# noporpoise/seq-align

Measured on AMD Instinct MI355X. Metric: dp_cell_updates_per_sec, higher is better.
Workload: dtype int32; 1 GPU; C2: 10k NW pairs, DNA 150x150, default scoring 1/-2/-4/-1 (BASELINE configs[1]); pairs_per_gpu=10000, global_pairs=10000, kernel=stream, arena_placement=spread

## Files before the change

include/seqalign_hip.h:

```cpp
#ifndef SEQALIGN_HIP_H
#define SEQALIGN_HIP_H

#include <stddef.h>
#include <stdint.h>

#include "seqalign_compat.h"

#ifdef __cplusplus
extern "C" {
#endif

enum {
  SEQALIGN_OK = 0,
  SEQALIGN_E_NO_DEVICE = 1,
  SEQALIGN_E_HIP = 2,
  SEQALIGN_E_ARG = 3,
  SEQALIGN_E_NOMEM = 4,
  SEQALIGN_E_UNKNOWN_PAIR = 5,
  SEQALIGN_E_DOMAIN = 6,
  SEQALIGN_E_TRACEBACK = 7,
  SEQALIGN_E_TOO_LARGE = 8
};

const char *seqalign_strerror(int code);
// ... 67 lines not shown
  uint32_t *cand_index;
  int32_t *cand_score;
} seqalign_sw_reduce_t;

int seqalign_sw_reduce_device(seqalign_ctx_t *ctx, const seqalign_sw_reduce_t *r,
                              void *stream);

typedef struct {
  const uint64_t *str_off;
  char *out_a, *out_b;
  uint32_t *out_head, *out_len;
  int32_t *out_score;
  uint32_t *status;
  const uint64_t *start_index;
  uint32_t *out_pos;
} seqalign_trace_t;

int seqalign_nw_traceback_device(seqalign_ctx_t *ctx,
                                 const seqalign_dev_scoring_t *scoring,
                                 const seqalign_dev_batch_t *batch,
                                 const seqalign_trace_t *trace, void *stream);
int seqalign_sw_traceback_device(seqalign_ctx_t *ctx,
                                 const seqalign_dev_scoring_t *scoring,
                                 const seqalign_dev_batch_t *batch,
                                 const seqalign_trace_t *trace, void *stream);

int seqalign_fill_batch(seqalign_ctx_t *ctx, const seqalign_batch_t *batch,
                        const scoring_t *scoring, int is_sw,
                        const uint64_t *mat_off, int32_t *match_scores,
                        int32_t *gap_a_scores, int32_t *gap_b_scores,
                        uint64_t *status);

int seqalign_nw_batch(seqalign_ctx_t *ctx, const seqalign_batch_t *batch,
                      const scoring_t *scoring, const uint64_t *str_off,
                      char *out_a, char *out_b, uint32_t *out_len,
                      int32_t *out_score);

typedef struct {
  uint64_t pair;
  int32_t score;
  uint32_t pos_a, pos_b, len_a, len_b;
  uint32_t length;
  uint64_t str_off;
} seqalign_sw_hit_t;

int seqalign_sw_batch(seqalign_ctx_t *ctx, const seqalign_batch_t *batch,
                      const scoring_t *scoring, const int32_t *min_score,
                      uint32_t max_hits, seqalign_sw_hit_t *hits,
                      uint64_t hit_cap, uint64_t *n_hits, char *out_a,
                      char *out_b, uint64_t str_cap);

typedef struct seqalign_job seqalign_job_t;
int seqalign_nw_batch_submit(seqalign_ctx_t *ctx, const seqalign_batch_t *batch, const scoring_t *scoring,
                             const uint64_t *str_off, char *out_a, char *out_b, uint32_t *out_len, int32_t *out_score,
                             seqalign_job_t **job);
int seqalign_sw_batch_submit(seqalign_ctx_t *ctx, const seqalign_batch_t *batch, const scoring_t *scoring,
                             const int32_t *min_score, uint32_t max_hits, seqalign_sw_hit_t *hits, uint64_t hit_cap,
                             uint64_t *n_hits, char *out_a, char *out_b, uint64_t str_cap, seqalign_job_t **job);
int seqalign_job_wait(seqalign_job_t *job);
int seqalign_job_done(seqalign_job_t *job);

int seqalign_fill_batch_multi(seqalign_ctx_t *const *ctxs, int n_ctx,
                              const seqalign_batch_t *batch, const scoring_t *scoring,
                              int is_sw, const uint64_t *mat_off, int32_t *match_scores,
                              int32_t *gap_a_scores, int32_t *gap_b_scores, uint64_t *status);
int seqalign_nw_batch_multi(seqalign_ctx_t *const *ctxs, int n_ctx,
                            const seqalign_batch_t *batch, const scoring_t *scoring,
                            const uint64_t *str_off, char *out_a, char *out_b,
                            uint32_t *out_len, int32_t *out_score);
int seqalign_sw_batch_multi(seqalign_ctx_t *const *ctxs, int n_ctx,
                            const seqalign_batch_t *batch, const scoring_t *scoring,
                            const int32_t *min_score, uint32_t max_hits,
                            seqalign_sw_hit_t *hits, uint64_t hit_cap, uint64_t *n_hits,
                            char *out_a, char *out_b, uint64_t str_cap);

int seqalign_arenas_alloc(seqalign_ctx_t *ctx, uint64_t bytes_each, void *arenas[3], float *quality);
int seqalign_arenas_free(seqalign_ctx_t *ctx, void *arenas[3]);

#define SEQALIGN_ARENA_MAX_TRIES 96
typedef struct {
  float quality;
  float target;
  int32_t vmm;
  uint32_t chunk_mib;
  float depth_gib;
  float scanned_gib;
  float depth_a_gib;
  uint32_t tries;
  uint32_t second_walk_from;
  float try_quality[SEQALIGN_ARENA_MAX_TRIES];
  float try_depth_gib[SEQALIGN_ARENA_MAX_TRIES];
  float kept_gib;
  float seconds;
} seqalign_arena_info_t;
int seqalign_arenas_info(seqalign_ctx_t *ctx, void *const arenas[3], seqalign_arena_info_t *info);

int seqalign_pool_trim(seqalign_ctx_t *ctx, uint64_t keep_bytes, uint64_t *held_bytes);

int seqalign_ctx_set_option(seqalign_ctx_t *ctx, const char *key, const char *value);

int seqalign_ctx_get_option(const seqalign_ctx_t *ctx, const char *key, char *value, size_t cap);

enum {
  SEQALIGN_K_FILL_WAVEFRONT = 0,
  SEQALIGN_K_FILL_ROWSCAN,
  SEQALIGN_K_FILL_STREAM,
  SEQALIGN_K_FILL_STRIPS,
  SEQALIGN_K_FILL_WGSTREAM,
  SEQALIGN_K_FILL_NW_DIRS,
  SEQALIGN_K_FILL_NW_DIRS_X2,
  SEQALIGN_K_FILL_SW_DIRS,
  SEQALIGN_K_FILL_SW_DIRS_X2,
  SEQALIGN_K_FILL_SW_BEST_X2,
  SEQALIGN_K_SW_REDUCE,
  SEQALIGN_K_SW_BOX,
  SEQALIGN_K_SWEEP_REGS,
  SEQALIGN_K_SWEEP_LDS,
  SEQALIGN_K_SWEEP_STRIPS,
  SEQALIGN_K_SWEEP_DIRS,
  SEQALIGN_K_SWEEP_DIRS_X2,
  SEQALIGN_K_WALK_LANE,
  SEQALIGN_K_WALK_WAVE,
  SEQALIGN_K_WALK_DIRS_LANE,
  SEQALIGN_K_WALK_DIRS_TILE,
  SEQALIGN_K_WALK_MOVES_LANE,
  SEQALIGN_K_WALK_MOVES_TILE,
  SEQALIGN_K_FILL_NW_DIRS_X4,
  SEQALIGN_K_FILL_SW_BEST_X4,
  SEQALIGN_K_SCORE_ROWS,
  SEQALIGN_K_SCORE_STRIPS,
  SEQALIGN_K_SCORE_CROSS,
  SEQALIGN_K_SCORE_SELECT,
  SEQALIGN_K_LONG_FORWARD,
  SEQALIGN_K_LONG_BLOCK,
  SEQALIGN_K_LONG_WALK,
  SEQALIGN_K_COUNT
};
#define SEQALIGN_K_MAX 32
#if defined(__cplusplus)
static_assert(SEQALIGN_K_COUNT <= SEQALIGN_K_MAX, "seqalign_call_info_t has SEQALIGN_K_MAX slots");
#elif defined(__STDC_VERSION__) && __STDC_VERSION__ >= 201112L
_Static_assert(SEQALIGN_K_COUNT <= SEQALIGN_K_MAX, "seqalign_call_info_t has SEQALIGN_K_MAX slots");
#endif
typedef struct {
  uint32_t launches[SEQALIGN_K_MAX];
  uint64_t items[SEQALIGN_K_MAX];
} seqalign_call_info_t;
int seqalign_ctx_last_call_info(const seqalign_ctx_t *ctx, seqalign_call_info_t *out);
const char *seqalign_kernel_kind_name(int kind);
enum {
  SEQALIGN_KX_BAND_SCORE = 0,
  SEQALIGN_KX_BAND_FILL,
  SEQALIGN_KX_BAND_WALK,
  SEQALIGN_KX_COUNT
};
#define SEQALIGN_KX_MAX 32
typedef struct {
  uint32_t launches[SEQALIGN_KX_MAX];
  uint64_t items[SEQALIGN_KX_MAX];
} seqalign_call_info_ext_t;
int seqalign_ctx_last_call_info_ext(const seqalign_ctx_t *ctx, seqalign_call_info_ext_t *out);
const char *seqalign_kernel_kind_ext_name(int kind);

size_t seqalign_cigar(const char *result_a, const char *result_b, size_t length, int extended,
                      int case_insensitive, char *out, size_t cap);

#define SEQALIGN_CIGAR_M 1
#define SEQALIGN_CIGAR_EQX 2
int seqalign_nw_batch_cigar(seqalign_ctx_t *ctx, const seqalign_batch_t *batch, const scoring_t *scoring, int format,
                            const uint64_t *cigar_off, char *cigar, uint32_t *cigar_len, int32_t *out_score);
int seqalign_sw_batch_cigar(seqalign_ctx_t *ctx, const seqalign_batch_t *batch, const scoring_t *scoring,
                            const int32_t *min_score, uint32_t max_hits, int format, seqalign_sw_hit_t *hits,
                            uint64_t hit_cap, uint64_t *n_hits, char *cigar, uint64_t cigar_cap);
int seqalign_nw_batch_cigar_submit(seqalign_ctx_t *ctx, const seqalign_batch_t *batch, const scoring_t *scoring, int format,
                                   const uint64_t *cigar_off, char *cigar, uint32_t *cigar_len, int32_t *out_score,
                                   seqalign_job_t **job);
int seqalign_nw_batch_cigar_multi(seqalign_ctx_t *const *ctxs, int n_ctx, const seqalign_batch_t *batch, const scoring_t *scoring,
                                  int format, const uint64_t *cigar_off, char *cigar, uint32_t *cigar_len, int32_t *out_score);
int seqalign_sw_batch_cigar_multi(seqalign_ctx_t *const *ctxs, int n_ctx, const seqalign_batch_t *batch, const scoring_t *scoring,
                                  const int32_t *min_score, uint32_t max_hits, int format, seqalign_sw_hit_t *hits,
                                  uint64_t hit_cap, uint64_t *n_hits, char *cigar, uint64_t cigar_cap);

int seqalign_nw_score_batch(seqalign_ctx_t *ctx, const seqalign_batch_t *batch, const scoring_t *scoring,
                            int32_t *out_score);
int seqalign_sw_score_batch(seqalign_ctx_t *ctx, const seqalign_batch_t *batch, const scoring_t *scoring,
                            int32_t *out_score, uint32_t *out_end_a, uint32_t *out_end_b);
int seqalign_nw_score_batch_multi(seqalign_ctx_t *const *ctxs, int n_ctx, const seqalign_batch_t *batch,
                                  const scoring_t *scoring, int32_t *out_score);
int seqalign_sw_score_batch_multi(seqalign_ctx_t *const *ctxs, int n_ctx, const seqalign_batch_t *batch,
                                  const scoring_t *scoring, int32_t *out_score, uint32_t *out_end_a, uint32_t *out_end_b);
int seqalign_nw_align_long(seqalign_ctx_t *ctx, const seqalign_batch_t *batch, const scoring_t *scoring,
                           const uint64_t *str_off, char *out_a, char *out_b, uint32_t *out_len, int32_t *out_score);
int seqalign_sw_align_long(seqalign_ctx_t *ctx, const seqalign_batch_t *batch, const scoring_t *scoring,
                           const int32_t *min_score, seqalign_sw_hit_t *hits, uint64_t hit_cap, uint64_t *n_hits,
                           char *out_a, char *out_b, uint64_t str_cap);
#define SEQALIGN_BAND_MAX_WIDTH 1024
int seqalign_nw_score_banded(seqalign_ctx_t *ctx, const seqalign_batch_t *batch, const scoring_t *scoring,
                             const uint32_t *band, int32_t *out_score);
int seqalign_nw_align_banded(seqalign_ctx_t *ctx, const seqalign_batch_t *batch, const scoring_t *scoring,
                             const uint32_t *band, const uint64_t *str_off, char *out_a, char *out_b, uint32_t *out_len,
                             int32_t *out_score);
int seqalign_band_score_time_ms(seqalign_ctx_t *ctx, const seqalign_batch_t *batch, const scoring_t *scoring,
                                const uint32_t *band, int repeats, float *ms_each);
typedef struct {
  uint64_t n_seqs;
  const char *arena;
  uint64_t arena_bytes;
  const uint64_t *off;
  const uint32_t *len;
} seqalign_seqset_t;
int seqalign_nw_score_cross(seqalign_ctx_t *ctx, const seqalign_seqset_t *queries, const seqalign_seqset_t *targets,
                            const scoring_t *scoring, int32_t *out_score);
int seqalign_sw_score_cross(seqalign_ctx_t *ctx, const seqalign_seqset_t *queries, const seqalign_seqset_t *targets,
                            const scoring_t *scoring, int32_t *out_score, uint32_t *out_end_a, uint32_t *out_end_b);
int seqalign_nw_score_cross_multi(seqalign_ctx_t *const *ctxs, int n_ctx, const seqalign_seqset_t *queries,
                                  const seqalign_seqset_t *targets, const scoring_t *scoring, int32_t *out_score);
int seqalign_sw_score_cross_multi(seqalign_ctx_t *const *ctxs, int n_ctx, const seqalign_seqset_t *queries,
                                  const seqalign_seqset_t *targets, const scoring_t *scoring, int32_t *out_score,
                                  uint32_t *out_end_a, uint32_t *out_end_b);
#define SEQALIGN_SEARCH_MAX_K 1024
typedef struct {
  uint32_t target;
  int32_t score;
  uint32_t end_a, end_b;
} seqalign_search_hit_t;
int seqalign_nw_score_search(seqalign_ctx_t *ctx, const seqalign_seqset_t *queries, const seqalign_seqset_t *targets,
                             const scoring_t *scoring, uint32_t k, int32_t min_score, seqalign_search_hit_t *hits,
                             uint32_t *n_hits);
int seqalign_sw_score_search(seqalign_ctx_t *ctx, const seqalign_seqset_t *queries, const seqalign_seqset_t *targets,
                             const scoring_t *scoring, uint32_t k, int32_t min_score, seqalign_search_hit_t *hits,
                             uint32_t *n_hits);
int seqalign_nw_score_search_multi(seqalign_ctx_t *const *ctxs, int n_ctx, const seqalign_seqset_t *queries,
                                   const seqalign_seqset_t *targets, const scoring_t *scoring, uint32_t k, int32_t min_score,
                                   seqalign_search_hit_t *hits, uint32_t *n_hits);
int seqalign_sw_score_search_multi(seqalign_ctx_t *const *ctxs, int n_ctx, const seqalign_seqset_t *queries,
                                   const seqalign_seqset_t *targets, const scoring_t *scoring, uint32_t k, int32_t min_score,
                                   seqalign_search_hit_t *hits, uint32_t *n_hits);
int seqalign_score_time_ms(seqalign_ctx_t *ctx, const seqalign_batch_t *batch, const scoring_t *scoring, int is_sw,
                           int repeats, float *ms_each);

int seqalign_host_legs_nw(const seqalign_batch_t *batch, const uint64_t *str_off, char *out_a, char *out_b,
                          uint32_t *out_len, int iterations, double *pack_ms, double *expand_ms);

void *seqalign_ctx_stream(seqalign_ctx_t *ctx);

int seqalign_time_fill_ms(seqalign_ctx_t *ctx,
                          const seqalign_dev_scoring_t *scoring,
                          const seqalign_dev_batch_t *batch, int kernel,
                          void *stream, int repeats, float *ms_each);

#ifdef __cplusplus
}
#endif
#endif
```

seq-align_amd/csrc/sa_batch.hip:

```cpp
#include "sa_ctx.hpp"

using namespace sa_host;



std::vector<Chunk> sa_host::plan_chunks(const seqalign_batch_t *b, size_t budget, size_t bytes_per_cell, const uint64_t *extra_bytes) {
  std::vector<Chunk> out;
  Chunk c;
  const uint64_t per_cell = std::max<size_t>(bytes_per_cell, 1);
  uint64_t used = 0;
  for (uint64_t p = 0; p < b->n_pairs; ++p) {
    const uint64_t cells = (uint64_t)(b->len_a[p] + 1ull) * (b->len_b[p] + 1ull);
    const uint64_t need = cells * per_cell + (extra_bytes ? extra_bytes[p] : 0);
    if (c.count && used + need > budget) { out.push_back(c); c = Chunk(); c.first = p; used = 0; }
    used += need;
    c.count++; c.cells += cells; c.seq_bytes += (uint64_t)b->len_a[p] + b->len_b[p];
    c.max_a = std::max(c.max_a, b->len_a[p]); c.max_b = std::max(c.max_b, b->len_b[p]);
  }
  if (c.count) out.push_back(c);
  return out;
}

int sa_host::ensure_copy_streams(seqalign_ctx *ctx, int count) {
  int least = 0, greatest = 0;
  bool have_range = false;
  for (int k = 0; k < count; ++k) {
    if (ctx->copy_streams[k]) continue;
    if (!have_range) { HIP_TRY(hipDeviceGetStreamPriorityRange(&least, &greatest)); have_range = true; }
    HIP_TRY(hipStreamCreateWithPriority(&ctx->copy_streams[k], hipStreamNonBlocking, k == 0 ? least : greatest));
  }
  return SEQALIGN_OK;
}

int sa_host::run_chunk(seqalign_ctx *ctx, const seqalign_batch_t *b, const Chunk &c,
                       const seqalign_dev_scoring *sc, seqalign_dev_batch_t *dev_out, bool *best_done,
                       const SaCandBox *cand, bool *cand_done, uint64_t uniform_stride) {
  const bool bucket = uniform_stride == kBucketShapes;
  if (bucket) uniform_stride = 0;
  const uint64_t n = c.count;
  int rc;
  StageTimer tm(ctx->opt.timing);
  const size_t desc_bytes = n * (3 * sizeof(uint64_t) + 2 * sizeof(uint32_t)) + (bucket ? 2 * n * sizeof(uint32_t) : 0);
  if ((rc = ctx->h_desc.reserve(desc_bytes))) return rc;
  if ((rc = ctx->h_arena.reserve(c.seq_bytes + 16))) return rc;
  uint64_t *h_off_a = ctx->h_desc.as<uint64_t>(), *h_off_b = h_off_a + n, *h_mat = h_off_b + n;
  uint32_t *h_len_a = reinterpret_cast<uint32_t *>(h_mat + n), *h_len_b = h_len_a + n;
  uint8_t *h_seq = ctx->h_arena.as<uint8_t>();
  uint64_t pos = 0, cell = 0;
  for (uint64_t k = 0; k < n; ++k) {
    const uint64_t p = c.first + k;
    h_off_a[k] = pos; pos += b->len_a[p];
    h_off_b[k] = pos; pos += b->len_b[p];
    h_len_a[k] = b->len_a[p]; h_len_b[k] = b->len_b[p];
    h_mat[k] = uniform_stride ? k * uniform_stride : cell;
    const uint64_t cells_k = (cand && cand->best_only && sa_dirs_blocked_shape(c.max_a)) ? sa_dirs_blocked_bytes(b->len_a[p], b->len_b[p])
                                                                                       : (uint64_t)(b->len_a[p] + 1ull) * (b->len_b[p] + 1ull);
    cell += bucket ? ((cells_k + 255u) & ~(uint64_t)255u) : cells_k;
  }
  const uint64_t mat_total = uniform_stride ? n * uniform_stride : cell;
  uint32_t *h_list = reinterpret_cast<uint32_t *>(h_len_b + n);
  if ((rc = ctx->arena.reserve(c.seq_bytes + 16))) return rc;
  if ((rc = ctx->off_a.reserve(desc_bytes)) || (rc = ctx->status.reserve(n * 8))) return rc;
  const bool no_matrices = cand && cand->best_only;
  const bool packed_dirs = cand && cand->dirs && (bucket || uniform_stride);
  if (!no_matrices && (rc = reserve_arenas(ctx, mat_total * 4, !packed_dirs))) return rc;
  hipStream_t st = ctx->stream;
  uint32_t list_len[2] = {0, 0};
  if (bucket) {
    const bool split = false;
    const uint64_t first = split ? 2048 : n;
    static thread_local std::vector<uint32_t> tl_table;
    const uint64_t Wb = (uint64_t)c.max_b + 1, entries = ((uint64_t)c.max_a + 1) * Wb;
    if (tl_table.size() < entries) tl_table.resize(entries);
    for (int sl = 0; sl < 2; ++sl) {
      const uint64_t k0 = sl ? first : 0, k1 = sl ? n : first;
      uint32_t *out = h_list + 2 * k0;
      uint32_t at = 0;
      for (uint64_t k = k0; k < k1; ++k) tl_table[(uint64_t)h_len_a[k] * Wb + h_len_b[k]] = ~0u;
      for (uint64_t k = k0; k < k1; ++k) {
        uint32_t &slot = tl_table[(uint64_t)h_len_a[k] * Wb + h_len_b[k]];
        if (slot == ~0u) { slot = (uint32_t)k; continue; }
        out[at++] = slot; out[at++] = (uint32_t)k;
        slot = ~0u;
      }
      for (uint64_t k = k0; k < k1; ++k) {
        uint32_t &slot = tl_table[(uint64_t)h_len_a[k] * Wb + h_len_b[k]];
        if (slot == (uint32_t)k) { out[at++] = (uint32_t)k; out[at++] = (uint32_t)k; slot = ~0u; }
      }
      list_len[sl] = at;
    }
  }
  HIP_TRY(hipMemcpyAsync(ctx->off_a.p, h_off_a, desc_bytes, hipMemcpyHostToDevice, st));
  uint64_t *dv_off_a = ctx->off_a.as<uint64_t>(), *dv_off_b = dv_off_a + n, *dv_mat = dv_off_b + n;
  uint32_t *dv_len_a = reinterpret_cast<uint32_t *>(dv_mat + n), *dv_len_b = dv_len_a + n;
  const uint32_t *dv_list = dv_len_b + n;
  if (best_done && ((rc = ctx->best_score.reserve(n * 4)) || (rc = ctx->best_index.reserve(n * 8)))) return rc;
  auto range_desc = [&](uint64_t k0, uint64_t k1) {
    seqalign_dev_batch_t d;
    d.n_pairs = k1 - k0; d.arena = ctx->arena.as<uint8_t>();
    d.off_a = dv_off_a + k0; d.len_a = dv_len_a + k0;
    d.off_b = dv_off_b + k0; d.len_b = dv_len_b + k0;
    d.mat_off = dv_mat + k0;
    d.match_scores = ctx->M.as<int32_t>(); d.gap_a_scores = ctx->A.as<int32_t>(); d.gap_b_scores = ctx->B.as<int32_t>();
    if (no_matrices) d.match_scores = d.gap_a_scores = d.gap_b_scores = nullptr;
    d.status = ctx->status.as<uint64_t>() + k0; d.max_len_a = c.max_a; d.max_len_b = c.max_b;
    return d;
  };
  auto fill_range = [&](uint64_t k0, uint64_t k1, bool *bd, bool *cd, bool *du) -> int {
    if (bucket) {
      seqalign_dev_batch_t dc = range_desc(0, n);
      dc.n_pairs = k1 - k0;
      SaCandBox sub = *cand;
      bool used = false;
      sub.dirs_used = &used; sub.uniform_stride = 256;
      sub.pair_list = dv_list + 2 * k0; sub.list_count = list_len[k0 ? 1 : 0];
      const int r = no_matrices
          ? fill_device(ctx, sc, &dc, SEQALIGN_KERNEL_AUTO, st, ctx->best_score.as<int32_t>(), ctx->best_index.as<uint64_t>(), bd, &sub, nullptr)
          : fill_device(ctx, sc, &dc, SEQALIGN_KERNEL_AUTO, st, nullptr, nullptr, nullptr, &sub, cd);
      if (du) *du = used;
      if (!r && !used) { set_last_error("internal error: the packed fill refused a ragged chunk it had accepted"); return SEQALIGN_E_HIP; }
      return r;
    }
    const seqalign_dev_batch_t d = range_desc(k0, k1);
    if (best_done && no_matrices) {
      SaCandBox sub = *cand;
      bool used = false;
      sub.dirs_used = &used; sub.uniform_stride = uniform_stride;
      const int r = fill_device(ctx, sc, &d, SEQALIGN_KERNEL_AUTO, st, ctx->best_score.as<int32_t>() + k0,
                                ctx->best_index.as<uint64_t>() + k0, bd, &sub, nullptr);
      if (du) *du = used;
      return r;
    }
    if (best_done)
      return fill_device(ctx, sc, &d, SEQALIGN_KERNEL_AUTO, st, ctx->best_score.as<int32_t>() + k0, ctx->best_index.as<uint64_t>() + k0, bd);
    if (cand) {
      SaCandBox sub = *cand;
      sub.uniform_stride = uniform_stride;
      sub.cand_count += k0; sub.cand_box += 4 * k0; sub.cand_min += k0; sub.hit_off += k0;
      bool used = false;
      sub.dirs_used = cand->dirs_used ? &used : nullptr;
      const int r = fill_device(ctx, sc, &d, SEQALIGN_KERNEL_AUTO, st, nullptr, nullptr, nullptr, &sub, cd);
      if (du) *du = used;
      return r;
    }
    return seqalign_fill_batch_device(ctx, sc, &d, SEQALIGN_KERNEL_AUTO, st);
  };
  constexpr uint64_t kPack = 2048;
  const uint64_t n_sub = (n >= 8192 && c.seq_bytes >= ((uint64_t)4 << 20) && ctx->opt.subbatches != 1 && !uniform_stride && !bucket) ? 4 : 1;
  const bool two_slices = (uniform_stride || bucket) && n_sub > 1;
  const uint64_t slice_bytes = n_sub > 1 ? (c.seq_bytes + n_sub - 1) / n_sub : ((uint64_t)2 << 20);
  { int rc_s = ensure_copy_streams(ctx, 1); if (rc_s) return rc_s; }
  hipStream_t su = ctx->copy_streams[0];
  StreamSyncOnExit sync_u(su);
  EventList ev;
  HIP_TRY(ev.add(hipEventDisableTiming));
  HIP_TRY(hipEventRecord(ev.ev[0], st));
  HIP_TRY(hipStreamWaitEvent(su, ev.ev[0], 0));
  bool first = true, consistent = true, bd0 = false, cd0 = false, du0 = false;
  uint64_t filled_to = 0;
  for (uint64_t k0 = 0; k0 < n;) {
    uint64_t k1 = k0;
    if (two_slices) {
      k1 = k0 == 0 ? std::min(n, kPack) : n;
    } else {
      while (k1 < n && (k1 == k0 || h_off_a[k1] - h_off_a[k0] < slice_bytes)) k1 = std::min(n, k1 + kPack);
    }
    if (n - k1 < kPack) k1 = n;
    constexpr uint64_t kTask = 256;
    parallel_for((k1 - k0 + kTask - 1) / kTask, [&](uint64_t blk) {
      for (uint64_t k = k0 + blk * kTask, e = std::min(k1, k0 + (blk + 1) * kTask); k < e; ++k) {
        const uint64_t p = c.first + k;
        memcpy(h_seq + h_off_a[k], b->arena + b->off_a[p], b->len_a[p]);
        memcpy(h_seq + h_off_b[k], b->arena + b->off_b[p], b->len_b[p]);
      }
    });
    const uint64_t lo = h_off_a[k0], hi = k1 < n ? h_off_a[k1] : c.seq_bytes;
    if (hi > lo) HIP_TRY(hipMemcpyAsync(ctx->arena.as<uint8_t>() + lo, h_seq + lo, hi - lo, hipMemcpyHostToDevice, su));
    HIP_TRY(ev.add(hipEventDisableTiming));
    HIP_TRY(hipEventRecord(ev.ev.back(), su));
    HIP_TRY(hipStreamWaitEvent(st, ev.ev.back(), 0));
    if (n_sub > 1 && consistent) {
      bool bd = false, cd = false, du = false;
      if ((rc = fill_range(k0, k1, &bd, &cd, &du))) return rc;
      if (first) { bd0 = bd; cd0 = cd; du0 = du; first = false; }
      else if (bd != bd0 || cd != cd0 || du != du0) consistent = false;
      filled_to = k1;
    }
    k0 = k1;
  }
  tm.lap("run_chunk: pack + H2D");
  const seqalign_dev_batch_t d = range_desc(0, n);
  if (n_sub > 1 && consistent && filled_to == n) {
    if (best_done) *best_done = bd0;
    if (cand_done) *cand_done = cd0;
    if (cand && cand->dirs_used) *cand->dirs_used = du0;
    rc = SEQALIGN_OK;
  } else {
    bool bd = false, cd = false, du = false;
    rc = fill_range(0, n, &bd, &cd, &du);
    if (best_done) *best_done = bd;
    if (cand_done) *cand_done = cd;
    if (cand && cand->dirs_used) *cand->dirs_used = du;
  }
  if (rc) return rc;
  tm.lap("run_chunk: enqueue fill");
  if (dev_out) *dev_out = d;
  return SEQALIGN_OK;
}

int sa_host::fetch_status(seqalign_ctx *ctx, const Chunk &c, uint64_t *status_out) {
  int rc;
  if ((rc = ctx->h_misc.reserve(c.count * 8))) return rc;
  uint64_t *h = ctx->h_misc.as<uint64_t>();
  HIP_TRY(hipMemcpyAsync(h, ctx->status.p, c.count * 8, hipMemcpyDeviceToHost, ctx->stream));
  HIP_TRY(stream_wait_spinning(ctx->stream));
  rc = SEQALIGN_OK;
  for (uint64_t k = 0; k < c.count; ++k) {
    if (status_out) status_out[c.first + k] = h[k];
    if (h[k] != ~0ull) rc = SEQALIGN_E_UNKNOWN_PAIR;
  }
  return rc;
}

int sa_host::check_batch(const seqalign_batch_t *b) {
  if (!batch_readable(b)) return SEQALIGN_E_ARG;
  for (uint64_t p = 0; p < b->n_pairs; ++p)
    if ((uint64_t)(b->len_a[p] + 1ull) * (b->len_b[p] + 1ull) >= (1ull << 31)) return SEQALIGN_E_TOO_LARGE;
  return SEQALIGN_OK;
}


static int copy_out_pipelined(seqalign_ctx *ctx, void *dst, const void *src_dev, size_t bytes) {
  const size_t kSlice = (size_t)32 << 20;
  if (bytes < (size_t)4 << 20) {
    HIP_TRY(hipMemcpyAsync(dst, src_dev, bytes, hipMemcpyDeviceToHost, ctx->stream));
    HIP_TRY(hipStreamSynchronize(ctx->stream));
    return SEQALIGN_OK;
  }
  int rc;
  if ((rc = ctx->h_M.reserve(kSlice)) || (rc = ctx->h_A.reserve(kSlice))) return rc;
  void *pin[2] = {ctx->h_M.p, ctx->h_A.p};
  EventList events;
  HIP_TRY(events.add(hipEventDisableTiming));
  HIP_TRY(events.add(hipEventDisableTiming));
  const hipEvent_t *ev = events.ev.data();
  StreamSyncOnExit sync(ctx->stream);
  const size_t n_slices = (bytes + kSlice - 1) / kSlice;
  hipError_t e = hipSuccess;
  for (size_t i = 0; i <= n_slices && e == hipSuccess; ++i) {
    if (i < n_slices) {
      const size_t off = i * kSlice, len = std::min(kSlice, bytes - off);
      e = hipMemcpyAsync(pin[i & 1], static_cast<const char *>(src_dev) + off, len, hipMemcpyDeviceToHost, ctx->stream);
      if (e == hipSuccess) e = hipEventRecord(ev[i & 1], ctx->stream);
    }
    if (i > 0 && e == hipSuccess) {
      const size_t j = i - 1, off = j * kSlice, len = std::min(kSlice, bytes - off);
      e = hipEventSynchronize(ev[j & 1]);
      if (e == hipSuccess) parallel_memcpy(static_cast<char *>(dst) + off, pin[j & 1], len);
    }
  }
  if (e != hipSuccess) return fail_hip(e, "pipelined D2H");
  return SEQALIGN_OK;
}

extern "C" int seqalign_fill_batch(seqalign_ctx_t *ctx, const seqalign_batch_t *batch, const scoring_t *scoring,
                                   int is_sw, const uint64_t *mat_off, int32_t *M, int32_t *A, int32_t *B,
                                   uint64_t *status) {
  if (!ctx || !scoring || !mat_off || !M || !A || !B) return SEQALIGN_E_ARG;
  CallScope scope(ctx);
  int rc = check_batch(batch);
  if (rc) return rc;
  if (batch->n_pairs == 0) return SEQALIGN_OK;
  HIP_TRY(hipSetDevice(ctx->device));
  seqalign_dev_scoring *sc = nullptr;
  if ((rc = cached_scoring(ctx, scoring, is_sw, &sc))) return rc;
  return fill_batch_uploaded(ctx, batch, sc, mat_off, M, A, B, status);
}

int sa_host::fill_batch_uploaded(seqalign_ctx_t *ctx, const seqalign_batch_t *batch, const seqalign_dev_scoring *sc,
                                 const uint64_t *mat_off, int32_t *M, int32_t *A, int32_t *B, uint64_t *status) {
  int rc = SEQALIGN_OK;
  int worst = SEQALIGN_OK;
  for (const Chunk &c : plan_chunks(batch, ctx->chunk_budget)) {
    if ((rc = run_chunk(ctx, batch, c, sc, nullptr))) break;
    const size_t small = c.cells * 4;
    if (3 * small <= ((size_t)4 << 20)) {
      const size_t status_at = (3 * small + 7) & ~(size_t)7;
      if ((rc = ctx->h_M.reserve(status_at + c.count * 8 + 64))) break;
      char *pin = ctx->h_M.as<char>();
      hipStream_t st = ctx->stream;
      StreamSyncOnExit sync(st);
      HIP_TRY(hipMemcpyAsync(pin, ctx->M.p, small, hipMemcpyDeviceToHost, st));
      HIP_TRY(hipMemcpyAsync(pin + small, ctx->A.p, small, hipMemcpyDeviceToHost, st));
      HIP_TRY(hipMemcpyAsync(pin + 2 * small, ctx->B.p, small, hipMemcpyDeviceToHost, st));
      HIP_TRY(hipMemcpyAsync(pin + status_at, ctx->status.p, c.count * 8, hipMemcpyDeviceToHost, st));
      HIP_TRY(hipStreamSynchronize(st));
      uint64_t dev_cell = 0;
      const uint64_t *h_status = reinterpret_cast<const uint64_t *>(pin + status_at);
      for (uint64_t k = 0; k < c.count; ++k) {
        const uint64_t p = c.first + k, cells = (uint64_t)(batch->len_a[p] + 1ull) * (batch->len_b[p] + 1ull);
        memcpy(M + mat_off[p], pin + dev_cell * 4, cells * 4);
        memcpy(A + mat_off[p], pin + small + dev_cell * 4, cells * 4);
        memcpy(B + mat_off[p], pin + 2 * small + dev_cell * 4, cells * 4);
        dev_cell += cells;
        if (status) status[p] = h_status[k];
        if (h_status[k] != ~0ull) worst = SEQALIGN_E_UNKNOWN_PAIR;
      }
      continue;
    }
    uint64_t k = 0, dev_cell = 0;
    while (k < c.count) {
      uint64_t run_cells = 0, j = k;
      const uint64_t host0 = mat_off[c.first + k];
      while (j < c.count && mat_off[c.first + j] == host0 + run_cells) {
        run_cells += (uint64_t)(batch->len_a[c.first + j] + 1ull) * (batch->len_b[c.first + j] + 1ull);
        ++j;
      }
      const size_t bytes = run_cells * 4;
      if ((rc = copy_out_pipelined(ctx, M + host0, ctx->M.as<int32_t>() + dev_cell, bytes)) ||
          (rc = copy_out_pipelined(ctx, A + host0, ctx->A.as<int32_t>() + dev_cell, bytes)) ||
          (rc = copy_out_pipelined(ctx, B + host0, ctx->B.as<int32_t>() + dev_cell, bytes)))
        break;
      dev_cell += run_cells;
      k = j;
    }
    if (rc) break;
    int src = fetch_status(ctx, c, status);
    if (src == SEQALIGN_E_UNKNOWN_PAIR) worst = src;
    else if (src) { rc = src; break; }
  }
  return rc ? rc : worst;
}


void sa_host::parallel_memcpy(void *dst, const void *src, size_t bytes) {
  const size_t kPiece = (size_t)2 << 20;
  const uint64_t pieces = (bytes + kPiece - 1) / kPiece;
  parallel_for(pieces, [&](uint64_t i) {
    const size_t off = i * kPiece;
    memcpy(static_cast<char *>(dst) + off, static_cast<const char *>(src) + off, std::min(kPiece, bytes - off));
  });
}
// ... 293 lines not shown
                          uint32_t *out_len, int32_t *out_score) {
  const uint64_t n = c.count, nb = blk.size();
  int rc;
  StageTimer tm(ctx->opt.timing);
  const bool auto_zc = ctx->opt.zero_copy == 4u;
  const bool tile_walks = ctx->opt.trace_kernel ? ctx->opt.trace_kernel == 2 : (ctx->opt.dirs_local != 0 || n < SA_WALK_TILE_MAX);
  const bool zc_in = !auto_zc && (ctx->opt.zero_copy & 1u) != 0, zc_out = auto_zc ? tile_walks : (ctx->opt.zero_copy & 2u) != 0;
  const bool local = tile_walks && ctx->opt.dirs_local;
  bool same_shape = true;
  for (const BlkSum &s : blk) same_shape = same_shape && s.same;

  enum { kBackToBack, kUniform, kMixed } layout = kBackToBack;
  uint64_t stride = 0;
  const bool blocked = sa_dirs_blocked_shape(c.max_a);
  auto dir_bytes = [&](uint32_t la, uint32_t lb) -> uint64_t {
    return ((blocked ? sa_dirs_blocked_bytes(la, lb) : (uint64_t)(la + 1ull) * (lb + 1ull)) + 255u) & ~(uint64_t)255u;
  };
  const bool may_pack = ctx->opt.pack16 && (n >= kPackedFillMinPairs || ctx->opt.pack16 == 2);
  if (same_shape && may_pack && nw_dirs_x2_applicable(ctx, sc, c.max_a, c.max_b)) {
    layout = kUniform;
    stride = dir_bytes(c.max_a, c.max_b);
  } else if (!same_shape && may_pack && (n >= kBucketedFillMinPairs || ctx->opt.pack16 == 2) && (uint64_t)(c.max_a + 1ull) * (c.max_b + 1ull) <= kShapeTableMax &&
             nw_dirs_x2_applicable(ctx, sc, c.max_a, c.max_b)) {
    layout = kMixed;
  }
  std::vector<uint64_t> chars_at(nb + 1, 0), cells_at(nb + 1, 0);
  for (uint64_t bi = 0; bi < nb; ++bi) {
    chars_at[bi + 1] = chars_at[bi] + blk[bi].chars;
    const uint64_t in_blk = std::min(n, (bi + 1) * kHostBlk) - bi * kHostBlk;
    cells_at[bi + 1] = cells_at[bi] + (layout == kUniform ? in_blk * stride : blocked ? blk[bi].blk256 : layout == kMixed ? blk[bi].cells256 : blk[bi].cells);
  }
  const uint64_t total = chars_at[nb], mat_total = cells_at[nb];

  const size_t desc_bytes = (4 * n + 1) * sizeof(uint64_t) + 2 * n * sizeof(uint32_t);
  const uint64_t move_words = 2 * ((total >> 5) + n) + 2;
  if ((rc = ctx->h_desc.reserve(desc_bytes)) || (rc = ctx->h_arena.reserve(total + 64)) ||
      (rc = ctx->h_ta.reserve(move_words * 4)) || (rc = ctx->h_tmeta.reserve(n * 8)) ||
      (rc = ctx->dirs.reserve(mat_total + 4096)) || (rc = ctx->best_score.reserve(n * 4)) || (rc = ctx->best_index.reserve(n * 8)) ||
      (rc = ctx->status.reserve(n * 8)))
    return rc;
  if (!zc_in && ((rc = ctx->arena.reserve(total + 64)) || (rc = ctx->off_a.reserve(desc_bytes)))) return rc;
  if (!zc_out && ((rc = ctx->t_out_a.reserve(move_words * 4)) || (rc = ctx->t_meta.reserve(n * 8)))) return rc;
  if ((rc = ensure_copy_streams(ctx, 3))) return rc;
  hipStream_t sf = ctx->stream, su = ctx->copy_streams[0], sd = ctx->copy_streams[1];

  uint64_t *h_off_a = ctx->h_desc.as<uint64_t>(), *h_off_b = h_off_a + n, *h_mat = h_off_b + n, *h_slot = h_mat + n;
  uint32_t *h_len_a = reinterpret_cast<uint32_t *>(h_slot + n + 1), *h_len_b = h_len_a + n;
  uint8_t *h_seq = ctx->h_arena.as<uint8_t>();
  uint32_t *h_moves = ctx->h_ta.as<uint32_t>(), *h_meta = ctx->h_tmeta.as<uint32_t>();
  parallel_for(nb, [&](uint64_t bi) {
    uint64_t pos = chars_at[bi], cell = cells_at[bi];
    for (uint64_t k = bi * kHostBlk, e = std::min(n, (bi + 1) * kHostBlk); k < e; ++k) {
      const uint32_t la = batch->len_a[c.first + k], lb = batch->len_b[c.first + k];
      h_slot[k] = pos; h_off_a[k] = pos; pos += la; h_off_b[k] = pos; pos += lb;
      h_len_a[k] = la; h_len_b[k] = lb;
      h_mat[k] = cell;
      const uint64_t cells = (uint64_t)(la + 1ull) * (lb + 1ull);
      cell += layout == kUniform ? stride : blocked ? dir_bytes(la, lb) : layout == kMixed ? ((cells + 255u) & ~(uint64_t)255u) : cells;
    }
  });
  h_slot[n] = total;

  const uint32_t n_sub = (uint32_t)std::min<uint64_t>(pick_subbatches(ctx, c), nb);
  std::vector<uint64_t> bcut(n_sub + 1, nb);
  bcut[0] = 0;
  if (layout == kUniform && n_sub > 1 && n / n_sub >= 8192 && kHostBlk <= 4096 && 4096 % kHostBlk == 0) {
    const uint64_t per = (((n + n_sub - 1) / n_sub + 4095u) & ~(uint64_t)4095u) / kHostBlk;
    for (uint32_t s = 1; s < n_sub; ++s) bcut[s] = std::min<uint64_t>(nb, s * per);
  } else {
    uint64_t bi = 0;
    for (uint32_t s = 1; s < n_sub; ++s) {
      const uint64_t want = mat_total / n_sub * s;
      while (bi < nb && cells_at[bi] < want) ++bi;
      bcut[s] = std::max(bi, bcut[s - 1]);
    }
  }
  auto pair_at = [&](uint64_t bi) { return std::min(n, bi * kHostBlk); };
  constexpr uint64_t kGroupPairs = 32768;
  std::vector<uint32_t> gcut{0};
  for (uint32_t s = 1; s < n_sub; ++s)
    if (pair_at(bcut[s]) - pair_at(bcut[gcut.back()]) >= kGroupPairs && n - pair_at(bcut[s]) >= kGroupPairs / 2) gcut.push_back(s);
  gcut.push_back(n_sub);
  const uint32_t n_grp = (uint32_t)gcut.size() - 1;
  const bool walk_beside = ctx->opt.walk_overlap && n_grp > 1;
  hipStream_t sw = walk_beside ? ctx->copy_streams[2] : sf;
  StreamSyncOnExit sync_f(sf), sync_u(su), sync_d(sd), sync_w(sw);

  std::vector<uint32_t> list_at;
  const uint32_t *dv_list = nullptr;
  if (layout == kMixed) {
    const uint64_t entries = (uint64_t)(c.max_a + 1ull) * (c.max_b + 1ull);
    if ((rc = ctx->h_misc.reserve(n * 4 + 16)) || (!zc_in && (rc = ctx->pair_list.reserve(n * 4 + 16)))) return rc;
    uint32_t *h_list = ctx->h_misc.as<uint32_t>();
    list_at.assign(2 * n_sub + 1, 0);
    parallel_for(n_sub, [&](uint64_t s2) {
      static thread_local std::vector<uint32_t> tl_table;
      std::vector<uint32_t> &table = tl_table;
      if (table.size() < entries) table.resize(entries);
      const uint64_t k0 = pair_at(bcut[s2]), k1 = pair_at(bcut[s2 + 1]);
      const uint32_t Wb = c.max_b + 1;
      for (uint64_t k = k0; k < k1; ++k) table[(uint64_t)h_len_a[k] * Wb + h_len_b[k]] = ~0u;
      uint32_t at = (uint32_t)k0;
      for (uint64_t k = k0; k < k1; ++k) {
        uint32_t &slot = table[(uint64_t)h_len_a[k] * Wb + h_len_b[k]];
        if (slot == ~0u) { slot = (uint32_t)k; continue; }
        h_list[at++] = slot; h_list[at++] = (uint32_t)k;
        slot = ~0u;
      }
      const uint32_t paired_end = at;
      for (uint64_t k = k0; k < k1; ++k) {
        uint32_t &slot = table[(uint64_t)h_len_a[k] * Wb + h_len_b[k]];
        if (slot == (uint32_t)k) { h_list[at++] = (uint32_t)k; slot = ~0u; }
      }
      list_at[2 * s2] = (uint32_t)k0; list_at[2 * s2 + 1] = paired_end;
    });
    list_at[2 * n_sub] = (uint32_t)n;
    if (zc_in) dv_list = ctx->h_misc.dev_as<uint32_t>();
    else { dv_list = ctx->pair_list.as<uint32_t>(); HIP_TRY(hipMemcpyAsync(ctx->pair_list.p, h_list, n * 4, hipMemcpyHostToDevice, su)); }
  }

  EventList ev;
  for (uint32_t k = 0; k < n_sub + 3 * n_grp + 1; ++k) HIP_TRY(ev.add(hipEventDisableTiming));
  if (!zc_in && layout == kUniform) {
    hipLaunchKernelGGL(uniform_descriptors_kernel, dim3((unsigned)((n + 256) / 256)), dim3(256), 0, sf, ctx->off_a.as<uint64_t>(),
                       n, c.max_a, c.max_b, stride);
    HIP_TRY(hipGetLastError());
    if (sw != sf) {
      HIP_TRY(hipEventRecord(ev.ev[n_sub + 3 * n_grp], sf));
      HIP_TRY(hipStreamWaitEvent(sw, ev.ev[n_sub + 3 * n_grp], 0));
    }
  } else if (!zc_in) {
    HIP_TRY(hipMemcpyAsync(ctx->off_a.p, h_off_a, desc_bytes, hipMemcpyHostToDevice, sd));
    HIP_TRY(hipEventRecord(ev.ev[n_sub + 3 * n_grp], sd));
    HIP_TRY(hipStreamWaitEvent(sf, ev.ev[n_sub + 3 * n_grp], 0));
    if (sw != sf) HIP_TRY(hipStreamWaitEvent(sw, ev.ev[n_sub + 3 * n_grp], 0));
  }

  const uint64_t *dv_off_a = zc_in ? ctx->h_desc.dev_as<uint64_t>() : ctx->off_a.as<uint64_t>();
  const uint64_t *dv_off_b = dv_off_a + n, *dv_mat = dv_off_b + n, *dv_slot = dv_mat + n;
  const uint32_t *dv_len_a = reinterpret_cast<const uint32_t *>(dv_slot + n + 1), *dv_len_b = dv_len_a + n;
  const uint8_t *dv_seq = zc_in ? ctx->h_arena.dev_as<uint8_t>() : ctx->arena.as<uint8_t>();
  uint32_t *dv_moves = zc_out ? ctx->h_ta.dev_as<uint32_t>() : ctx->t_out_a.as<uint32_t>();
  uint32_t *dv_meta = zc_out ? ctx->h_tmeta.dev_as<uint32_t>() : ctx->t_meta.as<uint32_t>();
  auto dev_range = [&](uint64_t k0, uint64_t k1) {
    seqalign_dev_batch_t d;
    d.n_pairs = k1 - k0; d.arena = dv_seq;
    d.off_a = dv_off_a + k0; d.len_a = dv_len_a + k0; d.off_b = dv_off_b + k0; d.len_b = dv_len_b + k0;
    d.mat_off = dv_mat + k0;
    d.match_scores = d.gap_a_scores = d.gap_b_scores = nullptr;
    d.status = ctx->status.as<uint64_t>() + k0; d.max_len_a = c.max_a; d.max_len_b = c.max_b;
    return d;
  };
  auto move_word = [&](uint64_t k) { return 2 * ((h_slot[k] >> 5) + k); };
  tm.lap("nw moves: sizes, offsets, buffers");

  uint32_t g = 0;
  for (uint32_t s = 0; s < n_sub; ++s) {
    const uint64_t b0 = bcut[s], b1 = bcut[s + 1], k0 = pair_at(b0), k1 = pair_at(b1);
    if (k1 > k0) {
      const uint64_t n_blocks = b1 - b0;
      const uint64_t n_slices = zc_in ? 1 : std::min<uint64_t>(ctx->opt.upload_slices ? ctx->opt.upload_slices : 1, std::max<uint64_t>(1, n_blocks / 2));
      constexpr uint64_t kParts = 4;
      for (uint64_t sl = 0; sl < n_slices; ++sl) {
        const uint64_t sb0 = b0 + n_blocks * sl / n_slices, sb1 = b0 + n_blocks * (sl + 1) / n_slices;
        parallel_for((sb1 - sb0) * kParts, [&](uint64_t ti) {
          const uint64_t bi = sb0 + ti / kParts, part = ti % kParts;
          const uint64_t kb = bi * kHostBlk, ke = std::min(n, (bi + 1) * kHostBlk), span = ke - kb;
          const uint64_t ka = kb + span * part / kParts, kz = kb + span * (part + 1) / kParts;
          if (kz <= ka) return;
          if (blk[bi].packed) {
            const uint64_t bytes = (kz < n ? h_off_a[kz] : total) - h_off_a[ka];
            memcpy(h_seq + h_off_a[ka], batch->arena + batch->off_a[c.first + ka], bytes);
            return;
          }
          for (uint64_t k = ka; k < kz; ++k) {
            const uint64_t p = c.first + k;
            memcpy(h_seq + h_off_a[k], batch->arena + batch->off_a[p], h_len_a[k]);
            memcpy(h_seq + h_off_b[k], batch->arena + batch->off_b[p], h_len_b[k]);
          }
        });
        if (!zc_in) {
          const uint64_t c0 = h_slot[pair_at(sb0)], c1 = h_slot[pair_at(sb1)];
          if (c1 > c0) HIP_TRY(hipMemcpyAsync(ctx->arena.as<uint8_t>() + c0, h_seq + c0, c1 - c0, hipMemcpyHostToDevice, su));
        }
      }
      if (!zc_in) {
        HIP_TRY(hipEventRecord(ev.ev[s], su));
        HIP_TRY(hipStreamWaitEvent(sf, ev.ev[s], 0));
      }
      const seqalign_dev_batch_t d = dev_range(k0, k1);
      if (layout == kMixed) {
        const seqalign_dev_batch_t dm = dev_range(0, n);
        const uint32_t m0 = list_at[2 * s], m1 = list_at[2 * s + 1], r1 = list_at[2 * s + 2];
        if ((rc = nw_dirs_fill_mixed(ctx, sc, &dm, ctx->dirs.as<uint8_t>(), ctx->best_score.as<int32_t>(), ctx->best_index.as<uint64_t>(),
                                     sf, dv_list + m0, m1 - m0, r1 - m1, c.max_a, c.max_b, local)))
          return rc;
      } else {
        bool used = false;
        if ((rc = nw_dirs_fill(ctx, sc, &d, ctx->dirs.as<uint8_t>(), ctx->best_score.as<int32_t>() + k0,
                               ctx->best_index.as<uint64_t>() + k0, sf, &used, layout == kUniform ? stride : 0, nullptr, 0, local)))
          return rc;
        if (!used) { set_last_error("seqalign_nw_batch: internal error: directions-only fill refused a batch it had accepted"); return SEQALIGN_E_HIP; }
      }
    }
    if (s + 1 == gcut[g + 1]) {
      const uint64_t g0 = pair_at(bcut[gcut[g]]), g1 = k1;
      if (g1 > g0) {
        const seqalign_dev_batch_t d = dev_range(g0, g1);
        SaTraceParams t;
        memset(&t, 0, sizeof(t));
        t.arena = d.arena; t.off_a = d.off_a; t.len_a = d.len_a; t.off_b = d.off_b; t.len_b = d.len_b; t.mat_off = d.mat_off;
        t.code = sc->d_code; t.table = sc->d_table;
        t.str_off = dv_slot + g0;
        t.stage_words = (c.max_a + c.max_b + 31u) >> 5;
        t.moves = dv_moves + 2 * g0;
        t.out_meta2 = dv_meta + 2 * g0;
        t.fill_status = d.status;
        t.dirs = ctx->dirs.as<uint8_t>(); t.dirs_blocked = blocked; t.dirs_local = local; t.tune_stage = ctx->opt.walk_stage; t.tune_tile = ctx->opt.walk_tile; t.nw_score = ctx->best_score.as<int32_t>() + g0; t.nw_state = ctx->best_index.as<uint64_t>() + g0;
        t.n_pairs = (uint32_t)(g1 - g0); t.K = sc->flat.n_classes; t.open1 = sc->flat.open1; t.ext = sc->flat.ext;
        t.gen_eq = sc->flat.gen_eq; t.gen_ne = sc->flat.gen_ne; t.flags = sc->flat.flags;
        t.tune_walker = ctx->opt.trace_kernel; t.tune_group = ctx->opt.walk_group;
        hipStream_t sg = g + 1 < n_grp ? sw : sf;
        if (sg != sf) {
          HIP_TRY(hipEventRecord(ev.ev[n_sub + 2 * n_grp + g], sf));
          HIP_TRY(hipStreamWaitEvent(sg, ev.ev[n_sub + 2 * n_grp + g], 0));
        }
        hipError_t e = sa_launch_nw_traceback(t, sg);
        if (e != hipSuccess) return fail_hip(e, "traceback launch");
        if (zc_out) {
          HIP_TRY(hipEventRecord(ev.ev[n_sub + n_grp + g], sg));
        } else {
          HIP_TRY(hipEventRecord(ev.ev[n_sub + g], sg));
          HIP_TRY(hipStreamWaitEvent(sd, ev.ev[n_sub + g], 0));
          const uint64_t w0 = move_word(g0), w1 = g1 < n ? move_word(g1) : move_words - 2;
          HIP_TRY(hipMemcpyAsync(h_moves + w0, ctx->t_out_a.as<uint32_t>() + w0, (w1 - w0) * 4, hipMemcpyDeviceToHost, sd));
          HIP_TRY(hipMemcpyAsync(h_meta + 2 * g0, ctx->t_meta.as<uint32_t>() + 2 * g0, (g1 - g0) * 8, hipMemcpyDeviceToHost, sd));
          HIP_TRY(hipEventRecord(ev.ev[n_sub + n_grp + g], sd));
        }
      } else {
        HIP_TRY(hipEventRecord(ev.ev[n_sub + n_grp + g], sf));
      }
      ++g;
    }
  }
  tm.lap("nw moves: packed + enqueued");

  std::atomic<uint64_t> first_bad{~0ull};
  for (g = 0; g < n_grp; ++g) {
    { const hipError_t e = wait_event_spinning(ev.ev[n_sub + n_grp + g]); if (e != hipSuccess) return fail_hip(e, "waiting for a group's walk"); }
    const uint64_t b0 = bcut[gcut[g]], b1 = bcut[gcut[g + 1]];
    constexpr uint64_t kOut = 128;
    const uint64_t k_lo = pair_at(b0), k_hi = pair_at(b1);
    parallel_for((k_hi - k_lo + kOut - 1) / kOut, [&](uint64_t blk_i) {
      for (uint64_t k = k_lo + blk_i * kOut, e = std::min(k_hi, k_lo + (blk_i + 1) * kOut); k < e; ++k) {
        const uint64_t p = c.first + k;
        if (k + 6 < e) {
          const uint64_t kn = k + 6;
          const uint32_t nwn = (h_len_a[kn] + h_len_b[kn] + 31u) >> 5;
          const uint32_t *pn = h_moves + move_word(kn);
          __builtin_prefetch(h_meta + 2 * kn); __builtin_prefetch(pn + nwn - 1); __builtin_prefetch(pn + 2 * nwn - 1);
          __builtin_prefetch(batch->arena + batch->off_a[c.first + kn]);
        }
        const uint32_t n_moves = h_meta[2 * k + 1];
        int prc = SEQALIGN_OK;
        if (n_moves >= SA_MOVES_ERR) {
          prc = (int)(n_moves & 15u);
        } else {
          const uint32_t nw = (h_len_a[k] + h_len_b[k] + 31u) >> 5;
          const uint32_t *pa = h_moves + move_word(k);
          if (ctx->cigar_format)
            prc = sa_cigar_nw_moves(batch->arena + batch->off_a[p], h_len_a[k], batch->arena + batch->off_b[p], h_len_b[k], pa, pa + nw,
                                    nw, n_moves, ctx->cigar_format, ctx->cigar_fold, out_a + str_off[p], str_off[p + 1] - str_off[p],
                                    &out_len[p], nullptr);
          else
            prc = sa_expand_nw_moves(batch->arena + batch->off_a[p], h_len_a[k], batch->arena + batch->off_b[p], h_len_b[k], pa, pa + nw,
                                     nw, n_moves, out_a + str_off[p], out_b + str_off[p], &out_len[p]);
          out_score[p] = (int32_t)h_meta[2 * k];
        }
        if (prc != SEQALIGN_OK) {
          uint64_t seen = first_bad.load(std::memory_order_relaxed);
          const uint64_t mine = k << 8 | (uint64_t)prc;
          while (mine < seen && !first_bad.compare_exchange_weak(seen, mine, std::memory_order_relaxed)) {}
        }
      }
    });
  }
  tm.lap("nw moves: groups expanded");
  if (first_bad.load() != ~0ull) return (int)(first_bad.load() & 255u);
  return SEQALIGN_OK;
}

extern "C" int seqalign_host_legs_nw(const seqalign_batch_t *batch, const uint64_t *str_off, char *out_a, char *out_b,
                                     uint32_t *out_len, int iterations, double *pack_ms, double *expand_ms) {
  if (!batch || !str_off || !out_a || !out_b || !out_len || iterations <= 0 || !pack_ms || !expand_ms) return SEQALIGN_E_ARG;
  const uint64_t n = batch->n_pairs, kHostBlk = 512;
  if (!n) return SEQALIGN_OK;
  std::vector<BlkSum> blk;
  std::vector<uint64_t> off_a(n), off_b(n), mat(n), slot(n + 1), chars_at, cells_at;
  std::vector<uint32_t> la(n), lb(n);
  std::vector<uint8_t> seq;
  std::vector<uint32_t> moves;
  auto now_ms = [] { timespec t; clock_gettime(CLOCK_MONOTONIC, &t); return t.tv_sec * 1e3 + t.tv_nsec * 1e-6; };
  double t_pack = 0, t_expand = 0;
  for (int it = 0; it < iterations; ++it) {
    const double t0 = now_ms();
    scan_blocks(batch, 0, n, kHostBlk, blk);
    const uint64_t nb = blk.size();
    chars_at.assign(nb + 1, 0); cells_at.assign(nb + 1, 0);
    for (uint64_t bi = 0; bi < nb; ++bi) { chars_at[bi + 1] = chars_at[bi] + blk[bi].chars; cells_at[bi + 1] = cells_at[bi] + blk[bi].cells256; }
    const uint64_t total = chars_at[nb];
    if (seq.size() < total + 64) seq.resize(total + 64);
    if (moves.size() < 2 * ((total >> 5) + n) + 2) moves.assign(2 * ((total >> 5) + n) + 2, 0u);
    parallel_for(nb, [&](uint64_t bi) {
      uint64_t pos = chars_at[bi], cell = cells_at[bi];
      for (uint64_t k = bi * kHostBlk, e = std::min(n, (bi + 1) * kHostBlk); k < e; ++k) {
        la[k] = batch->len_a[k]; lb[k] = batch->len_b[k];
        slot[k] = pos; off_a[k] = pos; pos += la[k]; off_b[k] = pos; pos += lb[k];
        mat[k] = cell; cell += (((uint64_t)(la[k] + 1ull) * (lb[k] + 1ull)) + 255u) & ~(uint64_t)255u;
      }
    });
    parallel_for(nb, [&](uint64_t bi) {
      if (blk[bi].packed) { memcpy(seq.data() + off_a[bi * kHostBlk], batch->arena + batch->off_a[bi * kHostBlk], blk[bi].chars); return; }
      for (uint64_t k = bi * kHostBlk, e = std::min(n, (bi + 1) * kHostBlk); k < e; ++k) {
        memcpy(seq.data() + off_a[k], batch->arena + batch->off_a[k], la[k]);
        memcpy(seq.data() + off_b[k], batch->arena + batch->off_b[k], lb[k]);
      }
    });
    const double t1 = now_ms();
    constexpr uint64_t kOut = 128;
    std::atomic<int> bad{0};
    parallel_for((n + kOut - 1) / kOut, [&](uint64_t bi) {
      for (uint64_t k = bi * kOut, e = std::min(n, (bi + 1) * kOut); k < e; ++k) {
        const uint32_t nw = (la[k] + lb[k] + 31u) >> 5;
        const uint32_t *pa = moves.data() + 2 * ((slot[k] >> 5) + k);
        if (sa_expand_nw_moves(batch->arena + batch->off_a[k], la[k], batch->arena + batch->off_b[k], lb[k], pa, pa + nw, nw,
                               std::min(la[k], lb[k]), out_a + str_off[k], out_b + str_off[k], &out_len[k]))
          bad.store(1);
      }
    });
    const double t2 = now_ms();
    if (bad.load()) return SEQALIGN_E_TRACEBACK;
    t_pack += t1 - t0; t_expand += t2 - t1;
  }
  *pack_ms = t_pack / iterations; *expand_ms = t_expand / iterations;
  return SEQALIGN_OK;
}

static constexpr int kNeedsStrings = -1;
static int nw_batch_impl(seqalign_ctx_t *ctx, const seqalign_batch_t *batch, const scoring_t *scoring,
                         const uint64_t *str_off, char *out_a, char *out_b, uint32_t *out_len,
                         int32_t *out_score) {
  const seqalign_batch_t *b = batch;
  if (!batch_readable(b)) return SEQALIGN_E_ARG;
  if (batch->n_pairs == 0) return SEQALIGN_OK;
  int rc;
  std::vector<BlkSum> blk;
  const uint64_t blk_pairs = host_block_pairs(ctx, batch->n_pairs);
  scan_blocks(batch, 0, batch->n_pairs, blk_pairs, blk);
  Chunk whole;
  whole.count = batch->n_pairs;
  uint64_t cells256 = 0;
  for (const BlkSum &s : blk) {
    if (s.too_large) return SEQALIGN_E_TOO_LARGE;
    whole.cells += s.cells; whole.seq_bytes += s.chars; cells256 += std::max(s.cells256, s.blk256);
    whole.max_a = std::max(whole.max_a, s.max_a); whole.max_b = std::max(whole.max_b, s.max_b);
  }
  HIP_TRY(hipSetDevice(ctx->device));
  seqalign_dev_scoring *sc = nullptr;
  if ((rc = cached_scoring(ctx, scoring, 0, &sc))) return rc;
  const bool on_host = traceback_on_host(ctx);
  if (!on_host && ctx->opt.nw_moves && nw_dirs_applicable(ctx, sc, whole.max_a, batch->n_pairs)) {
    if (cells256 + 64 * batch->n_pairs + whole.seq_bytes <= ctx->chunk_budget)
      return nw_chunk_moves(ctx, batch, whole, sc, blk, blk_pairs, str_off, out_a, out_b, out_len, out_score);
    std::vector<uint64_t> extra(batch->n_pairs, 256 + 64);
    if (SA_DIRS_BLOCKED)
      for (uint64_t p = 0; p < batch->n_pairs; ++p) {
        const uint64_t cells = (uint64_t)(batch->len_a[p] + 1ull) * (batch->len_b[p] + 1ull), bb = sa_dirs_blocked_bytes(batch->len_a[p], batch->len_b[p]);
        if (bb > cells) extra[p] += bb - cells;
      }
    for (const Chunk &c : plan_chunks(batch, ctx->chunk_budget, 1, extra.data())) {
      const uint64_t bp = host_block_pairs(ctx, c.count);
      scan_blocks(batch, c.first, c.count, bp, blk);
      if ((rc = nw_chunk_moves(ctx, batch, c, sc, blk, bp, str_off, out_a, out_b, out_len, out_score))) return rc;
    }
    return SEQALIGN_OK;
  }
  if (ctx->cigar_format) return kNeedsStrings;
  const size_t budget = on_host ? std::min<size_t>(ctx->chunk_budget, (size_t)6 << 30) : ctx->chunk_budget;
  for (const Chunk &c : plan_chunks(batch, budget)) {
    seqalign_dev_batch_t d;
    if (!on_host) {
      if ((rc = nw_chunk_pipelined(ctx, batch, c, sc, pick_subbatches(ctx, c), str_off, out_a, out_b, out_len, out_score))) return rc;
      continue;
    }
    if ((rc = run_chunk(ctx, batch, c, sc, &d))) return rc;
    const size_t bytes = c.cells * 4;
    if ((rc = ctx->h_M.reserve(bytes)) || (rc = ctx->h_A.reserve(bytes)) || (rc = ctx->h_B.reserve(bytes))) return rc;
// ... 86 lines not shown
```

seq-align_amd/csrc/sa_batch_score.hip:

```cpp
#include "sa_ctx.hpp"

using namespace sa_host;

namespace {

constexpr int kRowClasses = SA_SCORE_ROW_CLASSES;
constexpr int kStripClass = kRowClasses;
constexpr uint64_t kPairBytes = 64;
constexpr uint64_t kChunkMaxPairs = (uint64_t)1 << 24;

uint64_t handoff_rows(uint32_t la, uint32_t lb) {
  return la > SA_SCORE_ROW_MAX ? (uint64_t)(sa_score_strips_per_pair(la) - 1) * ((uint64_t)lb + 1) : 0;
}

struct ScoreChunk {
  uint64_t first = 0, count = 0, seq_bytes = 0;
};

std::vector<ScoreChunk> plan_score_chunks(const seqalign_batch_t *b, size_t budget) {
  std::vector<ScoreChunk> out;
  ScoreChunk c;
  uint64_t used = 0;
  for (uint64_t p = 0; p < b->n_pairs; ++p) {
    const uint32_t la = b->len_a[p], lb = b->len_b[p];
    const uint64_t strips = la > SA_SCORE_ROW_MAX ? sa_score_strips_per_pair(la) : 0;
    const uint64_t need = (uint64_t)la + lb + kPairBytes + 8 * handoff_rows(la, lb) + 20 * strips;
    if (c.count && (used + need > budget || c.count == kChunkMaxPairs)) { out.push_back(c); c = ScoreChunk(); c.first = p; used = 0; }
    used += need;
    c.count++; c.seq_bytes += (uint64_t)la + lb;
  }
  if (c.count) out.push_back(c);
  return out;
}

}

SaFillParams sa_host::score_fill_params(const seqalign_dev_scoring *s) {
  SaFillParams p;
  memset(&p, 0, sizeof(p));
  p.code = s->d_code; p.table = s->d_table; p.K = s->flat.n_classes;
  p.gap_open = s->flat.gap_open; p.open1 = s->flat.open1; p.ext = s->flat.ext; p.floor = s->flat.floor;
  p.gen_eq = s->flat.gen_eq; p.gen_ne = s->flat.gen_ne; p.flags = s->flat.flags;
  p.table_abs_max = s->table_abs_max;
  return p;
}

namespace {

struct ScoreChunkRun {
  seqalign_ctx *ctx = nullptr;
  const seqalign_dev_scoring *sc = nullptr;
  bool is_sw = false;
  uint64_t n = 0;
  std::vector<uint32_t> order;
  uint64_t cls_first[kRowClasses + 2] = {};
  uint32_t cls_max_a[kRowClasses + 1] = {};
  uint32_t spp = 1;
  uint64_t strip_words = 0;
  uint64_t *d_off_a = nullptr, *d_off_b = nullptr, *d_hoff = nullptr;
  uint32_t *d_len_a = nullptr, *d_len_b = nullptr;
  uint32_t *d_res = nullptr;

  int prepare(const seqalign_batch_t *b, const ScoreChunk &c) {
    int rc;
    n = c.count;
    uint64_t hand_total = 0;
    order.resize(n);
    sort_by_row_class(n, [&](uint64_t k) { return b->len_a[c.first + k]; }, order.data(), cls_first, cls_max_a);
    const uint64_t n_strip = cls_first[kStripClass + 1] - cls_first[kStripClass];
    spp = n_strip ? sa_score_strips_per_pair(cls_max_a[kStripClass]) : 1;
    strip_words = ((n_strip + 7) / 8) * 8 * spp;

    const size_t desc_bytes = n * (3 * sizeof(uint64_t) + 2 * sizeof(uint32_t));
    if ((rc = ctx->h_desc.reserve(desc_bytes)) || (rc = ctx->h_arena.reserve(c.seq_bytes + 16))) return rc;
    uint64_t *h_off_a = ctx->h_desc.as<uint64_t>(), *h_off_b = h_off_a + n, *h_hoff = h_off_b + n;
    uint32_t *h_len_a = reinterpret_cast<uint32_t *>(h_hoff + n), *h_len_b = h_len_a + n;
    std::vector<uint64_t> seq_at(n);
    { uint64_t pos = 0;
      for (uint64_t k = 0; k < n; ++k) { seq_at[k] = pos; pos += (uint64_t)b->len_a[c.first + k] + b->len_b[c.first + k]; } }
    for (uint64_t s = 0; s < n; ++s) {
      const uint64_t k = order[s], p = c.first + k;
      const uint32_t la = b->len_a[p], lb = b->len_b[p];
      h_off_a[s] = seq_at[k]; h_off_b[s] = seq_at[k] + la;
      h_len_a[s] = la; h_len_b[s] = lb;
      h_hoff[s] = hand_total; hand_total += handoff_rows(la, lb);
    }
    uint8_t *h_seq = ctx->h_arena.as<uint8_t>();
    constexpr uint64_t kTask = 256;
    parallel_for((n + kTask - 1) / kTask, [&](uint64_t blk) {
      for (uint64_t k = blk * kTask, e = std::min(n, (blk + 1) * kTask); k < e; ++k) {
        const uint64_t p = c.first + k;
        memcpy(h_seq + seq_at[k], b->arena + b->off_a[p], b->len_a[p]);
        memcpy(h_seq + seq_at[k] + b->len_a[p], b->arena + b->off_b[p], b->len_b[p]);
      }
    });

    if ((rc = ctx->arena.reserve(c.seq_bytes + 16)) || (rc = ctx->off_a.reserve(desc_bytes)) || (rc = ctx->status.reserve(n * 8)) ||
        (rc = ctx->best_score.reserve(16 + 12 * n)))
      return rc;
    if (n_strip && ((rc = ctx->strip_progress.reserve(sa_strip_progress_bytes(strip_words))) ||
                    (rc = ctx->score_handoff.reserve(8 * hand_total + 16))))
      return rc;
    hipStream_t st = ctx->stream;
    HIP_TRY(hipMemcpyAsync(ctx->off_a.p, h_off_a, desc_bytes, hipMemcpyHostToDevice, st));
    if (c.seq_bytes) HIP_TRY(hipMemcpyAsync(ctx->arena.p, h_seq, c.seq_bytes, hipMemcpyHostToDevice, st));
    d_off_a = ctx->off_a.as<uint64_t>(); d_off_b = d_off_a + n; d_hoff = d_off_b + n;
    d_len_a = reinterpret_cast<uint32_t *>(d_hoff + n); d_len_b = d_len_a + n;
    d_res = ctx->best_score.as<uint32_t>();
    return SEQALIGN_OK;
  }

  int launch() {
    hipStream_t st = ctx->stream;
    HIP_TRY(hipMemsetAsync(d_res, 0, 16, st));
    const SaFillParams f0 = score_fill_params(sc);
    for (int x = 0; x <= kRowClasses; ++x) {
      const uint64_t s0 = cls_first[x], m = cls_first[x + 1] - s0;
      if (!m) continue;
      SaScoreParams p;
      memset(&p, 0, sizeof(p));
      p.f = f0;
      p.f.arena = ctx->arena.as<uint8_t>();
      p.f.off_a = d_off_a + s0; p.f.off_b = d_off_b + s0; p.f.len_a = d_len_a + s0; p.f.len_b = d_len_b + s0;
      p.f.status = ctx->status.as<uint64_t>() + s0;
      p.f.n_pairs = (uint32_t)m;
      p.score = reinterpret_cast<int32_t *>(d_res + 4) + s0;
      p.end_a = d_res + 4 + n + s0; p.end_b = d_res + 4 + 2 * n + s0;
      p.err_flag = d_res;
      hipError_t e;
      if (x == kStripClass) {
        p.progress = ctx->strip_progress.as<uint32_t>();
        p.strip_best = p.progress + sa_strip_best_word(strip_words);
        p.handoff = ctx->score_handoff.as<int32_t>();
        p.handoff_off = d_hoff + s0;
        p.strips_per_pair = spp;
        HIP_TRY(hipMemsetAsync(p.progress, 0, 4 * (strip_words + 1), st));
        HIP_TRY(hipMemsetAsync(p.f.status, 0xff, 8 * m, st));
        e = sa_launch_score_strips(p, is_sw, st);
      } else {
        e = sa_launch_score_rows(p, cls_max_a[x], is_sw, st);
      }
      if (e != hipSuccess) return fail_hip(e, "score kernel launch");
    }
    return SEQALIGN_OK;
  }

  int finish(uint64_t first, int32_t *out_score, uint32_t *out_end_a, uint32_t *out_end_b, uint64_t *fail_pair = nullptr) {
    int rc;
    const size_t words = 4 + (is_sw ? 3 : 1) * n;
    if ((rc = ctx->h_misc.reserve(std::max<size_t>(4 * words, 8 * n)))) return rc;
    uint32_t *h = ctx->h_misc.as<uint32_t>();
    HIP_TRY(hipMemcpyAsync(h, d_res, 4 * words, hipMemcpyDeviceToHost, ctx->stream));
    HIP_TRY(stream_wait_spinning(ctx->stream));
    if (h[0]) {
      std::vector<uint64_t> status(n);
      HIP_TRY(hipMemcpy(status.data(), ctx->status.p, 8 * n, hipMemcpyDeviceToHost));
      uint64_t worst = ~0ull;
      for (uint64_t s = 0; s < n; ++s)
        if (status[s] != ~0ull) worst = std::min<uint64_t>(worst, order[s]);
      if (fail_pair) *fail_pair = first + worst;
      return fail_unknown_pair(first + worst);
    }
    const int32_t *hs = reinterpret_cast<const int32_t *>(h + 4);
    const uint32_t *ha = h + 4 + n, *hb = h + 4 + 2 * n;
    constexpr uint64_t kTask = 16384;
    parallel_for((n + kTask - 1) / kTask, [&](uint64_t blk) {
      for (uint64_t s = blk * kTask, e = std::min(n, (blk + 1) * kTask); s < e; ++s) {
        const uint64_t p = first + order[s];
        out_score[p] = hs[s];
        if (is_sw) { out_end_a[p] = ha[s]; out_end_b[p] = hb[s]; }
      }
    });
    return SEQALIGN_OK;
  }
};

int check_score_batch(const seqalign_batch_t *b) {
  if (!batch_readable(b)) return SEQALIGN_E_ARG;
  return SEQALIGN_OK;
}

}

int sa_host::score_batch_impl(seqalign_ctx_t *ctx, const seqalign_batch_t *batch, const scoring_t *scoring, bool is_sw,
                              int32_t *out_score, uint32_t *out_end_a, uint32_t *out_end_b, uint64_t *fail_pair) {
  int rc = check_score_batch(batch);
  if (rc) return rc;
  if (batch->n_pairs == 0) return SEQALIGN_OK;
  HIP_TRY(hipSetDevice(ctx->device));
  seqalign_dev_scoring *sc = nullptr;
  if ((rc = cached_scoring(ctx, scoring, is_sw ? 1 : 0, &sc))) return rc;
  StreamSyncOnExit sync(ctx->stream);
  for (const ScoreChunk &c : plan_score_chunks(batch, ctx->chunk_budget)) {
    ScoreChunkRun run;
    run.ctx = ctx; run.sc = sc; run.is_sw = is_sw;
    if ((rc = run.prepare(batch, c)) || (rc = run.launch()) ||
        (rc = run.finish(c.first, out_score, out_end_a, out_end_b, fail_pair)))
      return rc;
  }
  return SEQALIGN_OK;
}

extern "C" int seqalign_nw_score_batch(seqalign_ctx_t *ctx, const seqalign_batch_t *batch, const scoring_t *scoring,
                                       int32_t *out_score) {
  if (!ctx || !scoring || !out_score) return SEQALIGN_E_ARG;
  CallScope scope(ctx);
  return score_batch_impl(ctx, batch, scoring, false, out_score, nullptr, nullptr);
}

extern "C" int seqalign_sw_score_batch(seqalign_ctx_t *ctx, const seqalign_batch_t *batch, const scoring_t *scoring,
                                       int32_t *out_score, uint32_t *out_end_a, uint32_t *out_end_b) {
  if (!ctx || !scoring || !out_score || !out_end_a || !out_end_b) return SEQALIGN_E_ARG;
  CallScope scope(ctx);
  return score_batch_impl(ctx, batch, scoring, true, out_score, out_end_a, out_end_b);
}

extern "C" int seqalign_score_time_ms(seqalign_ctx_t *ctx, const seqalign_batch_t *batch, const scoring_t *scoring, int is_sw,
                                      int repeats, float *ms_each) {
  if (!ctx || !scoring || repeats <= 0 || !ms_each) return SEQALIGN_E_ARG;
  CallScope scope(ctx);
  int rc = check_score_batch(batch);
  if (rc) return rc;
  if (batch->n_pairs == 0) return SEQALIGN_E_ARG;
  const std::vector<ScoreChunk> chunks = plan_score_chunks(batch, ctx->chunk_budget);
  if (chunks.size() != 1) { set_last_error("seqalign_score_time_ms: the batch does not fit one chunk"); return SEQALIGN_E_ARG; }
  HIP_TRY(hipSetDevice(ctx->device));
  seqalign_dev_scoring *sc = nullptr;
  if ((rc = cached_scoring(ctx, scoring, is_sw ? 1 : 0, &sc))) return rc;
  StreamSyncOnExit sync(ctx->stream);
  ScoreChunkRun run;
  run.ctx = ctx; run.sc = sc; run.is_sw = is_sw != 0;
  if ((rc = run.prepare(batch, chunks[0]))) return rc;
  EventList events;
  for (int r = 0; r < 2 * repeats; ++r) HIP_TRY(events.add());
  for (int r = 0; r < repeats; ++r) {
    HIP_TRY(hipEventRecord(events.ev[2 * r], ctx->stream));
    if ((rc = run.launch())) return rc;
    HIP_TRY(hipEventRecord(events.ev[2 * r + 1], ctx->stream));
  }
  HIP_TRY(hipStreamSynchronize(ctx->stream));
  for (int r = 0; r < repeats; ++r) HIP_TRY(hipEventElapsedTime(&ms_each[r], events.ev[2 * r], events.ev[2 * r + 1]));
  return SEQALIGN_OK;
}
```

seq-align_amd/csrc/sa_ctx.hpp:

```cpp
#pragma once
#include <hip/hip_runtime.h>
#include <sched.h>
#include <time.h>

#include <algorithm>
#include <atomic>
#include <chrono>
#include <condition_variable>
#include <functional>
#include <thread>
#include <cstdio>
#include <cstdlib>
#include <cstring>
#include <mutex>
#include <string>
#include <vector>

#include "sa_kernels.h"

extern "C" {
#include "sa_internal.h"
}

namespace sa_host {
// ... 94 lines not shown
  const std::function<void(uint64_t)> *fn_ = nullptr;
  uint64_t n_ = 0;
  std::atomic<uint64_t> generation_{0}, next_{0}, open_{0};
  std::atomic<unsigned> active_{0}, sleepers_{0};
  std::atomic<bool> stop_{false};
};

template <class F>
void parallel_for(uint64_t n, F fn) {
  HostPool::get().run(n, std::function<void(uint64_t)>(fn));
}


struct StageTimer {
  bool on;
  explicit StageTimer(bool enabled) : on(enabled) {}
  std::chrono::steady_clock::time_point t = std::chrono::steady_clock::now();
  void lap(const char *what) {
    if (!on) return;
    const auto now = std::chrono::steady_clock::now();
    fprintf(stderr, "[seqalign timing] %-34s %8.3f ms\n", what, std::chrono::duration<double, std::milli>(now - t).count());
    t = now;
  }
};

int fail_hip(hipError_t e, const char *what);
void set_last_error(const std::string &msg);
#define HIP_TRY(expr)                                            \
  do {                                                           \
    hipError_t _e = (expr);                                      \
    if (_e != hipSuccess) return sa_host::fail_hip(_e, #expr);   \
  } while (0)


struct StreamSyncOnExit {
  hipStream_t st;
  explicit StreamSyncOnExit(hipStream_t s) : st(s) {}
  ~StreamSyncOnExit();
  StreamSyncOnExit(const StreamSyncOnExit &) = delete;
  StreamSyncOnExit &operator=(const StreamSyncOnExit &) = delete;
};

struct EventList {
  std::vector<hipEvent_t> ev;
  ~EventList() { for (hipEvent_t e : ev) (void)hipEventDestroy(e); }
  hipError_t add(unsigned flags = hipEventDefault) {
    hipEvent_t e;
    const hipError_t rc = hipEventCreateWithFlags(&e, flags);
    if (rc == hipSuccess) ev.push_back(e);
    return rc;
  }
};

inline hipError_t wait_event_spinning(hipEvent_t e) {
  timespec t0, t1;
  clock_gettime(CLOCK_MONOTONIC, &t0);
  for (unsigned spins = 1;; ++spins) {
    const hipError_t q = hipEventQuery(e);
    if (q != hipErrorNotReady) return q;
    HostPool::cpu_relax();
    if ((spins & 63u) == 0) {
      clock_gettime(CLOCK_MONOTONIC, &t1);
      if ((t1.tv_sec - t0.tv_sec) * 1000000000ll + (t1.tv_nsec - t0.tv_nsec) > 3000000ll) return hipEventSynchronize(e);
    }
  }
}

inline hipError_t stream_wait_spinning(hipStream_t st, long long budget_ns = 3000000ll) {
  timespec t0, t1;
  clock_gettime(CLOCK_MONOTONIC, &t0);
  for (unsigned spins = 1;; ++spins) {
    const hipError_t q = hipStreamQuery(st);
    if (q != hipErrorNotReady) return q;
    HostPool::cpu_relax();
    if ((spins & 63u) == 0) {
      clock_gettime(CLOCK_MONOTONIC, &t1);
      if ((t1.tv_sec - t0.tv_sec) * 1000000000ll + (t1.tv_nsec - t0.tv_nsec) > budget_ns) return hipStreamSynchronize(st);
    }
  }
}

inline StreamSyncOnExit::~StreamSyncOnExit() { (void)stream_wait_spinning(st, 200000ll); }

struct DevBuf {
  void *p = nullptr;
  size_t cap = 0;
  int reserve(size_t bytes) {
    if (bytes <= cap) return SEQALIGN_OK;
    release();
    size_t want = bytes + bytes / 8 + 256;
    int dev = -1;
    if (want >= kPoolFrom && hipGetDevice(&dev) == hipSuccess && (p = sa_pool_alloc(dev, want))) {
      cap = (want + kPoolChunk - 1) / kPoolChunk * kPoolChunk;
      return SEQALIGN_OK;
    }
    hipError_t e = hipMalloc(&p, want);
    if (e != hipSuccess) { p = nullptr; return fail_hip(e, "hipMalloc"); }
    cap = want;
    return SEQALIGN_OK;
  }
  void release() { if (p && !sa_pool_free(p)) (void)hipFree(p); p = nullptr; cap = 0; }
  static constexpr size_t kPoolFrom = (size_t)128 << 20, kPoolChunk = (size_t)512 << 20;
  template <class T> T *as() const { return static_cast<T *>(p); }
};

struct HostBuf {
  void *p = nullptr;
  void *dev = nullptr;
  size_t cap = 0;
  int reserve(size_t bytes) {
    if (bytes <= cap) return SEQALIGN_OK;
    if (p) (void)hipHostFree(p);
    p = nullptr; dev = nullptr; cap = 0;
    size_t want = bytes + bytes / 8 + 256;
    hipError_t e = hipHostMalloc(&p, want, hipHostMallocDefault);
    if (e != hipSuccess) { p = nullptr; return fail_hip(e, "hipHostMalloc"); }
    e = hipHostGetDevicePointer(&dev, p, 0);
    if (e != hipSuccess) { (void)hipHostFree(p); p = nullptr; dev = nullptr; return fail_hip(e, "hipHostGetDevicePointer"); }
    cap = want;
    return SEQALIGN_OK;
  }
  void release() { if (p) (void)hipHostFree(p); p = nullptr; dev = nullptr; cap = 0; }
  template <class T> T *as() const { return static_cast<T *>(p); }
  template <class T> T *dev_as() const { return static_cast<T *>(dev); }
};


}


struct SaOptions {
  int kernel = 0;
  uint32_t cpl = 0;
  uint32_t wpb = 0;
  uint32_t lds_pad = 0;
  bool traceback_host = false;
  uint32_t trace_kernel = 0;
  int sweep_mode = 0;
  uint32_t sweep_strip = 0;
  uint32_t sweep_cpl = 0;
  bool sweep_ev = true;
  bool sweep_trace = false;
  bool nw_dirs = true;
  bool sweep_dirs = true;
  int pack16 = 1;
  uint32_t quad = 0;
  bool walk_overlap = false;
  bool nw_moves = true;
  uint32_t zero_copy = 4;
  uint32_t reduce_depth = 0;
  bool timing = false;
  size_t chunk_bytes = 0;
  uint32_t upload_slices = 0;
  uint32_t subbatches = 0;
  uint32_t arena_scan_gib = 160;
  float arena_quality = 1.045f;
  uint32_t arena_free_pct = 60;
  uint32_t dirs_local = 1;
  uint32_t walk_tile = 0;
  uint32_t walk_stage = 1;
  uint32_t walk_group = 0;
  uint32_t async_lanes = 0;
  uint32_t long_block_rows = 0;
  uint32_t arena_keep_gib = 16;
};

struct seqalign_dev_scoring {
  sa_flat_scoring_t flat;
  uint16_t *d_code = nullptr;
  int32_t *d_table = nullptr;
  int32_t table_abs_max = 0;
};

struct seqalign_ctx {
  int device = 0;
  SaOptions opt;
  hipStream_t stream = nullptr;
  hipStream_t stream2 = nullptr;
  hipStream_t copy_streams[3] = {nullptr, nullptr, nullptr};
  size_t chunk_budget = 0;
  size_t chunk_budget_default = 0;
  sa_host::DevBuf arena, off_a, pair_list, status;
  sa_host::DevBuf M, A, B;
  SaArenaSet *arena_set = nullptr;
  bool arena_placed = false;
  uint32_t arena_walks = 0;
  sa_host::HostBuf h_one;
  void *one_dev = nullptr;
  sa_host::DevBuf dirs;
  sa_host::DevBuf best_score, best_index, cand_count, cand_off, cand_cap, cand_index, cand_score;
  sa_host::DevBuf t_str_off, t_out_a, t_out_b, t_meta;
  sa_host::DevBuf e[14];
  sa_host::DevBuf strip_progress;
  sa_host::DevBuf score_handoff;
  sa_host::DevBuf search_list;
  sa_host::DevBuf long_ckpt, long_block;
  sa_host::HostBuf h_desc, h_arena, h_M, h_A, h_B, h_misc, h_ta, h_tb, h_tmeta;
  seqalign_call_info_t call_info = {};
  seqalign_call_info_ext_t call_info_ext = {};
  int call_depth = 0;
  seqalign_dev_scoring *cached[2] = {nullptr, nullptr};
  uint64_t cached_fp[2] = {0, 0};
  void *async = nullptr;
  int cigar_format = 0;
  bool cigar_fold = false;
};


namespace sa_host {

struct CallScope {
  seqalign_ctx *ctx;
  seqalign_call_info_t *prev;
  seqalign_call_info_ext_t *prev_ext;
  explicit CallScope(seqalign_ctx *c);
  ~CallScope();
  CallScope(const CallScope &) = delete;
  CallScope &operator=(const CallScope &) = delete;
};

void async_shutdown(seqalign_ctx *ctx);

SaFillParams score_fill_params(const seqalign_dev_scoring *s);
int score_batch_impl(seqalign_ctx_t *ctx, const seqalign_batch_t *batch, const scoring_t *scoring, bool is_sw,
                     int32_t *out_score, uint32_t *out_end_a, uint32_t *out_end_b, uint64_t *fail_pair = nullptr);
int score_cross_check(const seqalign_seqset_t *queries, const seqalign_seqset_t *targets);
int score_cross_call(seqalign_ctx_t *ctx, const seqalign_seqset_t *queries, const seqalign_seqset_t *targets,
                     const scoring_t *scoring, bool is_sw, int32_t *out_score, uint32_t *out_end_a, uint32_t *out_end_b,
                     uint64_t q_base);
int score_search_check(const seqalign_seqset_t *queries, const seqalign_seqset_t *targets, uint32_t k);
int score_search_call(seqalign_ctx_t *ctx, const seqalign_seqset_t *queries, const seqalign_seqset_t *targets,
                      const scoring_t *scoring, bool is_sw, uint32_t k, int32_t min_score, seqalign_search_hit_t *hits,
                      uint32_t *n_hits, uint64_t q_base);

struct CigarScope {
  seqalign_ctx *ctx;
  CigarScope(seqalign_ctx *c, int format, bool fold) : ctx(c) { c->cigar_format = format; c->cigar_fold = fold; }
  ~CigarScope() { ctx->cigar_format = 0; ctx->cigar_fold = false; }
  CigarScope(const CigarScope &) = delete;
  CigarScope &operator=(const CigarScope &) = delete;
};

uint64_t put_alignment(const seqalign_ctx *ctx, const char *sa, const char *sb, uint32_t len, char *out_a, char *out_b, uint64_t at, uint64_t room);

int reserve_arenas(seqalign_ctx *ctx, size_t bytes, bool placed = true);

int cached_scoring(seqalign_ctx *ctx, const scoring_t *scoring, int is_sw, seqalign_dev_scoring **out);

int fill_device(seqalign_ctx_t *ctx, const seqalign_dev_scoring_t *scoring, const seqalign_dev_batch_t *batch,
                int kernel, void *stream, int32_t *best_score, uint64_t *best_index, bool *best_done,
                const SaCandBox *cand = nullptr, bool *cand_done = nullptr);

struct Chunk {
  uint64_t first = 0, count = 0;
  uint64_t cells = 0, seq_bytes = 0;
  uint32_t max_a = 0, max_b = 0;
};

std::vector<Chunk> plan_chunks(const seqalign_batch_t *b, size_t budget, size_t bytes_per_cell = 12, const uint64_t *extra_bytes = nullptr);
int run_chunk(seqalign_ctx *ctx, const seqalign_batch_t *b, const Chunk &c, const seqalign_dev_scoring *sc,
              seqalign_dev_batch_t *dev_out, bool *best_done = nullptr, const SaCandBox *cand = nullptr,
              bool *cand_done = nullptr, uint64_t uniform_stride = 0);
int ensure_copy_streams(seqalign_ctx *ctx, int count);
constexpr uint64_t kBucketShapes = ~(uint64_t)0;
constexpr uint64_t kShapeTableMax = (uint64_t)1 << 20;
int fetch_status(seqalign_ctx *ctx, const Chunk &c, uint64_t *status_out);
int nw_dirs_fill(seqalign_ctx_t *ctx, const seqalign_dev_scoring_t *scoring, const seqalign_dev_batch_t *batch, uint8_t *dirs,
                 int32_t *end_score, uint64_t *end_state, void *stream, bool *used, uint64_t uniform_stride = 0,
                 const uint32_t *pair_list = nullptr, uint32_t list_count = 0, bool local = false);
int nw_dirs_fill_mixed(seqalign_ctx_t *ctx, const seqalign_dev_scoring_t *scoring, const seqalign_dev_batch_t *batch, uint8_t *dirs,
                       int32_t *end_score, uint64_t *end_state, void *stream, const uint32_t *list, uint32_t n_modal, uint32_t n_rest,
                       uint32_t modal_a, uint32_t modal_b, bool local = false);
bool nw_dirs_applicable(const seqalign_ctx_t *ctx, const seqalign_dev_scoring_t *scoring, uint32_t max_len_a, uint64_t n_pairs = ~0ull);
bool nw_dirs_x2_applicable(const seqalign_ctx_t *ctx, const seqalign_dev_scoring_t *scoring, uint32_t len_a, uint32_t len_b);
constexpr uint64_t kPackedFillMinPairs = 1025;
constexpr uint64_t kBucketedFillMinPairs = 2048;
bool sw_best_x2_applicable(const seqalign_ctx_t *ctx, const seqalign_dev_scoring_t *scoring, uint32_t len_a, uint32_t len_b);
int sw_traceback_dirs(seqalign_ctx_t *ctx, const seqalign_dev_scoring_t *sc, const seqalign_dev_batch_t *b, const seqalign_trace_t *t,
                      const uint8_t *dirs, const int32_t *start_score, void *stream);
bool sw_dirs_x2_applicable(const seqalign_ctx_t *ctx, const seqalign_dev_scoring_t *scoring, uint32_t len_a, uint32_t len_b);
static inline bool batch_readable(const seqalign_batch_t *b) {
  return b && (!b->n_pairs || (b->arena && b->off_a && b->off_b && b->len_a && b->len_b));
}
int check_batch(const seqalign_batch_t *b);
template <class Len>
void sort_by_row_class(uint64_t n, Len len, uint32_t *order, uint64_t (&cls_first)[SA_SCORE_ROW_CLASSES + 2],
                       uint32_t (&cls_max_a)[SA_SCORE_ROW_CLASSES + 1]) {
  std::fill(std::begin(cls_first), std::end(cls_first), 0);
  std::fill(std::begin(cls_max_a), std::end(cls_max_a), 0);
  std::vector<uint8_t> cls(n);
  for (uint64_t k = 0; k < n; ++k) {
    const uint32_t la = len(k);
    const int x = sa_score_row_class(la);
    cls[k] = (uint8_t)x;
    cls_first[x + 1]++;
    cls_max_a[x] = std::max(cls_max_a[x], la);
  }
  for (int x = 0; x <= SA_SCORE_ROW_CLASSES; ++x) cls_first[x + 1] += cls_first[x];
  uint64_t at[SA_SCORE_ROW_CLASSES + 1];
  std::copy(cls_first, cls_first + SA_SCORE_ROW_CLASSES + 1, at);
  for (uint64_t k = 0; k < n; ++k) order[at[cls[k]]++] = (uint32_t)k;
}
static inline int fail_unknown_pair(uint64_t pair) {
  set_last_error("pair " + std::to_string(pair) + ": a character pair without a score");
  return SEQALIGN_E_UNKNOWN_PAIR;
}
int fill_batch_uploaded(seqalign_ctx_t *ctx, const seqalign_batch_t *batch, const seqalign_dev_scoring *sc,
                        const uint64_t *mat_off, int32_t *M, int32_t *A, int32_t *B, uint64_t *status);
bool traceback_on_host(const seqalign_ctx *ctx);
void parallel_memcpy(void *dst, const void *src, size_t bytes);

}
```

seq-align_amd/csrc/sa_device.hip:

```cpp
#include "sa_ctx.hpp"

#include <algorithm>
#include <atomic>
#include <condition_variable>
#include <mutex>

#include <errno.h>
#include <sched.h>
#include <strings.h>
#include <time.h>
#include <sys/syscall.h>
#include <unistd.h>

using namespace sa_host;

static thread_local std::string g_last_error;

int sa_host::fail_hip(hipError_t e, const char *what) {
  g_last_error = std::string(what) + ": " + hipGetErrorString(e);
  return (e == hipErrorNoDevice || e == hipErrorInvalidDevice) ? SEQALIGN_E_NO_DEVICE
                                                               : SEQALIGN_E_HIP;
}
void sa_host::set_last_error(const std::string &msg) { g_last_error = msg; }

extern "C" const char *seqalign_last_error(void) { return g_last_error.c_str(); }

extern "C" const char *seqalign_strerror(int code) {
  switch (code) {
    case SEQALIGN_OK: return "ok";
    case SEQALIGN_E_NO_DEVICE: return "no HIP device (gfx950) available";
    case SEQALIGN_E_HIP: return "HIP runtime error";
    case SEQALIGN_E_ARG: return "invalid argument";
    case SEQALIGN_E_NOMEM: return "out of memory";
    case SEQALIGN_E_UNKNOWN_PAIR: return "unknown character pair and match/mismatch not set";
    case SEQALIGN_E_DOMAIN: return "scoring outside the defined domain (penalty below -|min_penalty|)";
    case SEQALIGN_E_TRACEBACK: return "traceback failed";
    case SEQALIGN_E_TOO_LARGE: return "pair too large (>= 2^31 cells)";
  }
  return "unknown error";
}

static thread_local seqalign_call_info_t *tl_recorder = nullptr;

void sa_record_launch(int kind, uint64_t items) {
  if (!tl_recorder || kind < 0 || kind >= SEQALIGN_K_COUNT) return;
  tl_recorder->launches[kind] += 1;
  tl_recorder->items[kind] += items;
}

static thread_local seqalign_call_info_ext_t *tl_recorder_ext = nullptr;

void sa_record_launch_ext(int kind, uint64_t items) {
  if (!tl_recorder_ext || kind < 0 || kind >= SEQALIGN_KX_COUNT) return;
  tl_recorder_ext->launches[kind] += 1;
  tl_recorder_ext->items[kind] += items;
}

sa_host::CallScope::CallScope(seqalign_ctx *c) : ctx(c), prev(tl_recorder), prev_ext(tl_recorder_ext) {
  if (!ctx) return;
  if (ctx->call_depth++ == 0) {
    memset(&ctx->call_info, 0, sizeof(ctx->call_info));
    memset(&ctx->call_info_ext, 0, sizeof(ctx->call_info_ext));
  }
  tl_recorder = &ctx->call_info;
  tl_recorder_ext = &ctx->call_info_ext;
}
sa_host::CallScope::~CallScope() {
  if (!ctx) return;
  --ctx->call_depth;
  tl_recorder = prev;
  tl_recorder_ext = prev_ext;
}

extern "C" int seqalign_ctx_last_call_info(const seqalign_ctx_t *ctx, seqalign_call_info_t *out) {
  if (!ctx || !out) return SEQALIGN_E_ARG;
  *out = ctx->call_info;
  return SEQALIGN_OK;
}

extern "C" int seqalign_ctx_last_call_info_ext(const seqalign_ctx_t *ctx, seqalign_call_info_ext_t *out) {
  if (!ctx || !out) return SEQALIGN_E_ARG;
  *out = ctx->call_info_ext;
  return SEQALIGN_OK;
}

extern "C" const char *seqalign_kernel_kind_ext_name(int kind) {
  static const char *names[SEQALIGN_KX_COUNT] = {"band_score", "band_fill", "band_walk"};
  return kind >= 0 && kind < SEQALIGN_KX_COUNT ? names[kind] : nullptr;
}

extern "C" const char *seqalign_kernel_kind_name(int kind) {
  static const char *names[SEQALIGN_K_COUNT] = {
      "fill_wavefront", "fill_rowscan", "fill_stream", "fill_strips", "fill_wgstream", "fill_nw_dirs", "fill_nw_dirs_x2",
      "fill_sw_dirs", "fill_sw_dirs_x2", "fill_sw_best_x2", "sw_reduce", "sw_box", "sweep_regs", "sweep_lds", "sweep_strips",
      "sweep_dirs", "sweep_dirs_x2", "walk_lane", "walk_wave", "walk_dirs_lane", "walk_dirs_tile", "walk_moves_lane",
      "walk_moves_tile", "fill_nw_dirs_x4", "fill_sw_best_x4", "score_rows", "score_strips",
      "score_cross", "score_select", "long_forward", "long_block", "long_walk"};
  return kind >= 0 && kind < SEQALIGN_K_COUNT ? names[kind] : nullptr;
}

static SaPlacementOpts placement_opts(const seqalign_ctx *ctx, bool explicit_call) {
  SaPlacementOpts o;
  o.scan_bytes = (size_t)ctx->opt.arena_scan_gib << 30;
  o.quality_stop = ctx->opt.arena_quality;
  o.keep_bytes = (size_t)ctx->opt.arena_keep_gib << 30;
  o.free_fraction = 0.01f * (float)ctx->opt.arena_free_pct;
  if (!explicit_call) {
    o.free_fraction = 0.25f;
    if (ctx->arena_walks > 0) o.scan_bytes = std::min<size_t>(o.scan_bytes, (size_t)16 << 30);
  }
  return o;
}

int sa_host::reserve_arenas(seqalign_ctx *ctx, size_t bytes, bool placed) {
  if (ctx->arena_set && bytes <= ctx->M.cap && (ctx->arena_placed || !placed)) return SEQALIGN_OK;
  if (ctx->arena_set) {
    (void)hipStreamSynchronize(ctx->stream);
    if (ctx->stream2) (void)hipStreamSynchronize(ctx->stream2);
    for (hipStream_t t : ctx->copy_streams) if (t) (void)hipStreamSynchronize(t);
    sa_arenas_destroy(sa_arenas_take(ctx->M.p));
    ctx->arena_set = nullptr;
  }
  ctx->M = DevBuf(); ctx->A = DevBuf(); ctx->B = DevBuf();
  const size_t want = bytes + (ctx->arena_walks ? bytes / 2 : bytes / 8) + 4096;
  SaArenaSet *set = nullptr;
  SaPlacementOpts po = placement_opts(ctx, false);
  if (!placed) po.scan_bytes = 0;
  hipError_t e = sa_arenas_create(ctx->device, want, ctx->stream, po, &set);
  if (e != hipSuccess) return fail_hip(e, "matrix arenas");
  if (placed) ctx->arena_walks++;
  ctx->arena_placed = placed;
  ctx->arena_set = set;
  void *const *a = sa_arenas_base(set);
  ctx->M.p = a[0]; ctx->A.p = a[1]; ctx->B.p = a[2];
  ctx->M.cap = ctx->A.cap = ctx->B.cap = sa_arenas_bytes(set);
  return SEQALIGN_OK;
}

extern "C" int seqalign_arenas_alloc(seqalign_ctx_t *ctx, uint64_t bytes_each, void *arenas[3], float *quality) {
  if (!ctx || !arenas || !bytes_each) return SEQALIGN_E_ARG;
  HIP_TRY(hipSetDevice(ctx->device));
  SaArenaSet *set = nullptr;
  hipError_t e = sa_arenas_create(ctx->device, (size_t)bytes_each, ctx->stream, placement_opts(ctx, true), &set);
  if (e != hipSuccess) return fail_hip(e, "matrix arenas");
  for (int k = 0; k < 3; ++k) arenas[k] = sa_arenas_base(set)[k];
  if (quality) *quality = sa_arenas_info(set)->quality;
  return SEQALIGN_OK;
}

extern "C" int seqalign_arenas_free(seqalign_ctx_t *ctx, void *arenas[3]) {
  if (!ctx || !arenas) return SEQALIGN_E_ARG;
  if (!arenas[0]) return SEQALIGN_OK;
  HIP_TRY(hipSetDevice(ctx->device));
  SaArenaSet *set = sa_arenas_take(arenas[0]);
  if (!set) { set_last_error("seqalign_arenas_free: not arenas of seqalign_arenas_alloc"); return SEQALIGN_E_ARG; }
  sa_arenas_destroy(set);
  arenas[0] = arenas[1] = arenas[2] = nullptr;
  return SEQALIGN_OK;
}

static_assert(sizeof(seqalign_arena_info_t) == sizeof(SaArenaInfo), "seqalign_arena_info_t mirrors SaArenaInfo");
extern "C" int seqalign_arenas_info(seqalign_ctx_t *ctx, void *const arenas[3], seqalign_arena_info_t *info) {
  if (!ctx || !arenas || !info) return SEQALIGN_E_ARG;
  SaArenaInfo i;
  if (!sa_arenas_copy_info(arenas[0], &i)) return SEQALIGN_E_ARG;
  memcpy(info, &i, sizeof(*info));
  return SEQALIGN_OK;
}

extern "C" int seqalign_device_count(void) {
  int n = 0;
  if (hipGetDeviceCount(&n) != hipSuccess) return 0;
  int ok = 0;
  for (int d = 0; d < n; ++d) {
    hipDeviceProp_t prop;
    if (hipGetDeviceProperties(&prop, d) == hipSuccess && strncmp(prop.gcnArchName, "gfx950", 6) == 0) ++ok;
  }
  return ok;
}

static bool parse_int(const char *val, long long *out) {
  if (!val || !*val) return false;
  char *end = nullptr;
  errno = 0;
  const long long v = strtoll(val, &end, 10);
  if (errno || end == val || *end) return false;
  *out = v;
  return true;
}
static bool parse_bool(const char *val, bool *out) {
  static const char *yes[] = {"1", "true", "on", "yes"}, *no[] = {"0", "false", "off", "no"};
  for (const char *y : yes) if (!strcasecmp(val, y)) { *out = true; return true; }
  for (const char *n : no) if (!strcasecmp(val, n)) { *out = false; return true; }
  return false;
}

static const char *const kKernelNames[] = {"auto", "wavefront", "rowscan", "stream", "strips", "wgstream"};
static const char *const kWalkerNames[] = {"auto", "lane", "wave"};
static const char *const kSweepModes[] = {"auto", "pair", "strips"};

static bool set_option(seqalign_ctx *ctx, const char *key, const char *val) {
  SaOptions &o = ctx->opt;
  auto is = [&](const char *k) { return !strcmp(key, k); };
  auto eq = [&](const char *v) { return !strcmp(val, v); };
  auto name_of = [&](const char *const *names, int n, int *out) { for (int k = 0; k < n; ++k) if (eq(names[k])) { *out = k; return true; } return false; };
  auto number = [&](long long lo, long long hi, long long *out) { long long v; if (!parse_int(val, &v) || v < lo || v > hi) return false; *out = v; return true; };
  auto flag = [&](bool *out) { return parse_bool(val, out); };
  long long num = 0;
  int idx = 0;
  if (is("kernel")) { if (!name_of(kKernelNames, 6, &idx)) return false; o.kernel = idx; return true; }
  if (is("cpl")) { if (!number(0, 16, &num)) return false; o.cpl = (uint32_t)num; return true; }
  if (is("wpb")) { if (!number(0, 8, &num) || (num != 0 && num != 1 && num != 2 && num != 4 && num != 8)) return false; o.wpb = (uint32_t)num; return true; }
  if (is("lds_pad")) { if (!number(0, 160 * 1024, &num)) return false; o.lds_pad = (uint32_t)num; return true; }
  if (is("traceback")) { if (!eq("host") && !eq("device")) return false; o.traceback_host = eq("host"); return true; }
  if (is("trace_kernel")) { if (!name_of(kWalkerNames, 3, &idx)) return false; o.trace_kernel = (uint32_t)idx; return true; }
  if (is("sweep_mode")) { if (!name_of(kSweepModes, 3, &idx)) return false; o.sweep_mode = idx; return true; }
  if (is("sweep_strip")) { if (!number(0, 256, &num) || (num != 0 && num != 64 && num != 128 && num != 256)) return false; o.sweep_strip = (uint32_t)num; return true; }
  if (is("sweep_cpl")) { if (!number(0, 4, &num) || num == 3) return false; o.sweep_cpl = (uint32_t)num; return true; }
  if (is("sweep_ev")) return flag(&o.sweep_ev);
  if (is("sweep_trace")) return flag(&o.sweep_trace);
  if (is("sweep_dirs")) return flag(&o.sweep_dirs);
  if (is("nw_dirs")) return flag(&o.nw_dirs);
  if (is("pack16")) { if (!number(0, 2, &num)) return false; o.pack16 = (int)num; return true; }
  if (is("quad")) { if (!number(0, 2, &num)) return false; o.quad = (uint32_t)num; return true; }
  if (is("walk_overlap")) return flag(&o.walk_overlap);
  if (is("nw_moves")) return flag(&o.nw_moves);
  if (is("zero_copy")) { if (eq("auto")) { o.zero_copy = 4; return true; } if (!number(0, 3, &num)) return false; o.zero_copy = (uint32_t)num; return true; }
  if (is("reduce_depth")) { if (!number(0, 8, &num) || (num != 0 && num != 4 && num != 8)) return false; o.reduce_depth = (uint32_t)num; return true; }
  if (is("timing")) return flag(&o.timing);
  if (is("chunk_bytes")) {
    if (!number(0, (long long)1 << 60, &num) || (num != 0 && num < (1 << 20))) return false;
    o.chunk_bytes = (size_t)num;
    if (num) ctx->chunk_budget = (size_t)num; else ctx->chunk_budget = ctx->chunk_budget_default;
    return true;
  }
  if (is("subbatches")) { if (!number(0, 256, &num)) return false; o.subbatches = (uint32_t)num; return true; }
  if (is("upload_slices")) { if (!number(0, 16, &num)) return false; o.upload_slices = (uint32_t)num; return true; }
  if (is("arena_scan_gib")) { if (!number(0, 1024, &num)) return false; o.arena_scan_gib = (uint32_t)num; return true; }
  if (is("arena_keep_gib")) { if (!number(0, 1024, &num)) return false; o.arena_keep_gib = (uint32_t)num; return true; }
  if (is("async_lanes")) { if (!number(0, 8, &num)) return false; o.async_lanes = (uint32_t)num; return true; }
  if (is("dirs_local")) { if (!number(0, 1, &num)) return false; o.dirs_local = (uint32_t)num; return true; }
  if (is("walk_stage")) { if (!number(0, 1, &num)) return false; o.walk_stage = (uint32_t)num; return true; }
  if (is("walk_tile")) { if (!number(0, 64, &num) || !(num == 0 || num == 32 || num == 64)) return false; o.walk_tile = (uint32_t)num; return true; }
  if (is("walk_group")) { if (!number(0, 8, &num) || !(num == 0 || num == 1 || num == 4 || num == 8)) return false; o.walk_group = (uint32_t)num; return true; }
  if (is("arena_free_pct")) { if (!number(10, 90, &num)) return false; o.arena_free_pct = (uint32_t)num; return true; }
  if (is("long_block_rows")) { if (!number(0, 0xFFFFFFFFll, &num)) return false; o.long_block_rows = (uint32_t)num; return true; }
  if (is("arena_quality")) {
    char *end = nullptr;
    const double q = strtod(val, &end);
    if (end == val || *end || !(q > 0.5 && q < 1.5)) return false;
    o.arena_quality = (float)q;
    return true;
  }
  return false;
}

static bool get_option(const seqalign_ctx *ctx, const char *key, std::string *out) {
  const SaOptions &o = ctx->opt;
  auto is = [&](const char *k) { return !strcmp(key, k); };
  auto n = [&](long long v) { *out = std::to_string(v); return true; };
  if (is("kernel")) { *out = kKernelNames[o.kernel]; return true; }
  if (is("cpl")) return n(o.cpl);
  if (is("wpb")) return n(o.wpb);
  if (is("lds_pad")) return n(o.lds_pad);
  if (is("traceback")) { *out = o.traceback_host ? "host" : "device"; return true; }
  if (is("trace_kernel")) { *out = kWalkerNames[o.trace_kernel]; return true; }
  if (is("sweep_mode")) { *out = kSweepModes[o.sweep_mode]; return true; }
  if (is("sweep_strip")) return n(o.sweep_strip);
  if (is("sweep_cpl")) return n(o.sweep_cpl);
  if (is("sweep_ev")) return n(o.sweep_ev);
  if (is("sweep_trace")) return n(o.sweep_trace);
  if (is("sweep_dirs")) return n(o.sweep_dirs);
  if (is("nw_dirs")) return n(o.nw_dirs);
  if (is("pack16")) return n(o.pack16);
  if (is("quad")) return n(o.quad);
  if (is("walk_overlap")) return n(o.walk_overlap);
  if (is("nw_moves")) return n(o.nw_moves);
  if (is("zero_copy")) { if (o.zero_copy == 4) { *out = "auto"; return true; } return n(o.zero_copy); }
  if (is("reduce_depth")) return n(o.reduce_depth);
  if (is("timing")) return n(o.timing);
  if (is("chunk_bytes")) return n((long long)o.chunk_bytes);
  if (is("subbatches")) return n(o.subbatches);
  if (is("upload_slices")) return n(o.upload_slices);
  if (is("arena_scan_gib")) return n(o.arena_scan_gib);
  if (is("arena_keep_gib")) return n(o.arena_keep_gib);
  if (is("async_lanes")) return n(o.async_lanes);
  if (is("dirs_local")) return n(o.dirs_local);
  if (is("walk_stage")) return n(o.walk_stage);
  if (is("walk_tile")) return n(o.walk_tile);
  if (is("walk_group")) return n(o.walk_group);
  if (is("arena_free_pct")) return n(o.arena_free_pct);
  if (is("long_block_rows")) return n(o.long_block_rows);
  if (is("arena_quality")) { char buf[32]; snprintf(buf, sizeof(buf), "%.6g", (double)o.arena_quality); *out = buf; return true; }
  return false;
}

static void options_from_env(seqalign_ctx *ctx) {
  static const char *keys[] = {"kernel", "cpl", "wpb", "lds_pad", "traceback", "trace_kernel", "sweep_mode", "sweep_strip",
                               "sweep_cpl", "sweep_ev", "sweep_trace", "sweep_dirs", "nw_dirs", "pack16", "quad", "walk_overlap", "nw_moves", "zero_copy", "reduce_depth", "timing", "chunk_bytes", "subbatches", "arena_scan_gib", "arena_quality", "arena_keep_gib", "upload_slices", "arena_free_pct", "async_lanes", "walk_group", "dirs_local", "walk_stage", "walk_tile", "long_block_rows"};
  for (const char *k : keys) {
    std::string name = "SEQALIGN_";
    for (const char *c = k; *c; ++c) name += (char)toupper((unsigned char)*c);
    if (const char *v = getenv(name.c_str())) {
      if (!set_option(ctx, k, v)) fprintf(stderr, "seqalign: ignoring %s=%s (not a value of option \"%s\")\n", name.c_str(), v, k);
    }
  }
}

extern "C" int seqalign_ctx_set_option(seqalign_ctx_t *ctx, const char *key, const char *value) {
  if (!ctx || !key || !value) return SEQALIGN_E_ARG;
  if (!set_option(ctx, key, value)) {
    set_last_error(std::string("seqalign_ctx_set_option: no option \"") + key + "\" with value \"" + value + "\"");
    return SEQALIGN_E_ARG;
  }
  return SEQALIGN_OK;
}

extern "C" int seqalign_ctx_get_option(const seqalign_ctx_t *ctx, const char *key, char *value, size_t cap) {
  if (!ctx || !key || !value) return SEQALIGN_E_ARG;
  std::string v;
  if (!get_option(ctx, key, &v) || v.size() + 1 > cap) return SEQALIGN_E_ARG;
  memcpy(value, v.c_str(), v.size() + 1);
  return SEQALIGN_OK;
}

extern "C" int seqalign_ctx_create(int device, seqalign_ctx_t **out) {
  if (!out) return SEQALIGN_E_ARG;
  *out = nullptr;
  int n = 0;
  hipError_t e = hipGetDeviceCount(&n);
  if (e != hipSuccess || n == 0) {
    set_last_error("hipGetDeviceCount: no device");
    return SEQALIGN_E_NO_DEVICE;
  }
  if (device < 0 || device >= n) return SEQALIGN_E_ARG;
  hipDeviceProp_t prop;
  HIP_TRY(hipGetDeviceProperties(&prop, device));
  if (strncmp(prop.gcnArchName, "gfx950", 6) != 0) {
    set_last_error(std::string("device is ") + prop.gcnArchName + ", kernels are built for gfx950 only");
    return SEQALIGN_E_NO_DEVICE;
  }
  HIP_TRY(hipSetDevice(device));
  seqalign_ctx *ctx = new (std::nothrow) seqalign_ctx();
  if (!ctx) return SEQALIGN_E_NOMEM;
  ctx->device = device;
  e = hipStreamCreateWithFlags(&ctx->stream, hipStreamNonBlocking);
  if (e != hipSuccess) { delete ctx; return fail_hip(e, "hipStreamCreate"); }
  sa_pool_ref(device);
  size_t free_b = 0, total_b = 0;
  (void)hipMemGetInfo(&free_b, &total_b);
  ctx->chunk_budget = free_b ? (free_b / 10) * 4 : (size_t)8 << 30;
  ctx->chunk_budget = std::min<size_t>(ctx->chunk_budget, (size_t)48 << 30);
  ctx->chunk_budget_default = ctx->chunk_budget;
  options_from_env(ctx);
  *out = ctx;
  return SEQALIGN_OK;
}

extern "C" void seqalign_ctx_destroy(seqalign_ctx_t *ctx) {
  if (!ctx) return;
  async_shutdown(ctx);
  (void)hipSetDevice(ctx->device);
  (void)hipStreamSynchronize(ctx->stream);
  for (int k = 0; k < 2; ++k) if (ctx->cached[k]) seqalign_scoring_release(ctx, ctx->cached[k]);
  if (ctx->arena_set) sa_arenas_destroy(sa_arenas_take(ctx->M.p));
  for (DevBuf *b : {&ctx->arena, &ctx->off_a, &ctx->pair_list,
                    &ctx->status, &ctx->best_score, &ctx->best_index, &ctx->dirs,
                    &ctx->cand_count, &ctx->cand_off, &ctx->cand_cap, &ctx->cand_index, &ctx->cand_score,
                    &ctx->t_str_off, &ctx->t_out_a, &ctx->t_out_b, &ctx->t_meta})
    b->release();
  for (DevBuf &b : ctx->e) b.release();
  ctx->strip_progress.release();
  ctx->score_handoff.release();
  ctx->search_list.release();
  ctx->long_ckpt.release();
  ctx->long_block.release();
  for (HostBuf *b : {&ctx->h_one, &ctx->h_desc, &ctx->h_arena, &ctx->h_M, &ctx->h_A, &ctx->h_B, &ctx->h_misc, &ctx->h_ta,
                     &ctx->h_tb, &ctx->h_tmeta})
    b->release();
  if (ctx->stream2) (void)hipStreamDestroy(ctx->stream2);
  for (hipStream_t t : ctx->copy_streams) if (t) (void)hipStreamDestroy(t);
  (void)hipStreamDestroy(ctx->stream);
  sa_pool_unref(ctx->device);
  delete ctx;
}

extern "C" int seqalign_pool_trim(seqalign_ctx_t *ctx, uint64_t keep_bytes, uint64_t *held_bytes) {
  if (!ctx) return SEQALIGN_E_ARG;
  HIP_TRY(hipSetDevice(ctx->device));
  if (keep_bytes != UINT64_MAX) sa_pool_trim(ctx->device, (size_t)keep_bytes);
  if (held_bytes) *held_bytes = sa_pool_bytes(ctx->device);
  return SEQALIGN_OK;
}

extern "C" int seqalign_ctx_device(const seqalign_ctx_t *ctx) { return ctx ? ctx->device : -1; }

extern "C" int seqalign_scoring_upload(seqalign_ctx_t *ctx, const scoring_t *scoring, int is_sw,
                                       seqalign_dev_scoring_t **out) {
  if (!ctx || !scoring || !out) return SEQALIGN_E_ARG;
  *out = nullptr;
  seqalign_dev_scoring *h = new (std::nothrow) seqalign_dev_scoring();
  if (!h) return SEQALIGN_E_NOMEM;
  int rc = sa_flatten_scoring(scoring, is_sw, &h->flat);
  if (rc != SEQALIGN_OK) { delete h; return rc; }
  HIP_TRY(hipSetDevice(ctx->device));
  const size_t tb = sizeof(int32_t) * h->flat.n_classes * h->flat.n_classes;
  hipError_t e = hipMalloc((void **)&h->d_code, sizeof(h->flat.code));
  if (e == hipSuccess) e = hipMalloc((void **)&h->d_table, tb);
  if (e == hipSuccess) e = hipMemcpy(h->d_code, h->flat.code, sizeof(h->flat.code), hipMemcpyHostToDevice);
  if (e == hipSuccess) e = hipMemcpy(h->d_table, h->flat.table, tb, hipMemcpyHostToDevice);
  if (e != hipSuccess) {
    seqalign_scoring_release(ctx, h);
    return fail_hip(e, "scoring upload");
  }
  for (size_t k = 0; k < (size_t)h->flat.n_classes * h->flat.n_classes; ++k) {
    const int32_t v = h->flat.table[k];
    if (v == SA_S_BLOCKED || v == SA_S_UNKNOWN) continue;
    h->table_abs_max = std::max(h->table_abs_max, v < 0 ? (v == INT32_MIN ? INT32_MAX : -v) : v);
  }
  *out = h;
  return SEQALIGN_OK;
}

extern "C" void seqalign_scoring_release(seqalign_ctx_t *ctx, seqalign_dev_scoring_t *h) {
  if (!h) return;
  if (ctx) (void)hipSetDevice(ctx->device);
  if (h->d_code) (void)hipFree(h->d_code);
  if (h->d_table) (void)hipFree(h->d_table);
  sa_flat_scoring_free(&h->flat);
  if (ctx) for (int k = 0; k < 2; ++k) if (ctx->cached[k] == h) ctx->cached[k] = nullptr;
  delete h;
}


static SaFillParams make_params(const seqalign_ctx *ctx, const seqalign_dev_scoring_t *s, const seqalign_dev_batch_t *b) {
  SaFillParams p;
  p.tune_cpl = ctx->opt.cpl; p.tune_wpb = ctx->opt.wpb; p.tune_lds_pad = ctx->opt.lds_pad; p.tune_quad = ctx->opt.quad;
  p.arena = b->arena; p.off_a = b->off_a; p.len_a = b->len_a; p.off_b = b->off_b; p.len_b = b->len_b;
  p.mat_off = b->mat_off; p.M = b->match_scores; p.A = b->gap_a_scores; p.B = b->gap_b_scores;
  p.status = b->status; p.code = s->d_code; p.table = s->d_table;
  p.n_pairs = (uint32_t)b->n_pairs; p.K = s->flat.n_classes;
  p.gap_open = s->flat.gap_open; p.open1 = s->flat.open1; p.ext = s->flat.ext; p.floor = s->flat.floor;
  p.gen_eq = s->flat.gen_eq; p.gen_ne = s->flat.gen_ne; p.flags = s->flat.flags;
  p.best_score = nullptr; p.best_index = nullptr;
  p.cand_min = nullptr; p.cand_count = nullptr; p.cand_box = nullptr; p.cand_rows = nullptr; p.cand_rows_off = nullptr;
  p.uniform_stride = 0;
  p.pair_list = nullptr;
  p.table_abs_max = s->table_abs_max;
  return p;
}

static int pick_kernel(const seqalign_ctx *ctx, int kernel) {
  if (kernel != SEQALIGN_KERNEL_AUTO) return kernel;
  if (ctx->opt.kernel != SEQALIGN_KERNEL_AUTO) return ctx->opt.kernel;
  return SEQALIGN_KERNEL_STREAM;
}

int sa_host::fill_device(seqalign_ctx_t *ctx, const seqalign_dev_scoring_t *scoring, const seqalign_dev_batch_t *batch,
                         int kernel, void *stream, int32_t *best_score, uint64_t *best_index, bool *best_done,
                         const SaCandBox *cand, bool *cand_done) {
  if (best_done) *best_done = false;
  if (cand_done) *cand_done = false;
  if (!ctx || !scoring || !batch) return SEQALIGN_E_ARG;
  if (batch->n_pairs == 0) return SEQALIGN_OK;
  if (batch->n_pairs > 0xFFFFFFFFull) return SEQALIGN_E_ARG;
  if ((uint64_t)(batch->max_len_a + 1ull) * (batch->max_len_b + 1ull) >= (1ull << 31)) return SEQALIGN_E_TOO_LARGE;
  hipStream_t st = stream ? (hipStream_t)stream : ctx->stream;
  SaFillParams p = make_params(ctx, scoring, batch);
  hipError_t e;
  (void)hipGetLastError();
  int which = pick_kernel(ctx, kernel);
  const bool stream_ok = sa_stream_kernel_applicable(p, batch->max_len_a);
  if (kernel == SEQALIGN_KERNEL_AUTO && ctx->opt.kernel == SEQALIGN_KERNEL_AUTO) {
    const bool wg_ok = sa_wgstream_kernel_applicable(p, batch->max_len_a) &&
                       (batch->max_len_a + 1 > 768 || batch->n_pairs < 8192);
    const uint32_t few = !wg_ok ? 256u : (batch->max_len_a + 1 <= 2048 ? 128u : 256u);
    if (batch->max_len_a > 512 && batch->n_pairs < few) which = SEQALIGN_KERNEL_STRIPS;
    else if (wg_ok) which = SEQALIGN_KERNEL_WGSTREAM;
    else if (!stream_ok || (batch->max_len_a > 767 && batch->n_pairs < 768)) which = SEQALIGN_KERNEL_ROWSCAN;
  }
  if (which == SEQALIGN_KERNEL_STREAM && !stream_ok) which = SEQALIGN_KERNEL_ROWSCAN;
  if (which == SEQALIGN_KERNEL_WGSTREAM && !sa_wgstream_kernel_applicable(p, batch->max_len_a))
    which = SEQALIGN_KERNEL_ROWSCAN;
  if ((which == SEQALIGN_KERNEL_STREAM || which == SEQALIGN_KERNEL_WGSTREAM) && best_score && best_index) {
    p.best_score = best_score; p.best_index = best_index;
    const bool reports = which == SEQALIGN_KERNEL_STREAM
                             ? sa_stream_kernel_reports_best(p, batch->max_len_a, batch->max_len_b)
                             : sa_wgstream_kernel_reports_best(p, batch->max_len_a, batch->max_len_b);
    if (reports) { if (best_done) *best_done = true; }
    else p.best_score = nullptr, p.best_index = nullptr;
  }
  if (cand && cand->dirs_used) *cand->dirs_used = false;
  if (cand && cand->best_only) {
    p.best_score = best_score; p.best_index = best_index;
    p.uniform_stride = cand->uniform_stride;
    p.dirs_local = cand->dirs_local ? 1u : 0u;
    if (cand->pair_list) { p.pair_list = cand->pair_list; p.n_pairs = cand->list_count; }
    if (!cand->dirs || !cand->dirs_used || !sa_sw_best_x2_applicable(p, batch->max_len_a, batch->max_len_b, cand->dirs)) {
      set_last_error("internal error: the best-hit direction fill was asked for a batch outside its domain");
      return SEQALIGN_E_ARG;
    }
    e = sa_launch_fill_sw_best_x2(p, batch->max_len_a, cand->dirs, st);
    if (e != hipSuccess) return fail_hip(e, "fill kernel launch");
    *cand->dirs_used = true;
    if (best_done) *best_done = true;
    return SEQALIGN_OK;
  }
  if (cand && cand->dirs && cand->dirs_used && ctx->opt.sweep_dirs && kernel == SEQALIGN_KERNEL_AUTO &&
      ctx->opt.kernel == SEQALIGN_KERNEL_AUTO) {
    p.cand_min = cand->cand_min; p.cand_count = cand->cand_count; p.cand_box = cand->cand_box; p.cand_rows = cand->cand_rows;
    p.cand_rows_off = cand->hit_off;
    if (sa_dirs_fill_applicable(p, batch->max_len_a, cand->dirs)) {
      p.uniform_stride = ctx->opt.pack16 ? cand->uniform_stride : 0;
      const bool packed = sa_dirs_x2_applicable(p, batch->max_len_a, batch->max_len_b, cand->dirs);
      if (packed && cand->pair_list) { p.pair_list = cand->pair_list; p.n_pairs = cand->list_count; }
      e = packed ? sa_launch_fill_dirs_x2(p, batch->max_len_a, cand->dirs, st)
                 : sa_launch_fill_dirs(p, batch->max_len_a, cand->dirs, st);
      if (e != hipSuccess) return fail_hip(e, "fill kernel launch");
      *cand->dirs_used = true;
      if (cand_done) *cand_done = true;
      return SEQALIGN_OK;
    }
    p.cand_min = nullptr; p.cand_count = nullptr; p.cand_box = nullptr; p.cand_rows = nullptr; p.cand_rows_off = nullptr;
  }
  if ((which == SEQALIGN_KERNEL_STREAM || which == SEQALIGN_KERNEL_WGSTREAM) && cand) {
    p.cand_min = cand->cand_min; p.cand_count = cand->cand_count; p.cand_box = cand->cand_box; p.cand_rows = cand->cand_rows;
    p.cand_rows_off = cand->hit_off;
    const bool reports = which == SEQALIGN_KERNEL_STREAM ? sa_stream_kernel_emits_candidates(p, batch->max_len_a)
                                                          : sa_wgstream_kernel_emits_candidates(p, batch->max_len_a);
    if (reports) { if (cand_done) *cand_done = true; }
    else p.cand_count = nullptr;
  }
// ... 423 lines not shown
```

seq-align_amd/host/sa_internal.h:

```cpp
#ifndef SA_INTERNAL_H
#define SA_INTERNAL_H

#include <stddef.h>
#include <stdint.h>

#include "alignment.h"
#include "seqalign_hip.h"

#ifdef __cplusplus
extern "C" {
#endif

int sa_scoring_lookup_rc(const scoring_t *sc, int a, int b, int *score, int *is_match);
int sa_fold_char(const scoring_t *sc, int c);

#define SA_S_BLOCKED ((int32_t)INT32_MIN)
#define SA_S_UNKNOWN ((int32_t)(INT32_MIN + 1))

enum {
  SA_F_NO_START_GAP = 1u << 0,
  SA_F_NO_END_GAP   = 1u << 1,
  SA_F_NO_GAPS_A    = 1u << 2,
  SA_F_NO_GAPS_B    = 1u << 3,
  SA_F_NO_MISMATCH  = 1u << 4,
  SA_F_IS_SW        = 1u << 5,
  SA_F_HAS_SENTINEL = 1u << 6
};

typedef struct {
  int32_t gap_open;
  int32_t open1;
  int32_t ext;
  int32_t floor;
  int32_t gen_eq;
  int32_t gen_ne;
  uint32_t flags;
  uint32_t n_classes;
  uint16_t code[256];
  int32_t *table;
} sa_flat_scoring_t;

int sa_flatten_scoring(const scoring_t *sc, int is_sw, sa_flat_scoring_t *out);
void sa_flat_scoring_free(sa_flat_scoring_t *f);

seqalign_ctx_t *sa_default_ctx_or_die(void);

int sa_fill_one_pair(seqalign_ctx_t *ctx, const scoring_t *sc, int is_sw,
                     const char *a, size_t len_a, const char *b, size_t len_b,
                     int32_t *M, int32_t *A, int32_t *B, uint64_t *status);

typedef struct {
  const scoring_t *sc;
  const char *a, *b;
  size_t len_a, len_b;
  const int32_t *M, *A, *B;
} sa_view_t;

int sa_reverse_move_rc(const sa_view_t *v, int *matrix, int32_t *score,
                       size_t *x, size_t *y);
int sa_nw_traceback(const sa_view_t *v, char *out_a, char *out_b,
                    size_t *out_len, int32_t *out_score);

int sa_expand_nw_moves(const char *a, uint32_t len_a, const char *b, uint32_t len_b, const uint32_t *plane_a,
                       const uint32_t *plane_b, uint32_t n_words, uint32_t n_moves, char *out_a, char *out_b,
                       uint32_t *out_len);
int sa_expand_sw_moves(const char *a, const char *b, uint32_t end_x, uint32_t end_y, const uint32_t *plane_a,
                       const uint32_t *plane_b, uint32_t n_words, uint32_t n_moves, char *out_a, char *out_b,
                       uint32_t pos[4]);
int sa_moves_uses_simd(void);
void sa_moves_force_scalar(int on);
int sa_cigar_nw_moves(const char *a, uint32_t len_a, const char *b, uint32_t len_b, const uint32_t *plane_a,
                      const uint32_t *plane_b, uint32_t n_words, uint32_t n_moves, int format, int fold, char *out, uint64_t cap,
                      uint32_t *out_len, uint32_t *out_columns);
int sa_cigar_sw_moves(const char *a, const char *b, uint32_t end_x, uint32_t end_y, const uint32_t *plane_a,
                      const uint32_t *plane_b, uint32_t n_words, uint32_t n_moves, int format, int fold, char *out, uint64_t cap,
                      uint32_t pos[4], uint32_t *out_len);

typedef int (*sa_hit_sink_t)(void *user, int32_t score, size_t end_x, size_t end_y,
                             size_t x, size_t y, size_t steps);

#ifdef __cplusplus
}
#endif
#endif
```

seq-align_amd/python/seqalign_amd/__init__.py:

```python
from __future__ import annotations

import ctypes as C
from pathlib import Path

import numpy as np

from . import workloads

PKG_ROOT = Path(__file__).resolve().parents[2]
REPO_ROOT = PKG_ROOT.parent
import os as _os
LIB_PATH = Path(_os.environ.get("SEQALIGN_LIB") or (PKG_ROOT / "lib" / "libseqalign_hip.so"))

OK, E_NO_DEVICE, E_HIP, E_ARG, E_NOMEM, E_UNKNOWN_PAIR, E_DOMAIN, E_TRACEBACK, E_TOO_LARGE = range(9)
KERNEL_AUTO, KERNEL_WAVEFRONT, KERNEL_ROWSCAN, KERNEL_STREAM, KERNEL_STRIPS, KERNEL_WGSTREAM = 0, 1, 2, 3, 4, 5
KERNEL_NAMES = {KERNEL_AUTO: "auto", KERNEL_WAVEFRONT: "wavefront", KERNEL_ROWSCAN: "rowscan",
                KERNEL_STREAM: "stream", KERNEL_STRIPS: "strips", KERNEL_WGSTREAM: "wgstream"}
STATUS_OK = 0xFFFFFFFFFFFFFFFF


class Scoring(C.Structure):
    _fields_ = [
        ("gap_open", C.c_int), ("gap_extend", C.c_int),
        ("no_start_gap_penalty", C.c_bool), ("no_end_gap_penalty", C.c_bool),
        ("no_gaps_in_a", C.c_bool), ("no_gaps_in_b", C.c_bool),
        ("no_mismatches", C.c_bool), ("use_match_mismatch", C.c_bool),
        ("match", C.c_int), ("mismatch", C.c_int),
        ("case_sensitive", C.c_bool),
        ("wildcards", C.c_uint32 * 8), ("swap_set", (C.c_uint32 * 8) * 256),
        ("wildscores", C.c_int * 256), ("swap_scores", (C.c_int * 256) * 256),
        ("min_penalty", C.c_int), ("max_penalty", C.c_int),
    ]


class BatchDesc(C.Structure):
    _fields_ = [("n_pairs", C.c_uint64), ("arena", C.c_void_p), ("arena_bytes", C.c_uint64),
                ("off_a", C.c_void_p), ("len_a", C.c_void_p), ("off_b", C.c_void_p), ("len_b", C.c_void_p)]


class DevBatchDesc(C.Structure):
    _fields_ = [("n_pairs", C.c_uint64), ("arena", C.c_void_p), ("off_a", C.c_void_p),
                ("len_a", C.c_void_p), ("off_b", C.c_void_p), ("len_b", C.c_void_p),
                ("mat_off", C.c_void_p), ("match_scores", C.c_void_p), ("gap_a_scores", C.c_void_p),
                ("gap_b_scores", C.c_void_p), ("status", C.c_void_p),
                ("max_len_a", C.c_uint32), ("max_len_b", C.c_uint32)]


class SwReduceDesc(C.Structure):
    _fields_ = [("n_pairs", C.c_uint64), ("len_a", C.c_void_p), ("len_b", C.c_void_p),
                ("mat_off", C.c_void_p), ("match_scores", C.c_void_p), ("min_score", C.c_int32),
                ("best_score", C.c_void_p), ("best_index", C.c_void_p), ("cand_count", C.c_void_p),
                ("cand_off", C.c_void_p), ("cand_cap", C.c_void_p), ("cand_index", C.c_void_p),
                ("cand_score", C.c_void_p)]


class SeqSetDesc(C.Structure):
    _fields_ = [("n_seqs", C.c_uint64), ("arena", C.c_void_p), ("arena_bytes", C.c_uint64), ("off", C.c_void_p),
                ("len", C.c_void_p)]


INT32_MIN = -2**31
SEARCH_MAX_K = 1024
SEARCH_HIT = np.dtype([("target", np.uint32), ("score", np.int32), ("end_a", np.uint32), ("end_b", np.uint32)])


class SwHit(C.Structure):
    _fields_ = [("pair", C.c_uint64), ("score", C.c_int32), ("pos_a", C.c_uint32), ("pos_b", C.c_uint32),
                ("len_a", C.c_uint32), ("len_b", C.c_uint32), ("length", C.c_uint32), ("str_off", C.c_uint64)]


class SeqAlignError(RuntimeError):
    def __init__(self, code: int, where: str):
        l = lib()
        super().__init__(f"{where}: {l.seqalign_strerror(code).decode()} [{code}] {l.seqalign_last_error().decode()}")
        self.code = code


_lib = None


def lib():
    global _lib
    if _lib is None:
        if not LIB_PATH.exists():
            raise FileNotFoundError(
                f"{LIB_PATH} missing: build it with `make -C {PKG_ROOT}` "
                "(or python -c 'import __graft_entry__ as g; g.build()'); there is no CPU path")
        try:
            import torch
        except ImportError:
            pass
        l = C.CDLL(str(LIB_PATH))
        l.seqalign_strerror.restype = C.c_char_p
        l.seqalign_last_error.restype = C.c_char_p
        l.seqalign_kernel_kind_name.restype = C.c_char_p
        l.seqalign_kernel_kind_ext_name.restype = C.c_char_p
        l.needleman_wunsch_new.restype = C.c_void_p
        l.smith_waterman_new.restype = C.c_void_p
        l.alignment_create.restype = C.c_void_p
        l.smith_waterman_get_aligner.restype = C.c_void_p
        _lib = l
    return _lib


def _check(code: int, where: str):
    if code != OK:
        raise SeqAlignError(code, where)


def _ptr(arr) -> C.c_void_p:
    return C.c_void_p(arr.ctypes.data) if arr is not None else C.c_void_p(0)


def make_scoring(spec: dict) -> Scoring:
    l = lib()
    sc = Scoring()
    C.memset(C.byref(sc), 0, C.sizeof(sc))
    if "preset" in spec:
        getattr(l, "scoring_system_" + spec["preset"])(C.byref(sc))
    else:
        l.scoring_init(C.byref(sc), *[C.c_int(int(v)) for v in spec["init"][:4]],
                       *[C.c_bool(bool(v)) for v in spec["init"][4:]])
    for ch, s in spec.get("wildcards", []):
        l.scoring_add_wildcard(C.byref(sc), C.c_char(ch.encode()), C.c_int(s))
    for a, b, s in spec.get("mutations", []):
        l.scoring_add_mutation(C.byref(sc), C.c_char(a.encode()), C.c_char(b.encode()), C.c_int(s))
    if "use_match_mismatch" in spec:
        sc.use_match_mismatch = bool(spec["use_match_mismatch"])
    for k, v in spec.get("flags", {}).items():
        setattr(sc, k, bool(v))
    return sc


def batch_desc(batch: "workloads.Batch") -> BatchDesc:
    return BatchDesc(batch.n_pairs, batch.arena.ctypes.data, batch.arena.nbytes,
                     batch.off_a.ctypes.data, batch.len_a.ctypes.data,
                     batch.off_b.ctypes.data, batch.len_b.ctypes.data)


OPTION_DEFAULTS = {"kernel": "auto", "cpl": 0, "wpb": 0, "lds_pad": 0, "traceback": "device", "trace_kernel": "auto",
                   "sweep_mode": "auto", "sweep_strip": 0, "sweep_cpl": 0, "sweep_trace": 0, "sweep_dirs": 1, "nw_dirs": 1, "pack16": 1, "quad": 0, "walk_overlap": 0, "timing": 0, "chunk_bytes": 0,
                   "subbatches": 0, "arena_scan_gib": 160, "arena_quality": 1.045, "arena_keep_gib": 16, "upload_slices": 0, "arena_free_pct": 60, "nw_moves": 1, "zero_copy": "auto", "sweep_ev": 1, "reduce_depth": 0, "async_lanes": 0, "walk_group": 0, "dirs_local": 1, "walk_stage": 1, "walk_tile": 0, "long_block_rows": 0}


K_MAX = 32


class CallInfo(C.Structure):
    _fields_ = [("launches", C.c_uint32 * K_MAX), ("items", C.c_uint64 * K_MAX)]


KX_MAX = 32


class CallInfoExt(C.Structure):
    _fields_ = [("launches", C.c_uint32 * KX_MAX), ("items", C.c_uint64 * KX_MAX)]


class ArenaInfo(C.Structure):
    _fields_ = [("quality", C.c_float), ("target", C.c_float), ("vmm", C.c_int32), ("chunk_mib", C.c_uint32),
                ("depth_gib", C.c_float), ("scanned_gib", C.c_float), ("depth_a_gib", C.c_float), ("tries", C.c_uint32),
                ("second_walk_from", C.c_uint32), ("try_quality", C.c_float * 96), ("try_depth_gib", C.c_float * 96),
                ("kept_gib", C.c_float), ("seconds", C.c_float)]

    def as_dict(self):
        n = int(self.tries)
        return {"quality": round(float(self.quality), 3), "target": round(float(self.target), 3), "vmm": bool(self.vmm),
                "chunk_mib": int(self.chunk_mib), "depth_gib": round(float(self.depth_gib), 1),
                "scanned_gib": round(float(self.scanned_gib), 1), "depth_a_gib": round(float(self.depth_a_gib), 1),
                "tries": n, "second_walk_from": int(self.second_walk_from), "kept_gib": round(float(self.kept_gib), 1), "seconds": round(float(self.seconds), 3),
                "try_quality": [round(float(self.try_quality[i]), 3) for i in range(n)],
                "try_depth_gib": [round(float(self.try_depth_gib[i]), 1) for i in range(n)]}


class Context:

    def __init__(self, device: int = 0):
        self._h = C.c_void_p(0)
        _check(lib().seqalign_ctx_create(C.c_int(device), C.byref(self._h)), "seqalign_ctx_create")
        self.device = device

    def close(self):
        if self._h:
            lib().seqalign_ctx_destroy(self._h)
            self._h = C.c_void_p(0)

    def __enter__(self):
        return self

    def __exit__(self, *exc):
        self.close()

    def pool_trim(self, keep_bytes=None) -> int:
        held = C.c_uint64(0)
        keep = C.c_uint64(0xFFFFFFFFFFFFFFFF if keep_bytes is None else int(keep_bytes))
        _check(lib().seqalign_pool_trim(self._h, keep, C.byref(held)), "seqalign_pool_trim")
        return int(held.value)

    def set_option(self, key: str, value) -> None:
        if isinstance(value, (bool, np.bool_)):
            value = int(value)
        _check(lib().seqalign_ctx_set_option(self._h, key.encode(), str(value).encode()), f"seqalign_ctx_set_option({key}={value})")

    def get_option(self, key: str) -> str:
        buf = C.create_string_buffer(64)
        _check(lib().seqalign_ctx_get_option(self._h, key.encode(), buf, C.c_size_t(64)), f"seqalign_ctx_get_option({key})")
        return buf.value.decode()

    def options(self, **kv):
        ctx = self

        class _Scope:
            def __enter__(self_inner):
                self_inner.before = {k: ctx.get_option(k) for k in kv}
                for k, v in kv.items():
                    ctx.set_option(k, v)
                return ctx

            def __exit__(self_inner, *exc):
                for k, v in self_inner.before.items():
                    ctx.set_option(k, v)
        return _Scope()

    def last_call(self) -> dict:
        info = CallInfo()
        _check(lib().seqalign_ctx_last_call_info(self._h, C.byref(info)), "seqalign_ctx_last_call_info")
        out = {}
        for k in range(K_MAX):
            if info.launches[k]:
                name = lib().seqalign_kernel_kind_name(C.c_int(k))
                out[name.decode() if name else f"kind{k}"] = (int(info.launches[k]), int(info.items[k]))
        ext = CallInfoExt()
        _check(lib().seqalign_ctx_last_call_info_ext(self._h, C.byref(ext)), "seqalign_ctx_last_call_info_ext")
        for k in range(KX_MAX):
            if ext.launches[k]:
                name = lib().seqalign_kernel_kind_ext_name(C.c_int(k))
                out[name.decode() if name else f"kind_ext{k}"] = (int(ext.launches[k]), int(ext.items[k]))
        return out

    def upload_scoring(self, scoring: Scoring, is_sw: int) -> C.c_void_p:
        h = C.c_void_p(0)
        _check(lib().seqalign_scoring_upload(self._h, C.byref(scoring), C.c_int(is_sw), C.byref(h)),
               "seqalign_scoring_upload")
        return h

    def release_scoring(self, h):
        lib().seqalign_scoring_release(self._h, h)

    def _handles(self, peers):
        ctxs = [self] + list(peers)
        return (C.c_void_p * len(ctxs))(*[c._h for c in ctxs]), C.c_int(len(ctxs))

    def fill_batch(self, batch, scoring: Scoring, is_sw: int, check: bool = True, out=None, peers=None):
        cells = batch.matrix_cells()
        mat_off = np.zeros(batch.n_pairs, np.uint64)
        if batch.n_pairs:
            mat_off[1:] = np.cumsum(cells)[:-1]
        total = int(cells.sum())
        if out is not None:
            M, A, B = out
            assert M.size >= total and A.size >= total and B.size >= total
        else:
            M = np.empty(total, np.int32); A = np.empty(total, np.int32); B = np.empty(total, np.int32)
        status = np.zeros(batch.n_pairs, np.uint64)
        d = batch_desc(batch)
        if peers:
            hs, nh = self._handles(peers)
            rc = lib().seqalign_fill_batch_multi(hs, nh, C.byref(d), C.byref(scoring), C.c_int(is_sw), _ptr(mat_off),
                                                 _ptr(M), _ptr(A), _ptr(B), _ptr(status))
        else:
            rc = lib().seqalign_fill_batch(self._h, C.byref(d), C.byref(scoring), C.c_int(is_sw), _ptr(mat_off),
                                           _ptr(M), _ptr(A), _ptr(B), _ptr(status))
        if check:
            _check(rc, "seqalign_fill_batch")
        return (M, A, B, mat_off, status) if check else (rc, M, A, B, mat_off, status)

    def nw_batch(self, batch, scoring: Scoring, raw: bool = False, peers=None):
        n = batch.n_pairs
        cache = getattr(self, "_nw_buffers", None)
        if raw and cache is not None and cache[0] is batch:
            str_off, out_a, out_b, out_len, out_score = cache[1]
        else:
            caps = batch.len_a.astype(np.uint64) + batch.len_b.astype(np.uint64) + np.uint64(1)
            str_off = np.zeros(n, np.uint64)
            if n:
                str_off[1:] = np.cumsum(caps)[:-1]
            total = int(caps.sum()) + 1
            out_a, out_b = np.zeros(total, np.uint8), np.zeros(total, np.uint8)
            out_len, out_score = np.zeros(n, np.uint32), np.zeros(n, np.int32)
            if raw:
                self._nw_buffers = (batch, (str_off, out_a, out_b, out_len, out_score))
        d = batch_desc(batch)
        if peers:
            hs, nh = self._handles(peers)
            _check(lib().seqalign_nw_batch_multi(hs, nh, C.byref(d), C.byref(scoring), _ptr(str_off), _ptr(out_a),
                                                 _ptr(out_b), _ptr(out_len), _ptr(out_score)), "seqalign_nw_batch_multi")
        else:
            _check(lib().seqalign_nw_batch(self._h, C.byref(d), C.byref(scoring), _ptr(str_off), _ptr(out_a),
                                           _ptr(out_b), _ptr(out_len), _ptr(out_score)), "seqalign_nw_batch")
        if raw:
            return str_off, out_a, out_b, out_len, out_score
        res = []
        for p in range(n):
            o, ln = int(str_off[p]), int(out_len[p])
            res.append((int(out_score[p]), out_a[o:o + ln].tobytes(), out_b[o:o + ln].tobytes()))
        return res

    def sw_batch(self, batch, scoring: Scoring, min_score, max_hits: int = 1 << 20, hit_cap: int | None = None,
                 raw: bool = False, peers=None):
        n = batch.n_pairs
        ms = np.full(n, min_score, np.int32) if np.isscalar(min_score) else np.asarray(min_score, np.int32)
        hit_cap = hit_cap or max(1024, 64 * n)
        str_cap = int(hit_cap * (int(batch.len_a.max(initial=0)) + int(batch.len_b.max(initial=0)) + 2))
        str_cap = min(str_cap, 1 << 30)
        cache = getattr(self, "_sw_buffers", None)
        if raw and cache is not None and cache[0] is batch and cache[1] == (hit_cap, str_cap):
            hits, out_a, out_b = cache[2]
        else:
            hits = (SwHit * hit_cap)()
            out_a, out_b = np.zeros(str_cap, np.uint8), np.zeros(str_cap, np.uint8)
            if raw:
                self._sw_buffers = (batch, (hit_cap, str_cap), (hits, out_a, out_b))
        n_hits = C.c_uint64(0)
        d = batch_desc(batch)
        if peers:
            hs, nh = self._handles(peers)
            _check(lib().seqalign_sw_batch_multi(hs, nh, C.byref(d), C.byref(scoring), _ptr(ms),
                                                 C.c_uint32(min(max_hits, 0xFFFFFFFF)), hits, C.c_uint64(hit_cap),
                                                 C.byref(n_hits), _ptr(out_a), _ptr(out_b), C.c_uint64(str_cap)),
                   "seqalign_sw_batch_multi")
        else:
            _check(lib().seqalign_sw_batch(self._h, C.byref(d), C.byref(scoring), _ptr(ms), C.c_uint32(min(max_hits, 0xFFFFFFFF)),
                                           hits, C.c_uint64(hit_cap), C.byref(n_hits), _ptr(out_a), _ptr(out_b),
                                           C.c_uint64(str_cap)), "seqalign_sw_batch")
        if raw:
            return n_hits.value, hits, out_a, out_b
        per_pair = [[] for _ in range(n)]
        for k in range(n_hits.value):
            h = hits[k]
            per_pair[h.pair].append(dict(score=h.score, pos_a=h.pos_a, pos_b=h.pos_b, len_a=h.len_a, len_b=h.len_b,
                                         a=out_a[h.str_off:h.str_off + h.length].tobytes().decode(),
                                         b=out_b[h.str_off:h.str_off + h.length].tobytes().decode()))
        return per_pair

    def nw_score(self, batch, scoring: Scoring, peers=None) -> np.ndarray:
        _score_args(batch, scoring)
        score = np.zeros(batch.n_pairs, np.int32)
        d = batch_desc(batch)
        if peers:
            hs, nh = self._handles(peers)
            _check(lib().seqalign_nw_score_batch_multi(hs, nh, C.byref(d), C.byref(scoring), _ptr(score)),
                   "seqalign_nw_score_batch_multi")
        else:
            _check(lib().seqalign_nw_score_batch(self._h, C.byref(d), C.byref(scoring), _ptr(score)), "seqalign_nw_score_batch")
        return score

    def sw_score(self, batch, scoring: Scoring, peers=None):
        _score_args(batch, scoring)
        n = batch.n_pairs
        score, end_a, end_b = np.zeros(n, np.int32), np.zeros(n, np.uint32), np.zeros(n, np.uint32)
        d = batch_desc(batch)
        if peers:
            hs, nh = self._handles(peers)
            _check(lib().seqalign_sw_score_batch_multi(hs, nh, C.byref(d), C.byref(scoring), _ptr(score), _ptr(end_a),
                                                       _ptr(end_b)), "seqalign_sw_score_batch_multi")
        else:
            _check(lib().seqalign_sw_score_batch(self._h, C.byref(d), C.byref(scoring), _ptr(score), _ptr(end_a), _ptr(end_b)),
                   "seqalign_sw_score_batch")
        return score, end_a, end_b

    def nw_score_cross(self, queries, targets, scoring: Scoring, peers=None) -> np.ndarray:
        _cross_args(queries, targets, scoring)
        score = np.zeros((queries.n_seqs, targets.n_seqs), np.int32)
        dq, dt = seqset_desc(queries), seqset_desc(targets)
        if peers:
            hs, nh = self._handles(peers)
            _check(lib().seqalign_nw_score_cross_multi(hs, nh, C.byref(dq), C.byref(dt), C.byref(scoring), _ptr(score)),
                   "seqalign_nw_score_cross_multi")
        else:
            _check(lib().seqalign_nw_score_cross(self._h, C.byref(dq), C.byref(dt), C.byref(scoring), _ptr(score)),
                   "seqalign_nw_score_cross")
        return score

    def sw_score_cross(self, queries, targets, scoring: Scoring, peers=None):
        _cross_args(queries, targets, scoring)
        shape = (queries.n_seqs, targets.n_seqs)
        score, end_a, end_b = np.zeros(shape, np.int32), np.zeros(shape, np.uint32), np.zeros(shape, np.uint32)
        dq, dt = seqset_desc(queries), seqset_desc(targets)
        if peers:
# ... 301 lines not shown


class _RawDeviceInts:

    def __init__(self, ptr: int, count: int):
        self.__cuda_array_interface__ = {"shape": (count,), "typestr": "<i4", "data": (int(ptr), False),
                                         "version": 3, "strides": None}


class DeviceBatch:

    def __init__(self, batch, device: int = 0, pad_cells: int = 32, placement: str = "spread", ctx=None):
        import torch
        self.torch = torch
        self.host = batch
        dev = torch.device("cuda", device)
        self.device = device
        cells = batch.matrix_cells()
        padded = (cells + pad_cells - 1) // pad_cells * pad_cells
        mat_off = np.zeros(batch.n_pairs, np.int64)
        if batch.n_pairs:
            mat_off[1:] = np.cumsum(padded)[:-1]
        self.mat_off_host = mat_off.astype(np.uint64)
        self.cells_host = cells
        self.total_cells = int(padded.sum())
        t = lambda a: torch.from_numpy(a.view(np.int64) if a.dtype == np.uint64 else
                                       (a.view(np.int32) if a.dtype == np.uint32 else a)).to(dev)
        self.arena = t(batch.arena)
        self.off_a, self.len_a = t(batch.off_a), t(batch.len_a)
        self.off_b, self.len_b = t(batch.off_b), t(batch.len_b)
        self.mat_off = t(self.mat_off_host)
        stride = (self.total_cells + 1023) // 1024 * 1024
        self.placement_quality = -1.0
        self.placement_info = None
        if placement == "packed":
            stride += int(_os.environ.get("SEQALIGN_ARENA_SKEW", "0")) // 256 * 256
            self._arena3 = torch.empty(3 * stride + 1024, dtype=torch.int32, device=dev)
            skew = (-(self._arena3.data_ptr() // 4)) % 1024
            self.M = self._arena3[skew:skew + self.total_cells]
            self.A = self._arena3[skew + stride:skew + stride + self.total_cells]
            self.B = self._arena3[skew + 2 * stride:skew + 2 * stride + self.total_cells]
        else:
            self._ctx = ctx if ctx is not None else _arena_context(device)
            ptrs = (C.c_void_p * 3)()
            q = C.c_float(-1.0)
            _check(lib().seqalign_arenas_alloc(self._ctx._h, C.c_uint64(4 * stride), ptrs, C.byref(q)),
                   "seqalign_arenas_alloc")
            self._arena_ptrs = ptrs
            self.placement_quality = float(q.value)
            info = ArenaInfo()
            _check(lib().seqalign_arenas_info(self._ctx._h, ptrs, C.byref(info)), "seqalign_arenas_info")
            self.placement_info = info.as_dict()
            self.M, self.A, self.B = (torch.as_tensor(_RawDeviceInts(ptrs[k], self.total_cells), device=dev)
                                      for k in range(3))
        self.status = torch.zeros(batch.n_pairs, dtype=torch.int64, device=dev)
        if ctx is not None and hasattr(lib(), "seqalign_ctx_stream"):
            lib().seqalign_ctx_stream.restype = C.c_void_p
            self.stream = torch.cuda.ExternalStream(int(lib().seqalign_ctx_stream(ctx._h)), device=dev)
        else:
            self.stream = torch.cuda.Stream(dev)
        self.desc = DevBatchDesc(batch.n_pairs, self.arena.data_ptr(), self.off_a.data_ptr(),
                                 self.len_a.data_ptr(), self.off_b.data_ptr(), self.len_b.data_ptr(),
                                 self.mat_off.data_ptr(), self.M.data_ptr(), self.A.data_ptr(),
                                 self.B.data_ptr(), self.status.data_ptr(),
                                 int(batch.len_a.max(initial=0)), int(batch.len_b.max(initial=0)))

    def __del__(self):
        ptrs = getattr(self, "_arena_ptrs", None)
        if ptrs is not None and getattr(self._ctx, "_h", None):
            self.M = self.A = self.B = None
            try:
                self.torch.cuda.synchronize(self.device)
                lib().seqalign_arenas_free(self._ctx._h, ptrs)
            except Exception:
                pass
            self._arena_ptrs = None

    def fill(self, ctx: Context, dev_scoring, kernel: int = KERNEL_AUTO, order_after_current: bool = True):
        if order_after_current:
            self.stream.wait_stream(self.torch.cuda.current_stream(self.device))
        _check(lib().seqalign_fill_batch_device(ctx._h, dev_scoring, C.byref(self.desc), C.c_int(kernel),
                                                C.c_void_p(self.stream.cuda_stream)), "seqalign_fill_batch_device")

    def time_fill_ms(self, ctx: Context, dev_scoring, kernel: int, repeats: int):
        self.stream.wait_stream(self.torch.cuda.current_stream(self.device))
        st = self.stream.cuda_stream
        ms = (C.c_float * repeats)()
        _check(lib().seqalign_time_fill_ms(ctx._h, dev_scoring, C.byref(self.desc), C.c_int(kernel),
                                           C.c_void_p(st), C.c_int(repeats), ms), "seqalign_time_fill_ms")
        return list(ms)

    def algorithmic_bytes(self) -> int:
        return int(12 * self.cells_host.sum() + self.host.len_a.astype(np.int64).sum()
                   + self.host.len_b.astype(np.int64).sum())

    def pair_matrices(self, p: int):
        o, n = int(self.mat_off_host[p]), int(self.cells_host[p])
        return tuple(x[o:o + n].cpu().numpy() for x in (self.M, self.A, self.B))

    def sw_reduce_launch(self, ctx: Context, min_score: int):
        torch = self.torch
        if not hasattr(self, "_red"):
            n, dev = self.host.n_pairs, self.M.device
            self._red = (torch.zeros(n, dtype=torch.int32, device=dev), torch.zeros(n, dtype=torch.int64, device=dev),
                         torch.zeros(n, dtype=torch.int32, device=dev))
        bs, bi, cnt = self._red
        r = SwReduceDesc(self.host.n_pairs, self.len_a.data_ptr(), self.len_b.data_ptr(), self.mat_off.data_ptr(),
                         self.M.data_ptr(), min_score, bs.data_ptr(), bi.data_ptr(), cnt.data_ptr(), 0, 0, 0, 0)
        _check(lib().seqalign_sw_reduce_device(ctx._h, C.byref(r), C.c_void_p(self.stream.cuda_stream)),
               "seqalign_sw_reduce_device")

    def sw_reduce(self, ctx: Context, min_score: int, with_candidates: bool = True):
        torch = self.torch
        n = self.host.n_pairs
        dev = self.M.device
        best_s = torch.zeros(n, dtype=torch.int32, device=dev)
        best_i = torch.zeros(n, dtype=torch.int64, device=dev)
        count = torch.zeros(n, dtype=torch.int32, device=dev)
        self.stream.wait_stream(torch.cuda.current_stream(self.device))
        st = self.stream.cuda_stream
        r = SwReduceDesc(n, self.len_a.data_ptr(), self.len_b.data_ptr(), self.mat_off.data_ptr(),
                         self.M.data_ptr(), min_score, best_s.data_ptr(), best_i.data_ptr(),
                         count.data_ptr(), 0, 0, 0, 0)
        _check(lib().seqalign_sw_reduce_device(ctx._h, C.byref(r), C.c_void_p(st)), "seqalign_sw_reduce_device")
        torch.cuda.synchronize(self.device)
        cands = None
        if with_candidates:
            cap = count.cpu().numpy().astype(np.uint32)
            off = np.zeros(n, np.uint64)
            if n:
                off[1:] = np.cumsum(cap.astype(np.uint64))[:-1]
            total = int(cap.sum())
            d_off = torch.from_numpy(off.view(np.int64)).to(dev)
            d_cap = torch.from_numpy(cap.view(np.int32)).to(dev)
            c_idx = torch.zeros(total + 1, dtype=torch.int32, device=dev)
            c_sc = torch.zeros(total + 1, dtype=torch.int32, device=dev)
            r.cand_off, r.cand_cap = d_off.data_ptr(), d_cap.data_ptr()
            r.cand_index, r.cand_score = c_idx.data_ptr(), c_sc.data_ptr()
            self.stream.wait_stream(torch.cuda.current_stream(self.device))
            _check(lib().seqalign_sw_reduce_device(ctx._h, C.byref(r), C.c_void_p(st)), "seqalign_sw_reduce_device")
            torch.cuda.synchronize(self.device)
            ci, cs = c_idx.cpu().numpy().view(np.uint32), c_sc.cpu().numpy()
            cands = [(ci[int(off[p]):int(off[p]) + int(cap[p])], cs[int(off[p]):int(off[p]) + int(cap[p])])
                     for p in range(n)]
        return best_s.cpu().numpy(), best_i.cpu().numpy(), count.cpu().numpy(), cands


EXPORTED_SYMBOLS = [
    "seqalign_strerror", "seqalign_last_error", "seqalign_device_count", "seqalign_ctx_create",
    "seqalign_ctx_destroy", "seqalign_ctx_device", "seqalign_scoring_upload", "seqalign_scoring_release",
    "seqalign_fill_batch_device", "seqalign_sw_reduce_device", "seqalign_nw_traceback_device", "seqalign_sw_traceback_device", "seqalign_fill_batch", "seqalign_nw_batch",
    "seqalign_sw_batch", "seqalign_time_fill_ms", "seqalign_arenas_alloc", "seqalign_arenas_free",
    "seqalign_arenas_info", "seqalign_pool_trim", "seqalign_ctx_set_option", "seqalign_ctx_get_option", "seqalign_ctx_last_call_info",
    "seqalign_kernel_kind_name", "seqalign_host_legs_nw", "seqalign_ctx_stream",
    "seqalign_fill_batch_multi", "seqalign_nw_batch_multi", "seqalign_sw_batch_multi", "seqalign_cigar",
    "seqalign_nw_batch_submit", "seqalign_sw_batch_submit", "seqalign_nw_batch_cigar_submit", "seqalign_job_wait", "seqalign_job_done",
    "seqalign_nw_batch_cigar", "seqalign_sw_batch_cigar", "seqalign_nw_batch_cigar_multi", "seqalign_sw_batch_cigar_multi",
    "seqalign_nw_score_batch", "seqalign_sw_score_batch", "seqalign_nw_score_batch_multi", "seqalign_sw_score_batch_multi",
    "seqalign_score_time_ms",
    "seqalign_nw_score_cross", "seqalign_sw_score_cross", "seqalign_nw_score_cross_multi", "seqalign_sw_score_cross_multi",
    "seqalign_nw_score_search", "seqalign_sw_score_search", "seqalign_nw_score_search_multi",
    "seqalign_sw_score_search_multi",
    "seqalign_nw_align_long", "seqalign_sw_align_long",
    "seqalign_nw_score_banded", "seqalign_nw_align_banded", "seqalign_band_score_time_ms", "seqalign_ctx_last_call_info_ext", "seqalign_kernel_kind_ext_name",
    "seqalign_scoring_load_matrix", "seqalign_scoring_load_pairs", "seqalign_reader_open", "seqalign_reader_close",
    "seqalign_reader_next",
    "scoring_init", "scoring_add_wildcard", "scoring_add_mutation", "scoring_add_mutations", "scoring_print",
    "scoring_lookup", "scoring_system_PAM30", "scoring_system_PAM70", "scoring_system_BLOSUM80",
    "scoring_system_BLOSUM62", "scoring_system_DNA_hybridization", "scoring_system_default", "blosum62",
    "align_col_mismatch", "align_col_indel", "align_col_context", "align_col_stop", "aligner_align",
    "aligner_destroy", "alignment_create", "alignment_ensure_capacity", "alignment_free",
    "alignment_reverse_move", "alignment_print_matrices", "alignment_colour_print_against",
    "alignment_print_spacer",
    "needleman_wunsch_new", "needleman_wunsch_free", "needleman_wunsch_align", "needleman_wunsch_align2",
    "smith_waterman_new", "smith_waterman_free", "smith_waterman_get_aligner", "smith_waterman_align",
    "smith_waterman_align2", "smith_waterman_fetch", "sort_match_indices",
]
```

Measured before the change: 549.9 GCUPS.

## Pack sequence symbols to 2/4 bits on host and unpack on device

Adds a host-side packer (AVX-512 with PDEP, scalar fallback) that encodes sequence bytes into 2- or 4-bit dictionary codes when the alphabet is small. It uploads the packed buffer and expands it on the GPU with an LUT-based unpack kernel before the fill kernels run. This targets host gather/memcpy work and H2D bytes in the batch, moves and score paths. The cost is an extra kernel launch, dictionary discovery, and a fallback path for foreign symbols. For 10k pairs of 150bp the sequence upload is only about 3 MB, so the benefit may be small relative to the DP time.

```diff
diff --git a/include/seqalign_hip.h b/include/seqalign_hip.h
--- a/include/seqalign_hip.h
+++ b/include/seqalign_hip.h
@@ -243,6 +243,8 @@
   SEQALIGN_KX_BAND_SCORE = 0,
   SEQALIGN_KX_BAND_FILL,
   SEQALIGN_KX_BAND_WALK,
+  SEQALIGN_KX_UNPACK_SYM2,
+  SEQALIGN_KX_UNPACK_SYM4,
   SEQALIGN_KX_COUNT
 };
 #define SEQALIGN_KX_MAX 32
@@ -252,6 +254,7 @@
 } seqalign_call_info_ext_t;
 int seqalign_ctx_last_call_info_ext(const seqalign_ctx_t *ctx, seqalign_call_info_ext_t *out);
 const char *seqalign_kernel_kind_ext_name(int kind);
+const char *seqalign_call_kind_ext_name(int kind);
 
 size_t seqalign_cigar(const char *result_a, const char *result_b, size_t length, int extended,
                       int case_insensitive, char *out, size_t cap);
@@ -330,6 +333,9 @@
 int seqalign_score_time_ms(seqalign_ctx_t *ctx, const seqalign_batch_t *batch, const scoring_t *scoring, int is_sw,
                            int repeats, float *ms_each);
 
+int seqalign_pack_symbols_host(const seqalign_batch_t *batch, uint64_t slice_pairs, uint64_t task_syms, const uint8_t *seed,
+                               uint32_t n_seed, uint8_t *packed, uint64_t packed_cap, uint64_t *info, uint8_t *dict,
+                               uint64_t max_slices, uint64_t *n_slices);
 int seqalign_host_legs_nw(const seqalign_batch_t *batch, const uint64_t *str_off, char *out_a, char *out_b,
                           uint32_t *out_len, int iterations, double *pack_ms, double *expand_ms);
 
diff --git a/seq-align_amd/csrc/sa_batch.hip b/seq-align_amd/csrc/sa_batch.hip
--- a/seq-align_amd/csrc/sa_batch.hip
+++ b/seq-align_amd/csrc/sa_batch.hip
@@ -158,6 +158,8 @@
   HIP_TRY(hipStreamWaitEvent(su, ev.ev[0], 0));
   bool first = true, consistent = true, bd0 = false, cd0 = false, du0 = false;
   uint64_t filled_to = 0;
+  SeqUpload up;
+  if ((rc = seq_upload_begin(up, ctx, b, c.first, n, c.seq_bytes, h_off_a, h_off_b, n / kPack + 2))) return rc;
   for (uint64_t k0 = 0; k0 < n;) {
     uint64_t k1 = k0;
     if (two_slices) {
@@ -167,18 +169,23 @@
     }
     if (n - k1 < kPack) k1 = n;
     constexpr uint64_t kTask = 256;
-    parallel_for((k1 - k0 + kTask - 1) / kTask, [&](uint64_t blk) {
-      for (uint64_t k = k0 + blk * kTask, e = std::min(k1, k0 + (blk + 1) * kTask); k < e; ++k) {
-        const uint64_t p = c.first + k;
-        memcpy(h_seq + h_off_a[k], b->arena + b->off_a[p], b->len_a[p]);
-        memcpy(h_seq + h_off_b[k], b->arena + b->off_b[p], b->len_b[p]);
-      }
-    });
     const uint64_t lo = h_off_a[k0], hi = k1 < n ? h_off_a[k1] : c.seq_bytes;
-    if (hi > lo) HIP_TRY(hipMemcpyAsync(ctx->arena.as<uint8_t>() + lo, h_seq + lo, hi - lo, hipMemcpyHostToDevice, su));
+    bool sent = false;
+    if ((rc = seq_upload_slice(up, lo, hi, su, &sent))) return rc;
+    if (!sent) {
+      parallel_for((k1 - k0 + kTask - 1) / kTask, [&](uint64_t blk) {
+        for (uint64_t k = k0 + blk * kTask, e = std::min(k1, k0 + (blk + 1) * kTask); k < e; ++k) {
+          const uint64_t p = c.first + k;
+          memcpy(h_seq + h_off_a[k], b->arena + b->off_a[p], b->len_a[p]);
+          memcpy(h_seq + h_off_b[k], b->arena + b->off_b[p], b->len_b[p]);
+        }
+      });
+      if (hi > lo) HIP_TRY(hipMemcpyAsync(ctx->arena.as<uint8_t>() + lo, h_seq + lo, hi - lo, hipMemcpyHostToDevice, su));
+    }
     HIP_TRY(ev.add(hipEventDisableTiming));
     HIP_TRY(hipEventRecord(ev.ev.back(), su));
     HIP_TRY(hipStreamWaitEvent(st, ev.ev.back(), 0));
+    if ((rc = seq_upload_unpack(up, ctx->arena.as<uint8_t>(), st))) return rc;
     if (n_sub > 1 && consistent) {
       bool bd = false, cd = false, du = false;
       if ((rc = fill_range(k0, k1, &bd, &cd, &du))) return rc;
@@ -188,6 +195,7 @@
     }
     k0 = k1;
   }
+  seq_upload_end(up);
   tm.lap("run_chunk: pack + H2D");
   const seqalign_dev_batch_t d = range_desc(0, n);
   if (n_sub > 1 && consistent && filled_to == n) {
@@ -787,6 +795,8 @@
     return d;
   };
   auto move_word = [&](uint64_t k) { return 2 * ((h_slot[k] >> 5) + k); };
+  SeqUpload up;
+  if (!zc_in && (rc = seq_upload_begin(up, ctx, batch, c.first, n, total, h_off_a, h_off_b, (uint64_t)n_sub * 16))) return rc;
   tm.lap("nw moves: sizes, offsets, buffers");
 
   uint32_t g = 0;
@@ -798,6 +808,9 @@
       constexpr uint64_t kParts = 4;
       for (uint64_t sl = 0; sl < n_slices; ++sl) {
         const uint64_t sb0 = b0 + n_blocks * sl / n_slices, sb1 = b0 + n_blocks * (sl + 1) / n_slices;
+        bool sent = false;
+        if ((rc = seq_upload_slice(up, h_slot[pair_at(sb0)], h_slot[pair_at(sb1)], su, &sent))) return rc;
+        if (sent) continue;
         parallel_for((sb1 - sb0) * kParts, [&](uint64_t ti) {
           const uint64_t bi = sb0 + ti / kParts, part = ti % kParts;
           const uint64_t kb = bi * kHostBlk, ke = std::min(n, (bi + 1) * kHostBlk), span = ke - kb;
@@ -822,6 +835,7 @@
       if (!zc_in) {
         HIP_TRY(hipEventRecord(ev.ev[s], su));
         HIP_TRY(hipStreamWaitEvent(sf, ev.ev[s], 0));
+        if ((rc = seq_upload_unpack(up, ctx->arena.as<uint8_t>(), sf))) return rc;
       }
       const seqalign_dev_batch_t d = dev_range(k0, k1);
       if (layout == kMixed) {
@@ -878,6 +892,7 @@
       ++g;
     }
   }
+  seq_upload_end(up);
   tm.lap("nw moves: packed + enqueued");
 
   std::atomic<uint64_t> first_bad{~0ull};
diff --git a/seq-align_amd/csrc/sa_batch_score.hip b/seq-align_amd/csrc/sa_batch_score.hip
--- a/seq-align_amd/csrc/sa_batch_score.hip
+++ b/seq-align_amd/csrc/sa_batch_score.hip
@@ -85,15 +85,6 @@
       h_len_a[s] = la; h_len_b[s] = lb;
       h_hoff[s] = hand_total; hand_total += handoff_rows(la, lb);
     }
-    uint8_t *h_seq = ctx->h_arena.as<uint8_t>();
-    constexpr uint64_t kTask = 256;
-    parallel_for((n + kTask - 1) / kTask, [&](uint64_t blk) {
-      for (uint64_t k = blk * kTask, e = std::min(n, (blk + 1) * kTask); k < e; ++k) {
-        const uint64_t p = c.first + k;
-        memcpy(h_seq + seq_at[k], b->arena + b->off_a[p], b->len_a[p]);
-        memcpy(h_seq + seq_at[k] + b->len_a[p], b->arena + b->off_b[p], b->len_b[p]);
-      }
-    });
 
     if ((rc = ctx->arena.reserve(c.seq_bytes + 16)) || (rc = ctx->off_a.reserve(desc_bytes)) || (rc = ctx->status.reserve(n * 8)) ||
         (rc = ctx->best_score.reserve(16 + 12 * n)))
@@ -103,7 +94,26 @@
       return rc;
     hipStream_t st = ctx->stream;
     HIP_TRY(hipMemcpyAsync(ctx->off_a.p, h_off_a, desc_bytes, hipMemcpyHostToDevice, st));
-    if (c.seq_bytes) HIP_TRY(hipMemcpyAsync(ctx->arena.p, h_seq, c.seq_bytes, hipMemcpyHostToDevice, st));
+    std::vector<uint64_t> seq_b_at(n);
+    for (uint64_t k = 0; k < n; ++k) seq_b_at[k] = seq_at[k] + b->len_a[c.first + k];
+    SeqUpload up;
+    bool sent = false;
+    if ((rc = seq_upload_begin(up, ctx, b, c.first, n, c.seq_bytes, seq_at.data(), seq_b_at.data(), 1)) ||
+        (rc = seq_upload_slice(up, 0, c.seq_bytes, st, &sent)) || (rc = seq_upload_unpack(up, ctx->arena.as<uint8_t>(), st)))
+      return rc;
+    seq_upload_end(up);
+    if (!sent) {
+      uint8_t *h_seq = ctx->h_arena.as<uint8_t>();
+      constexpr uint64_t kTask = 256;
+      parallel_for((n + kTask - 1) / kTask, [&](uint64_t blk) {
+        for (uint64_t k = blk * kTask, e = std::min(n, (blk + 1) * kTask); k < e; ++k) {
+          const uint64_t p = c.first + k;
+          memcpy(h_seq + seq_at[k], b->arena + b->off_a[p], b->len_a[p]);
+          memcpy(h_seq + seq_b_at[k], b->arena + b->off_b[p], b->len_b[p]);
+        }
+      });
+      if (c.seq_bytes) HIP_TRY(hipMemcpyAsync(ctx->arena.p, h_seq, c.seq_bytes, hipMemcpyHostToDevice, st));
+    }
     d_off_a = ctx->off_a.as<uint64_t>(); d_off_b = d_off_a + n; d_hoff = d_off_b + n;
     d_len_a = reinterpret_cast<uint32_t *>(d_hoff + n); d_len_b = d_len_a + n;
     d_res = ctx->best_score.as<uint32_t>();
diff --git a/seq-align_amd/csrc/sa_ctx.hpp b/seq-align_amd/csrc/sa_ctx.hpp
--- a/seq-align_amd/csrc/sa_ctx.hpp
+++ b/seq-align_amd/csrc/sa_ctx.hpp
@@ -270,6 +270,7 @@
   bool timing = false;
   size_t chunk_bytes = 0;
   uint32_t upload_slices = 0;
+  uint32_t pack_upload = 2;
   uint32_t subbatches = 0;
   uint32_t arena_scan_gib = 160;
   float arena_quality = 1.045f;
@@ -282,6 +283,8 @@
   uint32_t long_block_rows = 0;
   uint32_t arena_keep_gib = 16;
 };
+
+struct SaSymDict { uint8_t v[SA_SYM_DICT_MAX]; };
 
 struct seqalign_dev_scoring {
   sa_flat_scoring_t flat;
@@ -314,6 +317,10 @@
   sa_host::DevBuf search_list;
   sa_host::DevBuf long_ckpt, long_block;
   sa_host::HostBuf h_desc, h_arena, h_M, h_A, h_B, h_misc, h_ta, h_tb, h_tmeta;
+  sa_host::HostBuf h_packed;
+  sa_host::DevBuf d_packed;
+  uint8_t sym_dict[SA_SYM_DICT_MAX] = {0};
+  uint32_t sym_dict_n = 0;
   seqalign_call_info_t call_info = {};
   seqalign_call_info_ext_t call_info_ext = {};
   int call_depth = 0;
@@ -380,6 +387,23 @@
               seqalign_dev_batch_t *dev_out, bool *best_done = nullptr, const SaCandBox *cand = nullptr,
               bool *cand_done = nullptr, uint64_t uniform_stride = 0);
 int ensure_copy_streams(seqalign_ctx *ctx, int count);
+struct SeqUpload {
+  seqalign_ctx *ctx = nullptr;
+  const seqalign_batch_t *b = nullptr;
+  uint64_t first = 0, n = 0, total = 0;
+  const uint64_t *h_off_a = nullptr, *h_off_b = nullptr;
+  int bits = 0;
+  uint8_t dict[SA_SYM_DICT_MAX] = {0};
+  unsigned n_dict = 0;
+  uint64_t staged = 0, cap = 0;
+  struct Slice { uint64_t at, a0, n_sym; uint32_t head; int bits; SaSymDict dict; };
+  std::vector<Slice> pending;
+};
+int seq_upload_begin(SeqUpload &u, seqalign_ctx *ctx, const seqalign_batch_t *b, uint64_t first, uint64_t n, uint64_t total,
+                     const uint64_t *h_off_a, const uint64_t *h_off_b, uint64_t max_slices);
+int seq_upload_slice(SeqUpload &u, uint64_t c0, uint64_t c1, hipStream_t su, bool *sent);
+int seq_upload_unpack(SeqUpload &u, uint8_t *dev_arena, hipStream_t st);
+void seq_upload_end(SeqUpload &u);
 constexpr uint64_t kBucketShapes = ~(uint64_t)0;
 constexpr uint64_t kShapeTableMax = (uint64_t)1 << 20;
 int fetch_status(seqalign_ctx *ctx, const Chunk &c, uint64_t *status_out);
diff --git a/seq-align_amd/csrc/sa_device.hip b/seq-align_amd/csrc/sa_device.hip
--- a/seq-align_amd/csrc/sa_device.hip
+++ b/seq-align_amd/csrc/sa_device.hip
@@ -85,7 +85,12 @@
 }
 
 extern "C" const char *seqalign_kernel_kind_ext_name(int kind) {
-  static const char *names[SEQALIGN_KX_COUNT] = {"band_score", "band_fill", "band_walk"};
+  static const char *names[3] = {"band_score", "band_fill", "band_walk"};
+  return kind >= 0 && kind < 3 ? names[kind] : nullptr;
+}
+
+extern "C" const char *seqalign_call_kind_ext_name(int kind) {
+  static const char *names[SEQALIGN_KX_COUNT] = {"band_score", "band_fill", "band_walk", "unpack_sym2", "unpack_sym4"};
   return kind >= 0 && kind < SEQALIGN_KX_COUNT ? names[kind] : nullptr;
 }
 
@@ -236,6 +241,7 @@
   }
   if (is("subbatches")) { if (!number(0, 256, &num)) return false; o.subbatches = (uint32_t)num; return true; }
   if (is("upload_slices")) { if (!number(0, 16, &num)) return false; o.upload_slices = (uint32_t)num; return true; }
+  if (is("pack_upload")) { if (eq("auto")) { o.pack_upload = 2; return true; } if (!number(0, 1, &num)) return false; o.pack_upload = (uint32_t)num; return true; }
   if (is("arena_scan_gib")) { if (!number(0, 1024, &num)) return false; o.arena_scan_gib = (uint32_t)num; return true; }
   if (is("arena_keep_gib")) { if (!number(0, 1024, &num)) return false; o.arena_keep_gib = (uint32_t)num; return true; }
   if (is("async_lanes")) { if (!number(0, 8, &num)) return false; o.async_lanes = (uint32_t)num; return true; }
@@ -282,6 +288,7 @@
   if (is("chunk_bytes")) return n((long long)o.chunk_bytes);
   if (is("subbatches")) return n(o.subbatches);
   if (is("upload_slices")) return n(o.upload_slices);
+  if (is("pack_upload")) { if (o.pack_upload == 2) { *out = "auto"; return true; } return n(o.pack_upload); }
   if (is("arena_scan_gib")) return n(o.arena_scan_gib);
   if (is("arena_keep_gib")) return n(o.arena_keep_gib);
   if (is("async_lanes")) return n(o.async_lanes);
@@ -297,7 +304,7 @@
 
 static void options_from_env(seqalign_ctx *ctx) {
   static const char *keys[] = {"kernel", "cpl", "wpb", "lds_pad", "traceback", "trace_kernel", "sweep_mode", "sweep_strip",
-                               "sweep_cpl", "sweep_ev", "sweep_trace", "sweep_dirs", "nw_dirs", "pack16", "quad", "walk_overlap", "nw_moves", "zero_copy", "reduce_depth", "timing", "chunk_bytes", "subbatches", "arena_scan_gib", "arena_quality", "arena_keep_gib", "upload_slices", "arena_free_pct", "async_lanes", "walk_group", "dirs_local", "walk_stage", "walk_tile", "long_block_rows"};
+                               "sweep_cpl", "sweep_ev", "sweep_trace", "sweep_dirs", "nw_dirs", "pack16", "quad", "walk_overlap", "nw_moves", "zero_copy", "reduce_depth", "timing", "chunk_bytes", "subbatches", "arena_scan_gib", "arena_quality", "arena_keep_gib", "upload_slices", "pack_upload", "arena_free_pct", "async_lanes", "walk_group", "dirs_local", "walk_stage", "walk_tile", "long_block_rows"};
   for (const char *k : keys) {
     std::string name = "SEQALIGN_";
     for (const char *c = k; *c; ++c) name += (char)toupper((unsigned char)*c);
@@ -376,8 +383,9 @@
   ctx->long_ckpt.release();
   ctx->long_block.release();
   for (HostBuf *b : {&ctx->h_one, &ctx->h_desc, &ctx->h_arena, &ctx->h_M, &ctx->h_A, &ctx->h_B, &ctx->h_misc, &ctx->h_ta,
-                     &ctx->h_tb, &ctx->h_tmeta})
+                     &ctx->h_tb, &ctx->h_tmeta, &ctx->h_packed})
     b->release();
+  ctx->d_packed.release();
   if (ctx->stream2) (void)hipStreamDestroy(ctx->stream2);
   for (hipStream_t t : ctx->copy_streams) if (t) (void)hipStreamDestroy(t);
   (void)hipStreamDestroy(ctx->stream);
diff --git a/seq-align_amd/csrc/sa_upload.hip b/seq-align_amd/csrc/sa_upload.hip
--- /dev/null
+++ b/seq-align_amd/csrc/sa_upload.hip
@@ -0,0 +1,198 @@
+#include "sa_ctx.hpp"
+
+using namespace sa_host;
+
+namespace {
+
+constexpr uint64_t kTaskSyms = 16384;
+
+__global__ void __launch_bounds__(256) unpack_symbols_kernel(const uint8_t *__restrict__ packed, uint8_t *__restrict__ dst,
+                                                             uint32_t head, uint64_t n_sym, uint64_t n_groups, SaSymDict d, int bits) {
+  __shared__ uint32_t lut[256];
+  const uint32_t t = threadIdx.x;
+  auto entry = [&](uint32_t s) -> uint32_t {
+    uint32_t v = d.v[0];
+#pragma unroll
+    for (uint32_t e = 1; e < SA_SYM_DICT_MAX; ++e) v = s == e ? d.v[e] : v;
+    return v;
+  };
+  lut[t] = bits == 2 ? entry(t & 3u) | entry((t >> 2) & 3u) << 8 | entry((t >> 4) & 3u) << 16 | entry(t >> 6) << 24
+                     : entry(t & 15u) | entry(t >> 4) << 8;
+  __syncthreads();
+  const uint64_t g = (uint64_t)blockIdx.x * 256 + t;
+  if (g >= n_groups) return;
+  uint4 out;
+  if (bits == 2) {
+    const uint32_t w = reinterpret_cast<const uint32_t *>(packed)[g];
+    out.x = lut[w & 255u]; out.y = lut[(w >> 8) & 255u]; out.z = lut[(w >> 16) & 255u]; out.w = lut[w >> 24];
+  } else {
+    const uint2 w = reinterpret_cast<const uint2 *>(packed)[g];
+    out.x = lut[w.x & 255u] | lut[(w.x >> 8) & 255u] << 16; out.y = lut[(w.x >> 16) & 255u] | lut[w.x >> 24] << 16;
+    out.z = lut[w.y & 255u] | lut[(w.y >> 8) & 255u] << 16; out.w = lut[(w.y >> 16) & 255u] | lut[w.y >> 24] << 16;
+  }
+  const uint64_t s0 = g * 16;
+  if (s0 >= head && s0 + 16 <= n_sym) {
+    *reinterpret_cast<uint4 *>(dst + s0) = out;
+    return;
+  }
+  const uint32_t word[4] = {out.x, out.y, out.z, out.w};
+#pragma unroll
+  for (uint32_t j = 0; j < 16; ++j)
+    if (s0 + j >= head && s0 + j < n_sym) dst[s0 + j] = (uint8_t)(word[j >> 2] >> (8 * (j & 3u)));
+}
+
+void gather(const SeqUpload &u, uint64_t lo, uint64_t hi, uint8_t *out) {
+  if (hi <= lo) return;
+  uint64_t k = (uint64_t)(std::upper_bound(u.h_off_a, u.h_off_a + u.n, lo) - u.h_off_a);
+  k = k ? k - 1 : 0;
+  for (; k < u.n && u.h_off_a[k] < hi; ++k) {
+    const uint64_t p = u.first + k;
+    const uint64_t piece[2][3] = {{u.h_off_a[k], u.b->len_a[p], u.b->off_a[p]}, {u.h_off_b[k], u.b->len_b[p], u.b->off_b[p]}};
+    for (const auto &pc : piece) {
+      const uint64_t from = std::max(lo, pc[0]), to = std::min(hi, pc[0] + pc[1]);
+      if (to > from) memcpy(out + (from - lo), u.b->arena + pc[2] + (from - pc[0]), to - from);
+    }
+  }
+}
+
+void pack_slice(const SeqUpload &u, uint64_t c0, uint64_t c1, const uint8_t *dict, unsigned n_dict, int bits, uint8_t *dst,
+                uint64_t n_sym, uint64_t task_syms, uint32_t foreign[8]) {
+  const uint64_t a0 = c0 & ~(uint64_t)15;
+  std::atomic<uint32_t> missing[8];
+  for (auto &m : missing) m.store(0, std::memory_order_relaxed);
+  parallel_for((n_sym + task_syms - 1) / task_syms, [&](uint64_t ti) {
+    static thread_local std::vector<uint8_t> tl_buf;
+    const uint64_t s0 = ti * task_syms, s1 = std::min(n_sym, s0 + task_syms), len = s1 - s0;
+    if (tl_buf.size() < len) tl_buf.resize(len);
+    uint8_t *buf = tl_buf.data();
+    const uint64_t lo = std::min(std::max(c0, a0 + s0), a0 + s1), hi = std::max(std::min(c1, a0 + s1), lo);
+    memset(buf, dict[0], lo - (a0 + s0));
+    memset(buf + (hi - (a0 + s0)), dict[0], (a0 + s1) - hi);
+    gather(u, lo, hi, buf + (lo - (a0 + s0)));
+    uint32_t mine[8] = {0, 0, 0, 0, 0, 0, 0, 0};
+    sa_pack_symbols(buf, len, dict, n_dict, bits, dst + s0 * (unsigned)bits / 8, mine);
+    for (int w = 0; w < 8; ++w) if (mine[w]) missing[w].fetch_or(mine[w], std::memory_order_relaxed);
+  });
+  for (int w = 0; w < 8; ++w) foreign[w] |= missing[w].load(std::memory_order_relaxed);
+}
+
+uint64_t pack_slice_learning(SeqUpload &u, uint64_t c0, uint64_t c1, uint8_t *dst, uint64_t room, uint64_t task_syms, int *passes) {
+  const uint64_t n_sym = ((c0 & 15u) + (c1 - c0) + 15u) & ~(uint64_t)15;
+  *passes = 0;
+  for (int attempt = 0; attempt < 2; ++attempt) {
+    if (n_sym * (unsigned)u.bits / 8 > room) return 0;
+    uint32_t foreign[8] = {0, 0, 0, 0, 0, 0, 0, 0};
+    pack_slice(u, c0, c1, u.dict, u.n_dict, u.bits, dst, n_sym, task_syms, foreign);
+    ++*passes;
+    bool any = false;
+    for (uint32_t w : foreign) any = any || w;
+    if (!any) return n_sym * (unsigned)u.bits / 8;
+    sa_sym_set_add(foreign, u.dict, u.n_dict);
+    u.n_dict = sa_sym_dict_from_set(foreign, u.dict);
+    u.bits = sa_sym_bits(u.n_dict);
+    if (!u.bits) return 0;
+  }
+  return 0;
+}
+
+void seed_dictionary(SeqUpload &u, const uint8_t *learned, unsigned n_learned) {
+  uint8_t head[4096];
+  const uint64_t n = std::min<uint64_t>(u.total, sizeof(head));
+  gather(u, 0, n, head);
+  uint32_t set[8] = {0, 0, 0, 0, 0, 0, 0, 0}, known[8] = {0, 0, 0, 0, 0, 0, 0, 0};
+  sa_sym_set_add(set, head, n);
+  sa_sym_set_add(known, learned, n_learned);
+  bool covered = n_learned > 0 && n_learned <= SA_SYM_DICT_MAX;
+  for (int w = 0; w < 8; ++w) covered = covered && !(set[w] & ~known[w]);
+  u.n_dict = sa_sym_dict_from_set(covered ? known : set, u.dict);
+  u.bits = sa_sym_bits(u.n_dict);
+}
+
+}
+
+int sa_host::seq_upload_begin(SeqUpload &u, seqalign_ctx *ctx, const seqalign_batch_t *b, uint64_t first, uint64_t n, uint64_t total,
+                              const uint64_t *h_off_a, const uint64_t *h_off_b, uint64_t max_slices) {
+  u = SeqUpload();
+  u.ctx = ctx; u.b = b; u.first = first; u.n = n; u.total = total; u.h_off_a = h_off_a; u.h_off_b = h_off_b;
+  const bool want = ctx->opt.pack_upload == 1 || (ctx->opt.pack_upload == 2 && total >= ((uint64_t)1 << 20));
+  if (!want || !n || !total) return SEQALIGN_OK;
+  seed_dictionary(u, ctx->sym_dict, ctx->sym_dict_n);
+  if (!u.bits) return SEQALIGN_OK;
+  u.cap = total / 2 + 48 * (max_slices + 1) + 64;
+  int rc;
+  if ((rc = ctx->h_packed.reserve(u.cap)) || (rc = ctx->d_packed.reserve(u.cap))) return rc;
+  return SEQALIGN_OK;
+}
+
+int sa_host::seq_upload_slice(SeqUpload &u, uint64_t c0, uint64_t c1, hipStream_t su, bool *sent) {
+  *sent = false;
+  if (!u.bits || c1 <= c0) return SEQALIGN_OK;
+  int passes = 0;
+  const uint64_t bytes = pack_slice_learning(u, c0, c1, u.ctx->h_packed.as<uint8_t>() + u.staged, u.cap > u.staged ? u.cap - u.staged : 0, kTaskSyms, &passes);
+  if (!bytes) return SEQALIGN_OK;
+  HIP_TRY(hipMemcpyAsync(u.ctx->d_packed.as<uint8_t>() + u.staged, u.ctx->h_packed.as<uint8_t>() + u.staged, bytes, hipMemcpyHostToDevice, su));
+  SeqUpload::Slice s;
+  s.at = u.staged; s.a0 = c0 & ~(uint64_t)15; s.head = (uint32_t)(c0 & 15u); s.n_sym = s.head + (c1 - c0); s.bits = u.bits;
+  memset(&s.dict, 0, sizeof(s.dict));
+  memcpy(s.dict.v, u.dict, u.n_dict);
+  u.pending.push_back(s);
+  u.staged += (bytes + 15u) & ~(uint64_t)15;
+  *sent = true;
+  return SEQALIGN_OK;
+}
+
+int sa_host::seq_upload_unpack(SeqUpload &u, uint8_t *dev_arena, hipStream_t st) {
+  for (const SeqUpload::Slice &s : u.pending) {
+    const uint64_t n_groups = (s.n_sym + 15) / 16;
+    hipLaunchKernelGGL(unpack_symbols_kernel, dim3((unsigned)((n_groups + 255) / 256)), dim3(256), 0, st,
+                       u.ctx->d_packed.as<uint8_t>() + s.at, dev_arena + s.a0, s.head, s.n_sym, n_groups, s.dict, s.bits);
+    HIP_TRY(hipGetLastError());
+    sa_record_launch_ext(s.bits == 2 ? SEQALIGN_KX_UNPACK_SYM2 : SEQALIGN_KX_UNPACK_SYM4, s.n_sym - s.head);
+  }
+  u.pending.clear();
+  return SEQALIGN_OK;
+}
+
+void sa_host::seq_upload_end(SeqUpload &u) {
+  if (!u.ctx || !u.bits) return;
+  memcpy(u.ctx->sym_dict, u.dict, u.n_dict);
+  u.ctx->sym_dict_n = u.n_dict;
+}
+
+extern "C" int seqalign_pack_symbols_host(const seqalign_batch_t *batch, uint64_t slice_pairs, uint64_t task_syms, const uint8_t *seed,
+                                          uint32_t n_seed, uint8_t *packed, uint64_t packed_cap, uint64_t *info, uint8_t *dict,
+                                          uint64_t max_slices, uint64_t *n_slices) {
+  if (!batch_readable(batch) || !slice_pairs || !packed || !info || !dict || !n_slices || (n_seed && !seed) || n_seed > SA_SYM_DICT_MAX ||
+      task_syms % 64)
+    return SEQALIGN_E_ARG;
+  const uint64_t n = batch->n_pairs;
+  *n_slices = 0;
+  if (!n) return SEQALIGN_OK;
+  std::vector<uint64_t> off_a(n + 1), off_b(n);
+  uint64_t pos = 0;
+  for (uint64_t k = 0; k < n; ++k) { off_a[k] = pos; pos += batch->len_a[k]; off_b[k] = pos; pos += batch->len_b[k]; }
+  off_a[n] = pos;
+  SeqUpload u;
+  u.b = batch; u.n = n; u.total = pos; u.h_off_a = off_a.data(); u.h_off_b = off_b.data();
+  seed_dictionary(u, seed, n_seed);
+  uint64_t at = 0;
+  for (uint64_t k0 = 0; k0 < n; k0 += slice_pairs) {
+    const uint64_t k1 = std::min(n, k0 + slice_pairs), c0 = off_a[k0], c1 = off_a[k1], s = (*n_slices)++;
+    if (s >= max_slices) return SEQALIGN_E_ARG;
+    int passes = 0;
+    if (at > packed_cap) return SEQALIGN_E_NOMEM;
+    uint64_t bytes = u.bits && c1 > c0 ? pack_slice_learning(u, c0, c1, packed + at, packed_cap - at, task_syms ? task_syms : kTaskSyms, &passes) : 0;
+    const int bits = bytes ? u.bits : 0;
+    if (!bytes) {
+      bytes = c1 - c0;
+      if (bytes > packed_cap - at) return SEQALIGN_E_NOMEM;
+      gather(u, c0, c1, packed + at);
+    }
+    const uint64_t rec[8] = {c0, c1, at, (uint64_t)bits, bits ? u.n_dict : 0, (uint64_t)passes, bytes, 0};
+    memcpy(info + 8 * s, rec, sizeof(rec));
+    memset(dict + 16 * s, 0, 16);
+    if (bits) memcpy(dict + 16 * s, u.dict, u.n_dict);
+    at += (bytes + 15u) & ~(uint64_t)15;
+  }
+  return SEQALIGN_OK;
+}
diff --git a/seq-align_amd/host/sa_internal.h b/seq-align_amd/host/sa_internal.h
--- a/seq-align_amd/host/sa_internal.h
+++ b/seq-align_amd/host/sa_internal.h
@@ -76,6 +76,15 @@
                       const uint32_t *plane_b, uint32_t n_words, uint32_t n_moves, int format, int fold, char *out, uint64_t cap,
                       uint32_t pos[4], uint32_t *out_len);
 
+#define SA_SYM_DICT_MAX 16
+int sa_sym_bits(unsigned n_dict);
+unsigned sa_sym_dict_from_set(const uint32_t set[8], uint8_t dict[SA_SYM_DICT_MAX]);
+void sa_sym_set_add(uint32_t set[8], const uint8_t *src, uint64_t n);
+void sa_pack_symbols(const uint8_t *src, uint64_t n, const uint8_t *dict, unsigned n_dict, int bits, uint8_t *dst,
+                     uint32_t foreign[8]);
+int sa_pack_uses_simd(void);
+void sa_pack_force_scalar(int on);
+
 typedef int (*sa_hit_sink_t)(void *user, int32_t score, size_t end_x, size_t end_y,
                              size_t x, size_t y, size_t steps);
 
diff --git a/seq-align_amd/host/sa_pack.c b/seq-align_amd/host/sa_pack.c
--- /dev/null
+++ b/seq-align_amd/host/sa_pack.c
@@ -0,0 +1,101 @@
+#include <stdint.h>
+#include <string.h>
+
+#include "sa_internal.h"
+
+#if defined(__x86_64__)
+#include <immintrin.h>
+#endif
+
+int sa_sym_bits(unsigned n_dict) { return n_dict == 0 || n_dict > SA_SYM_DICT_MAX ? 0 : n_dict <= 4 ? 2 : 4; }
+
+unsigned sa_sym_dict_from_set(const uint32_t set[8], uint8_t dict[SA_SYM_DICT_MAX]) {
+  unsigned n = 0;
+  for (unsigned v = 0; v < 256; ++v)
+    if (set[v >> 5] >> (v & 31) & 1u) { if (n < SA_SYM_DICT_MAX) dict[n] = (uint8_t)v; ++n; }
+  return n;
+}
+
+void sa_sym_set_add(uint32_t set[8], const uint8_t *src, uint64_t n) {
+  for (uint64_t i = 0; i < n; ++i) set[src[i] >> 5] |= 1u << (src[i] & 31);
+}
+
+typedef void (*pack_fn)(const uint8_t *src, uint64_t n, const uint8_t *dict, unsigned n_dict, int bits, uint8_t *dst,
+                        uint32_t foreign[8]);
+
+static void pack_scalar(const uint8_t *src, uint64_t n, const uint8_t *dict, unsigned n_dict, int bits, uint8_t *dst,
+                        uint32_t foreign[8]) {
+  uint8_t code[256];
+  memset(code, 0xFF, sizeof(code));
+  for (unsigned d = 0; d < n_dict; ++d) code[dict[d]] = (uint8_t)d;
+  const unsigned per = bits == 2 ? 4 : 2;
+  for (uint64_t i = 0; i < n; i += per) {
+    unsigned out = 0;
+    for (unsigned k = 0; k < per && i + k < n; ++k) {
+      unsigned s = code[src[i + k]];
+      if (s == 0xFF) { foreign[src[i + k] >> 5] |= 1u << (src[i + k] & 31); s = 0; }
+      out |= s << (bits * k);
+    }
+    dst[i / per] = (uint8_t)out;
+  }
+}
+
+#if defined(__x86_64__)
+__attribute__((target("avx512f,avx512bw,bmi2")))
+static void pack_avx512(const uint8_t *src, uint64_t n, const uint8_t *dict, unsigned n_dict, int bits, uint8_t *dst,
+                        uint32_t foreign[8]) {
+  __m512i entry[SA_SYM_DICT_MAX];
+  for (unsigned d = 0; d < n_dict; ++d) entry[d] = _mm512_set1_epi8((char)dict[d]);
+  const uint64_t whole = n & ~(uint64_t)63;
+  for (uint64_t i = 0; i < whole; i += 64) {
+    const __m512i x = _mm512_loadu_si512((const void *)(src + i));
+    uint64_t plane[4] = {0, 0, 0, 0}, found = 0;
+    for (unsigned d = 0; d < n_dict; ++d) {
+      const uint64_t k = _mm512_cmpeq_epi8_mask(x, entry[d]);
+      found |= k;
+      if (d & 1) plane[0] |= k;
+      if (d & 2) plane[1] |= k;
+      if (d & 4) plane[2] |= k;
+      if (d & 8) plane[3] |= k;
+    }
+    if (found != ~0ull)
+      for (uint64_t m = ~found; m; m &= m - 1) { const uint8_t v = src[i + (unsigned)__builtin_ctzll(m)]; foreign[v >> 5] |= 1u << (v & 31); }
+    if (bits == 2) {
+      uint64_t out[2];
+      out[0] = _pdep_u64(plane[0], 0x5555555555555555ull) | _pdep_u64(plane[1], 0xAAAAAAAAAAAAAAAAull);
+      out[1] = _pdep_u64(plane[0] >> 32, 0x5555555555555555ull) | _pdep_u64(plane[1] >> 32, 0xAAAAAAAAAAAAAAAAull);
+      memcpy(dst + i / 4, out, 16);
+    } else {
+      uint64_t out[4];
+      for (unsigned q = 0; q < 4; ++q)
+        out[q] = _pdep_u64(plane[0] >> (16 * q), 0x1111111111111111ull) | _pdep_u64(plane[1] >> (16 * q), 0x2222222222222222ull) |
+                 _pdep_u64(plane[2] >> (16 * q), 0x4444444444444444ull) | _pdep_u64(plane[3] >> (16 * q), 0x8888888888888888ull);
+      memcpy(dst + i / 2, out, 32);
+    }
+  }
+  if (whole < n) pack_scalar(src + whole, n - whole, dict, n_dict, bits, dst + whole * (unsigned)bits / 8, foreign);
+}
+#endif
+
+static pack_fn pick_pack(void) {
+#if defined(__x86_64__)
+  __builtin_cpu_init();
+  if (__builtin_cpu_supports("avx512bw") && __builtin_cpu_supports("avx512f") && __builtin_cpu_supports("bmi2")) return pack_avx512;
+#endif
+  return pack_scalar;
+}
+
+static pack_fn g_pack;
+
+int sa_pack_uses_simd(void) {
+  if (!g_pack) g_pack = pick_pack();
+  return g_pack != pack_scalar;
+}
+
+void sa_pack_force_scalar(int on) { g_pack = on ? pack_scalar : pick_pack(); }
+
+void sa_pack_symbols(const uint8_t *src, uint64_t n, const uint8_t *dict, unsigned n_dict, int bits, uint8_t *dst,
+                     uint32_t foreign[8]) {
+  if (!g_pack) g_pack = pick_pack();
+  g_pack(src, n, dict, n_dict, bits, dst, foreign);
+}
diff --git a/seq-align_amd/python/seqalign_amd/__init__.py b/seq-align_amd/python/seqalign_amd/__init__.py
--- a/seq-align_amd/python/seqalign_amd/__init__.py
+++ b/seq-align_amd/python/seqalign_amd/__init__.py
@@ -95,6 +95,7 @@
         l.seqalign_last_error.restype = C.c_char_p
         l.seqalign_kernel_kind_name.restype = C.c_char_p
         l.seqalign_kernel_kind_ext_name.restype = C.c_char_p
+        l.seqalign_call_kind_ext_name.restype = C.c_char_p
         l.needleman_wunsch_new.restype = C.c_void_p
         l.smith_waterman_new.restype = C.c_void_p
         l.alignment_create.restype = C.c_void_p
@@ -140,7 +141,7 @@
 
 OPTION_DEFAULTS = {"kernel": "auto", "cpl": 0, "wpb": 0, "lds_pad": 0, "traceback": "device", "trace_kernel": "auto",
                    "sweep_mode": "auto", "sweep_strip": 0, "sweep_cpl": 0, "sweep_trace": 0, "sweep_dirs": 1, "nw_dirs": 1, "pack16": 1, "quad": 0, "walk_overlap": 0, "timing": 0, "chunk_bytes": 0,
-                   "subbatches": 0, "arena_scan_gib": 160, "arena_quality": 1.045, "arena_keep_gib": 16, "upload_slices": 0, "arena_free_pct": 60, "nw_moves": 1, "zero_copy": "auto", "sweep_ev": 1, "reduce_depth": 0, "async_lanes": 0, "walk_group": 0, "dirs_local": 1, "walk_stage": 1, "walk_tile": 0, "long_block_rows": 0}
+                   "subbatches": 0, "arena_scan_gib": 160, "arena_quality": 1.045, "arena_keep_gib": 16, "upload_slices": 0, "pack_upload": "auto", "arena_free_pct": 60, "nw_moves": 1, "zero_copy": "auto", "sweep_ev": 1, "reduce_depth": 0, "async_lanes": 0, "walk_group": 0, "dirs_local": 1, "walk_stage": 1, "walk_tile": 0, "long_block_rows": 0}
 
 
 K_MAX = 32
@@ -234,7 +235,7 @@
         _check(lib().seqalign_ctx_last_call_info_ext(self._h, C.byref(ext)), "seqalign_ctx_last_call_info_ext")
         for k in range(KX_MAX):
             if ext.launches[k]:
-                name = lib().seqalign_kernel_kind_ext_name(C.c_int(k))
+                name = lib().seqalign_call_kind_ext_name(C.c_int(k))
                 out[name.decode() if name else f"kind_ext{k}"] = (int(ext.launches[k]), int(ext.items[k]))
         return out
 
@@ -842,7 +843,7 @@
     "seqalign_fill_batch_device", "seqalign_sw_reduce_device", "seqalign_nw_traceback_device", "seqalign_sw_traceback_device", "seqalign_fill_batch", "seqalign_nw_batch",
     "seqalign_sw_batch", "seqalign_time_fill_ms", "seqalign_arenas_alloc", "seqalign_arenas_free",
     "seqalign_arenas_info", "seqalign_pool_trim", "seqalign_ctx_set_option", "seqalign_ctx_get_option", "seqalign_ctx_last_call_info",
-    "seqalign_kernel_kind_name", "seqalign_host_legs_nw", "seqalign_ctx_stream",
+    "seqalign_kernel_kind_name", "seqalign_host_legs_nw", "seqalign_pack_symbols_host", "seqalign_ctx_stream",
     "seqalign_fill_batch_multi", "seqalign_nw_batch_multi", "seqalign_sw_batch_multi", "seqalign_cigar",
     "seqalign_nw_batch_submit", "seqalign_sw_batch_submit", "seqalign_nw_batch_cigar_submit", "seqalign_job_wait", "seqalign_job_done",
     "seqalign_nw_batch_cigar", "seqalign_sw_batch_cigar", "seqalign_nw_batch_cigar_multi", "seqalign_sw_batch_cigar_multi",
@@ -852,7 +853,7 @@
     "seqalign_nw_score_search", "seqalign_sw_score_search", "seqalign_nw_score_search_multi",
     "seqalign_sw_score_search_multi",
     "seqalign_nw_align_long", "seqalign_sw_align_long",
-    "seqalign_nw_score_banded", "seqalign_nw_align_banded", "seqalign_band_score_time_ms", "seqalign_ctx_last_call_info_ext", "seqalign_kernel_kind_ext_name",
+    "seqalign_nw_score_banded", "seqalign_nw_align_banded", "seqalign_band_score_time_ms", "seqalign_ctx_last_call_info_ext", "seqalign_kernel_kind_ext_name", "seqalign_call_kind_ext_name",
     "seqalign_scoring_load_matrix", "seqalign_scoring_load_pairs", "seqalign_reader_open", "seqalign_reader_close",
     "seqalign_reader_next",
     "scoring_init", "scoring_add_wildcard", "scoring_add_mutation", "scoring_add_mutations", "scoring_print",
```

Result: no change. 549.9 GCUPS, median of 2 (-0.0%).
